# laomao0/BIN

Measured on AMD Instinct MI355X. Metric: interpolated frames/sec at 1280x720, higher is better.
Workload: dtype f16x3 (fp16 hi+lo pairs = 22-bit significands, 3 MFMA products, f32 accumulate; fp32-class: 1e-6 vs the fp32 reference); 1 GPU; Adobe240 test_blur 1280x720 inference, batch=1 per GPU (6-frame window padded to 768x1344 by the test.py rule), window-sharded; precision=f16x3, streams=1, pipelined_steps=False, four_call_schedule=False, parity=max-abs <= 2e-5 (f16x3) vs the fp32 reference (tests/)

## Files before the change

### bin_amd/_lib.py

```python
import ctypes as C
import os

from .build import EMA_LIB_PATH, ENS_LIB_PATH, GRAD_LIB_PATH, LIB_PATH, OPT_LIB_PATH, YUV_LIB_PATH

RDN_LAYERS = 66
RDN_MAX_LAYERS, RDN_MAX_CONVS = 192, 7
PLAN_KEEP_ACTS, PLAN_NO_FUSE, PLAN_RDB3, PLAN_FUSED_UPNET, PLAN_FUSED_UPNET_TRAIN = 1, 2, 4, 8, 16
BWD_ACCUMULATE = 1
BWD_SAVED_X3 = 2
BWD_FUSED_UPNET = 4
EPI_PLANES, EPI_SHUFFLE, EPI_FINAL, EPI_FINAL_SUBPIX = 0, 1, 2, 4
PROF_WGRAD = 16
LOSS_CHARBONNIER, LOSS_L1_SUM, LOSS_L2_SUM = 0, 1, 2
RDN_LAYOUT_WORDS, RDN_BWD_LAYOUT_WORDS = 16, 24


class BinConvDesc(C.Structure):
    _fields_ = [("N", C.c_int32), ("H", C.c_int32), ("W", C.c_int32), ("ksize", C.c_int32),
                ("cin_chunks", C.c_int32), ("cout", C.c_int32), ("cout_pad", C.c_int32),
                ("nterms", C.c_int32), ("epilogue", C.c_int32), ("relu", C.c_int32),
                ("x_cpg", C.c_int32), ("x_group_stride", C.c_int64), ("n_images", C.c_int32),
                ("reserved", C.c_int32), ("status", C.c_void_p)]


LOSS_MAX_TERMS = 24
CONV_HALF_LAST_CHUNK = 1


class BinLossTerms(C.Structure):
    _fields_ = [("x", C.c_void_p * LOSS_MAX_TERMS), ("y", C.c_void_p * LOSS_MAX_TERMS), ("n_terms", C.c_int32)]


class BinLossGrads(C.Structure):
    _fields_ = [("out", C.c_void_p * LOSS_MAX_TERMS), ("term_a", C.c_int32 * LOSS_MAX_TERMS),
                ("term_b", C.c_int32 * LOSS_MAX_TERMS), ("sign_a", C.c_float * LOSS_MAX_TERMS),
                ("sign_b", C.c_float * LOSS_MAX_TERMS), ("n_out", C.c_int32)]


class BinRdnShape(C.Structure):
    _fields_ = [("G0", C.c_int32), ("D", C.c_int32), ("C", C.c_int32), ("G", C.c_int32)]


class BinRdnPlan(C.Structure):
    _fields_ = [("N", C.c_int32), ("H", C.c_int32), ("W", C.c_int32), ("n_inputs", C.c_int32),
                ("nterms", C.c_int32), ("reserved", C.c_int32), ("shape", BinRdnShape),
                ("w_hi", C.c_void_p * RDN_MAX_LAYERS), ("w_lo", C.c_void_p * RDN_MAX_LAYERS),
                ("bias", C.c_void_p * RDN_MAX_LAYERS), ("status", C.c_void_p), ("profiler", C.c_void_p)]


class BinRdnBwdPlan(C.Structure):
    _fields_ = [("N", C.c_int32), ("H", C.c_int32), ("W", C.c_int32), ("n_inputs", C.c_int32),
                ("nterms", C.c_int32), ("reserved", C.c_int32), ("shape", BinRdnShape),
                ("wt_hi", C.c_void_p * RDN_MAX_LAYERS), ("wt_lo", C.c_void_p * RDN_MAX_LAYERS),
                ("zero_bias", C.c_void_p),
                ("dw", C.c_void_p * RDN_MAX_LAYERS), ("db", C.c_void_p * RDN_MAX_LAYERS), ("gin", C.c_void_p * 5),
                ("status", C.c_void_p), ("aux_stream", C.c_void_p), ("profiler", C.c_void_p)]


class BinRelayoutItem(C.Structure):
    _fields_ = [("w", C.c_void_p * (RDN_MAX_CONVS + 1)), ("bias", C.c_void_p), ("w_hi", C.c_void_p), ("w_lo", C.c_void_p),
                ("bias_out", C.c_void_p), ("kind", C.c_int32), ("cout", C.c_int32), ("cin", C.c_int32),
                ("ksize", C.c_int32), ("rows_pad", C.c_int32), ("cin_chunks", C.c_int32), ("cout_block", C.c_int32),
                ("shuffle_or_group", C.c_int32), ("shape", BinRdnShape)]


RELAYOUT_FWD, RELAYOUT_DGRAD, RELAYOUT_RDB_GATHER = 0, 1, 2
SCORE_SSIM_G11, SCORE_SSIM_U7 = 1, 2
SCORE_MAX_PAIRS = 32

ADAM_MAX_TENSORS = 64


class BinAdamTensor(C.Structure):
    _fields_ = [("p", C.c_void_p), ("g", C.c_void_p), ("m", C.c_void_p), ("v", C.c_void_p), ("numel", C.c_int64),
                ("step_size", C.c_float), ("inv_sqrt_bc2", C.c_float)]


GRAD_MAX_TENSORS = 128
GRAD_FLAG_NONFINITE, GRAD_FLAG_STATUS = 1, 2


class BinGradTensor(C.Structure):
    _fields_ = [("g", C.c_void_p), ("numel", C.c_int64)]


class BinGradRecord(C.Structure):
    _fields_ = [("sumsq", C.c_double), ("norm", C.c_float), ("coef", C.c_float), ("flags", C.c_int32), ("status", C.c_uint32),
                ("reserved", C.c_int32 * 2)]


EMA_MAX_TENSORS = 136


class BinEmaTensor(C.Structure):
    _fields_ = [("e", C.c_void_p), ("p", C.c_void_p), ("numel", C.c_int64)]


ENS_FLIP_W, ENS_FLIP_H = 1, 2
ENS_MAX_ORIENT, ENS_MAX_SOURCES, ENS_MAX_SLOTS = 8, 6, 14


class BinEnsOrient(C.Structure):
    _fields_ = [("src", C.c_void_p), ("dst", C.c_void_p * ENS_MAX_ORIENT), ("flip", C.c_uint8 * ENS_MAX_ORIENT), ("n_dst", C.c_int32)]


class BinEnsMerge(C.Structure):
    _fields_ = [("src", C.c_void_p * ENS_MAX_ORIENT), ("dst", C.c_void_p)]


YUV_CHROMA_420, YUV_CHROMA_444 = 420, 444
YUV_MATRIX_BT601, YUV_MATRIX_BT709 = 0, 1
YUV_RANGE_LIMITED, YUV_RANGE_FULL = 0, 1


class BinYuvFormat(C.Structure):
    _fields_ = [("chroma", C.c_int32), ("matrix", C.c_int32), ("range", C.c_int32)]


_SIGNATURES = {
    "binhip_version": (C.c_int, []),
    "binhip_device_cus": (C.c_int, []),
    "binhip_conv_cout_block": (C.c_int, [C.c_int, C.c_int, C.c_int]),
    "binhip_weights_bytes": (C.c_size_t, [C.c_int, C.c_int, C.c_int]),
    "binhip_weights_relayout": (C.c_int, [C.c_void_p, C.c_void_p, C.c_int, C.c_int, C.c_int, C.c_int, C.c_int,
                                          C.c_int, C.c_int, C.c_void_p, C.c_void_p, C.c_void_p, C.c_void_p]),
    "binhip_weights_relayout_batch": (C.c_int, [C.POINTER(BinRelayoutItem), C.c_int, C.c_void_p]),
    "binhip_conv2d_fwd": (C.c_int, [C.POINTER(BinConvDesc)] + [C.c_void_p] * 10 +
                          [C.POINTER(C.c_void_p), C.c_void_p]),
    "binhip_nchw_to_planes": (C.c_int, [C.c_void_p, C.c_int, C.c_int, C.c_int, C.c_int, C.c_void_p, C.c_void_p,
                                        C.c_void_p, C.c_void_p]),
    "binhip_planes_to_nchw": (C.c_int, [C.c_void_p, C.c_void_p, C.c_int, C.c_int, C.c_int, C.c_int, C.c_void_p,
                                        C.c_void_p]),
    "binhip_pixel_unshuffle_f32": (C.c_int, [C.c_void_p, C.c_int, C.c_int, C.c_int, C.c_int, C.c_int, C.c_void_p,
                                             C.c_void_p]),
    "binhip_pack_inputs": (C.c_int, [C.POINTER(C.c_void_p), C.c_int, C.c_int, C.c_int, C.c_int, C.c_void_p,
                                     C.c_void_p, C.c_void_p, C.c_void_p]),
    "binhip_u8_to_frame": (C.c_int, [C.c_void_p, C.c_int, C.c_int, C.c_int, C.c_int, C.c_int, C.c_int, C.c_void_p,
                                     C.c_void_p]),
    "binhip_frame_to_u8": (C.c_int, [C.c_void_p, C.c_int, C.c_int, C.c_int, C.c_int, C.c_int, C.c_int, C.c_void_p,
                                     C.c_void_p]),
    "binhip_convlstm_fwd": (C.c_int, [C.c_void_p] * 5 + [C.c_float, C.c_int, C.c_int, C.c_int, C.c_void_p,
                                                          C.c_void_p, C.c_void_p]),
    "binhip_lstm_gates_fwd": (C.c_int, [C.c_void_p, C.c_void_p, C.c_float, C.c_int, C.c_int, C.c_int, C.c_int, C.c_void_p,
                                        C.c_void_p, C.c_void_p]),
    "binhip_lstm_gates_bwd": (C.c_int, [C.c_void_p] * 4 + [C.c_float, C.c_int, C.c_int, C.c_int, C.c_int, C.c_void_p, C.c_void_p,
                                        C.c_void_p]),
    "binhip_charbonnier_partials": (C.c_int, [C.c_int64]),
    "binhip_charbonnier_fwd": (C.c_int, [C.c_void_p, C.c_void_p, C.c_int64, C.c_float, C.c_void_p, C.c_void_p,
                                         C.c_void_p]),
    "binhip_charbonnier_bwd": (C.c_int, [C.c_void_p, C.c_void_p, C.c_int64, C.c_float, C.c_void_p, C.c_void_p,
                                         C.c_void_p, C.c_void_p]),
    "binhip_pixel_loss_fwd": (C.c_int, [C.c_int, C.c_void_p, C.c_void_p, C.c_int64, C.c_float, C.c_void_p, C.c_void_p,
                                        C.c_void_p]),
    "binhip_pixel_loss_bwd": (C.c_int, [C.c_int, C.c_void_p, C.c_void_p, C.c_int64, C.c_float, C.c_void_p, C.c_void_p,
                                        C.c_void_p, C.c_void_p]),
    "binhip_multi_loss_fwd": (C.c_int, [C.c_int, C.POINTER(BinLossTerms), C.c_int64, C.c_float, C.c_void_p, C.c_void_p,
                                        C.c_void_p, C.c_void_p]),
    "binhip_multi_loss_bwd": (C.c_int, [C.c_int, C.POINTER(BinLossTerms), C.c_int64, C.c_float, C.c_void_p,
                                        C.POINTER(BinLossGrads), C.c_void_p]),
    "binhip_dgrad_rows_pad": (C.c_int, [C.c_int, C.c_int]),
    "binhip_weights_relayout_dgrad": (C.c_int, [C.c_void_p, C.c_int, C.c_int, C.c_int, C.c_int, C.c_int, C.c_int,
                                                C.c_int, C.c_void_p, C.c_void_p, C.c_void_p, C.c_void_p]),
    "binhip_weights_relayout_rdb_gather": (C.c_int, [C.c_void_p, C.c_int, C.c_int, C.c_void_p, C.c_void_p, C.c_void_p,
                                                     C.c_void_p]),
    "binhip_conv2d_bwd_data": (C.c_int, [C.POINTER(BinConvDesc)] + [C.c_void_p] * 7 + [C.c_int, C.c_void_p,
                                         C.c_void_p, C.c_void_p, C.c_int, C.c_int, C.c_int64, C.c_void_p,
                                         C.c_void_p, C.c_void_p]),
    "binhip_wgrad_workspace_bytes": (C.c_size_t, [C.c_int] * 6),
    "binhip_conv2d_bwd_weight": (C.c_int, [C.POINTER(BinConvDesc)] + [C.c_void_p] * 6 + [C.c_size_t, C.c_void_p,
                                           C.c_void_p, C.c_int, C.c_int, C.c_int, C.c_void_p]),
    "binhip_grad_scale": (C.c_int, [C.c_void_p, C.c_int64, C.c_float, C.c_void_p, C.c_void_p, C.c_void_p]),
    "binhip_nchw_to_planes_scaled": (C.c_int, [C.c_void_p, C.c_int, C.c_int, C.c_int, C.c_int, C.c_void_p,
                                               C.c_void_p, C.c_void_p, C.c_void_p, C.c_void_p]),
    "binhip_unshuffle_planes": (C.c_int, [C.c_void_p, C.c_void_p, C.c_int, C.c_int, C.c_int, C.c_int, C.c_void_p,
                                          C.c_void_p, C.c_void_p]),
    "binhip_unpack_input_grads": (C.c_int, [C.c_void_p, C.c_void_p, C.c_void_p, C.c_void_p, C.c_int, C.c_int, C.c_int,
                                            C.c_int, C.POINTER(C.c_void_p), C.c_void_p]),
    "binhip_convlstm_bwd_workspace_bytes": (C.c_size_t, [C.c_int, C.c_int, C.c_int]),
    "binhip_convlstm_bwd": (C.c_int, [C.c_void_p] * 5 + [C.c_float, C.c_int, C.c_int, C.c_int, C.c_void_p, C.c_void_p,
                                      C.c_void_p, C.c_size_t] + [C.c_void_p] * 6),
    "binhip_rdn_backward_workspace_bytes": (C.c_size_t, [C.c_int] * 5 + [C.POINTER(BinRdnShape)]),
    "binhip_rdn_backward": (C.c_int, [C.POINTER(BinRdnBwdPlan), C.c_void_p, C.c_size_t, C.c_void_p, C.c_void_p,
                                      C.c_size_t, C.c_void_p]),
    "binhip_profiler_create": (C.c_int, [C.c_int, C.c_int, C.c_int, C.c_int, C.POINTER(C.c_void_p)]),
    "binhip_profiler_read": (C.c_int, [C.c_void_p, C.POINTER(C.c_double), C.POINTER(C.c_int)]),
    "binhip_profiler_destroy": (None, [C.c_void_p]),
    "binhip_rdb_tail_fwd": (C.c_int, [C.c_int, C.c_int, C.c_int, C.c_int] + [C.c_void_p] * 10 +
                            [C.c_int, C.c_void_p, C.c_void_p]),
    "binhip_rdn_workspace_bytes": (C.c_size_t, [C.c_int, C.c_int, C.c_int, C.c_int, C.c_int, C.POINTER(BinRdnShape)]),
    "binhip_rdn_workspace_layout": (C.c_int, [C.c_int] * 5 + [C.POINTER(BinRdnShape), C.POINTER(C.c_int64), C.c_int]),
    "binhip_rdn_backward_workspace_layout": (C.c_int, [C.c_int] * 5 + [C.POINTER(BinRdnShape), C.POINTER(C.c_int64), C.c_int]),
    "binhip_rdn_forward": (C.c_int, [C.POINTER(BinRdnPlan), C.POINTER(C.c_void_p), C.c_void_p, C.c_void_p,
                                     C.c_size_t, C.c_void_p]),
    "binhip_image_score_workspace_bytes": (C.c_size_t, [C.c_int] * 4),
    "binhip_image_score": (C.c_int, [C.c_void_p, C.c_void_p, C.c_int, C.c_int, C.c_int, C.c_int, C.POINTER(C.c_double),
                                     C.c_void_p, C.c_size_t, C.c_void_p, C.c_void_p]),
    "binhip_frame_score_workspace_bytes": (C.c_size_t, [C.c_int] * 4),
    "binhip_frame_score": (C.c_int, [C.POINTER(C.c_void_p), C.POINTER(C.c_void_p), C.c_int, C.c_int, C.c_int, C.c_int,
                                     C.POINTER(C.c_double), C.c_void_p, C.c_size_t, C.c_void_p, C.c_void_p]),
    "binhip_gather_windows": (C.c_int, [C.c_void_p, C.c_int, C.c_int, C.c_int, C.c_void_p, C.c_int, C.c_int, C.c_int, C.c_int,
                                        C.c_void_p, C.c_void_p]),
    "binhip_gather_windows_blur": (C.c_int, [C.c_void_p, C.c_int, C.c_int, C.c_int, C.c_void_p] + [C.c_int] * 5 +
                                   [C.c_void_p, C.c_void_p]),
}

OPT_VERSION = 100
_OPT_SIGNATURES = {
    "binopt_version": (C.c_int, []),
    "binopt_adam_step": (C.c_int, [C.POINTER(BinAdamTensor), C.c_int, C.c_float, C.c_float, C.c_float, C.c_float, C.c_void_p]),
}

GRAD_VERSION = 100
_GRAD_SIGNATURES = {
    "bingrad_version": (C.c_int, []),
    "bingrad_norm_workspace_bytes": (C.c_int64, [C.POINTER(BinGradTensor), C.c_int]),
    "bingrad_norm": (C.c_int, [C.POINTER(BinGradTensor), C.c_int, C.c_float, C.c_void_p, C.c_uint32, C.c_void_p, C.c_void_p,
                               C.c_void_p]),
    "bingrad_scale": (C.c_int, [C.POINTER(BinGradTensor), C.c_int, C.c_void_p, C.c_void_p]),
}

EMA_VERSION = 100
_EMA_SIGNATURES = {
    "binema_version": (C.c_int, []),
    "binema_step": (C.c_int, [C.POINTER(BinEmaTensor), C.c_int, C.c_float, C.c_void_p]),
}

ENS_VERSION = 100
_ENS_SIGNATURES = {
    "binens_version": (C.c_int, []),
    "binens_orient": (C.c_int, [C.POINTER(BinEnsOrient), C.c_int, C.c_int, C.c_int, C.c_int, C.c_void_p]),
    "binens_merge": (C.c_int, [C.POINTER(BinEnsMerge), C.c_int, C.c_int, C.POINTER(C.c_uint8), C.c_int, C.c_int, C.c_int, C.c_void_p]),
}

YUV_VERSION = 100
_YUV_SIGNATURES = {
    "binyuv_version": (C.c_int, []),
    "binyuv_to_frame": (C.c_int, [C.c_void_p, C.c_void_p, C.c_void_p, C.c_int, C.c_int, C.POINTER(BinYuvFormat), C.c_int, C.c_int, C.c_int,
                                  C.c_int, C.c_void_p, C.c_void_p]),
    "binyuv_from_frame": (C.c_int, [C.c_void_p, C.c_int, C.c_int, C.c_int, C.c_int, C.c_int, C.c_int, C.POINTER(BinYuvFormat), C.c_void_p,
                                    C.c_void_p, C.c_void_p, C.c_void_p]),
}

STATUS_SATURATED = 1
STATUS_SYNC_TIMEOUT = 2

_lib = _optlib = _gradlib = _emalib = _enslib = _yuvlib = None


def _load(path, built_path, signatures, version=None):
    if not os.path.exists(path):
        raise RuntimeError(
            f"bin_amd: HIP library {built_path} not built. Run `python -c 'import __graft_entry__ as g; "
            f"g.build()'` (hipcc --offload-arch=gfx950). There is no CPU fallback by design.")
    h = C.CDLL(path)
    for name, (res, args) in signatures.items():
        fn = getattr(h, name)
        fn.restype = res
        fn.argtypes = args
    if version is not None and getattr(h, version[0])() != version[1]:
        raise RuntimeError(f"bin_amd: {path} is version {getattr(h, version[0])()}, this binding is for {version[1]}")
    return h


def exported_symbols():
    return sorted(_SIGNATURES)


def lib():
    global _lib
    if _lib is None:
        _lib = _load(os.environ.get("BIN_AMD_LIB", LIB_PATH), LIB_PATH, _SIGNATURES)
    return _lib


def opt_exported_symbols():
    return sorted(_OPT_SIGNATURES)


def optlib():
    global _optlib
    if _optlib is None:
        _optlib = _load(OPT_LIB_PATH, OPT_LIB_PATH, _OPT_SIGNATURES, ("binopt_version", OPT_VERSION))
    return _optlib


def grad_exported_symbols():
    return sorted(_GRAD_SIGNATURES)


def gradlib():
    global _gradlib
    if _gradlib is None:
        _gradlib = _load(GRAD_LIB_PATH, GRAD_LIB_PATH, _GRAD_SIGNATURES, ("bingrad_version", GRAD_VERSION))
    return _gradlib


def ema_exported_symbols():
    return sorted(_EMA_SIGNATURES)


def emalib():
    global _emalib
    if _emalib is None:
        _emalib = _load(EMA_LIB_PATH, EMA_LIB_PATH, _EMA_SIGNATURES, ("binema_version", EMA_VERSION))
    return _emalib


def ens_exported_symbols():
    return sorted(_ENS_SIGNATURES)


def enslib():
    global _enslib
    if _enslib is None:
        _enslib = _load(ENS_LIB_PATH, ENS_LIB_PATH, _ENS_SIGNATURES, ("binens_version", ENS_VERSION))
    return _enslib


def yuv_exported_symbols():
    return sorted(_YUV_SIGNATURES)


def yuvlib():
    global _yuvlib
    if _yuvlib is None:
        _yuvlib = _load(YUV_LIB_PATH, YUV_LIB_PATH, _YUV_SIGNATURES, ("binyuv_version", YUV_VERSION))
    return _yuvlib


def check(rc, what):
    if rc != 0:
        kind = {-1: "bad argument", -2: "unsupported shape", -3: "workspace too small"}.get(rc, f"hipError {rc}")
        raise RuntimeError(f"bin_amd: {what} failed: {kind}")
```

### bin_amd/csrc/binhip_conv.hip

```cpp
#include "binhip_conv_common.h"
#include <vector>
#include <cstdio>
#include <cstdlib>

template <int KS, int MT, int WM, int R, int WN, int KC, int NT, int NBUF, int EPI>
struct ConvCfg {
    static constexpr int PAD = KS / 2;
    static constexpr int COUTB = 32 * MT * WM;
    static constexpr int TH = R * WN;
    static constexpr int PH = TH + KS - 1;
    static constexpr int PW = 32 + KS - 1;
    static constexpr int PP = (PH * PW * 2 + 63) / 64;
    static constexpr int WP = KS * KS * MT * WM;
    static constexpr int CHUNK_BYTES = (PP + WP) * 1024;
    static constexpr int NPL = (NT == 3) ? 2 : 1;
    static constexpr int PLANE_BYTES = KC * CHUNK_BYTES;
    static constexpr int BUF_BYTES = NPL * PLANE_BYTES;
    static constexpr int NW = WM * WN;
    static constexpr int LDS_BYTES = NBUF * BUF_BYTES + 1024;
    static constexpr int NPJ = (PP + NW - 1) / NW;
    static constexpr int NWJ = (WP + NW - 1) / NW;
    static constexpr int PS = NPL * KC * (NPJ + NWJ);
    static_assert(NW == 4 || NW == 8 || NW == 16, "4, 8 or 16 waves per workgroup");
    static_assert(LDS_BYTES <= 160 * 1024, "LDS budget");
    static_assert(NBUF >= 2, "ring of at least two stage buffers");
    static_assert(NBUF <= 2 || (NBUF - 2) * PS <= 63, "vmcnt immediate range");
};

template <class C, int KS, int KC>
__device__ __forceinline__ void issue_stage(const ConvKArgs& a, char* smem, int st, int buf, int wave, int lane, const ConvTile& t,
                                            const unsigned* voff) {
    char* bbase = smem + buf * C::BUF_BYTES;
    char* dummy = smem + (C::LDS_BYTES - 1024);
    const int nchunks = a.nchunks;
#pragma unroll
    for (int pl = 0; pl < C::NPL; ++pl) {
#pragma unroll
        for (int kc = 0; kc < KC; ++kc) {
            const int c = st * KC + kc;
            if (c < nchunks) {
                __amdgpu_buffer_rsrc_t rs = patch_plane_grouped(a, c, pl, t);
                char* lds = bbase + pl * C::PLANE_BYTES + kc * C::CHUNK_BYTES;
#pragma unroll
                for (int j = 0; j < C::NPJ; ++j) {
                    const int i = wave + C::NW * j;
                    const bool real = ((C::PP % C::NW == 0) || (i < C::PP));
                    __builtin_amdgcn_raw_ptr_buffer_load_lds(rs, (lds_void_t*)(real ? lds + i * 1024 : dummy), 16,
                                                             real ? voff[j] : 0x80000000u, 0, 0, 0);
                }
                const _Float16* wb = (pl ? a.w_lo : a.w_hi) +
                                     ((long long)t.z * nchunks + c) * (KS * KS * C::COUTB * 16);
                __amdgpu_buffer_rsrc_t ws = __builtin_amdgcn_make_buffer_rsrc(
                    (void*)wb, 0, KS * KS * C::COUTB * 32, 0x00020000);
#pragma unroll
                for (int j = 0; j < C::NWJ; ++j) {
                    const int i = wave + C::NW * j;
                    const bool real = ((C::WP % C::NW == 0) || (i < C::WP));
                    __builtin_amdgcn_raw_ptr_buffer_load_lds(ws, (lds_void_t*)(real ? lds + (C::PP + i) * 1024 : dummy), 16,
                                                             real ? (unsigned)(lane * 16) : 0x80000000u,
                                                             real ? i * 1024 : 0, 0, 0);
                }
            }
        }
    }
}

template <class C, int KS, int MT, int R, int NT>
__device__ __forceinline__ void load_frags(const char* bbase, int kc, int dx, int wm, int a_lane_off, int b_lane_off,
                                           half8 (&Bh)[R + KS - 1], half8 (&Bl)[R + KS - 1],
                                           half8 (&Ah)[KS][MT], half8 (&Al)[KS][MT]) {
    const char* pb = bbase + kc * C::CHUNK_BYTES;
    const char* wb = pb + C::PP * 1024 + wm * (MT * 32 * 32);
#pragma unroll
    for (int rr = 0; rr < R + KS - 1; ++rr) {
        const int off = b_lane_off + (rr * C::PW + dx) * 16;
        Bh[rr] = ld8(pb + off);
        if constexpr (NT == 3) Bl[rr] = ld8(pb + C::PLANE_BYTES + off);
    }
#pragma unroll
    for (int dy = 0; dy < KS; ++dy)
#pragma unroll
        for (int mt = 0; mt < MT; ++mt) {
            const int off = ((dy * KS + dx) * C::COUTB + mt * 32) * 32 + a_lane_off;
            Ah[dy][mt] = ld8(wb + off);
            if constexpr (NT == 3) Al[dy][mt] = ld8(wb + C::PLANE_BYTES + off);
        }
}

template <class C, int KS, int MT, int R, int KC, int NT>
__device__ __forceinline__ void compute_stage(const char* smem, int st, int buf, int nchunks, int wm,
                                              int a_lane_off, int b_lane_off, floatx16 (&acc)[MT][R]) {
    const char* bbase = smem + buf * C::BUF_BYTES;
    constexpr int NSTEP = KC * KS;
    constexpr int FRAG_REGS = ((R + KS - 1) + KS * MT) * 4 * ((NT == 3) ? 2 : 1);
    constexpr bool PIPE = (MT * R * 16 + 2 * FRAG_REGS + 40) <= 232;
    constexpr int NSET = PIPE ? 2 : 1;
    half8 Bh[NSET][R + KS - 1], Bl[NSET][R + KS - 1], Ah[NSET][KS][MT], Al[NSET][KS][MT];
    int nvalid = NSTEP;
    if constexpr (KC > 1) {
        const int left = nchunks - st * KC;
        nvalid = (left < KC ? left : KC) * KS;
    }
    if constexpr (PIPE)
        load_frags<C, KS, MT, R, NT>(bbase, 0, 0, wm, a_lane_off, b_lane_off, Bh[0], Bl[0], Ah[0], Al[0]);
#pragma unroll
    for (int s = 0; s < NSTEP; ++s) {
        if (KC == 1 || s < nvalid) {
            if constexpr (PIPE) {
                if (s + 1 < NSTEP && (KC == 1 || s + 1 < nvalid))
                    load_frags<C, KS, MT, R, NT>(bbase, (s + 1) / KS, (s + 1) % KS, wm, a_lane_off, b_lane_off,
                                                 Bh[(s + 1) & 1], Bl[(s + 1) & 1], Ah[(s + 1) & 1], Al[(s + 1) & 1]);
            } else {
                load_frags<C, KS, MT, R, NT>(bbase, s / KS, s % KS, wm, a_lane_off, b_lane_off, Bh[0], Bl[0], Ah[0], Al[0]);
            }
            if constexpr (PIPE) __builtin_amdgcn_sched_barrier(0);
#pragma unroll
            for (int dy = 0; dy < KS; ++dy)
#pragma unroll
                for (int mt = 0; mt < MT; ++mt)
#pragma unroll
                    for (int r = 0; r < R; ++r) {
                        if constexpr (NT == 3) {
                            acc[mt][r] = mfma_32x32x16(Al[s & (NSET - 1)][dy][mt], Bh[s & (NSET - 1)][r + dy], acc[mt][r]);
                            acc[mt][r] = mfma_32x32x16(Ah[s & (NSET - 1)][dy][mt], Bl[s & (NSET - 1)][r + dy], acc[mt][r]);
                        }
                        acc[mt][r] = mfma_32x32x16(Ah[s & (NSET - 1)][dy][mt], Bh[s & (NSET - 1)][r + dy], acc[mt][r]);
                    }
            if constexpr (PIPE) __builtin_amdgcn_sched_barrier(0);
        }
    }
}

template <int KS, int MT, int WM, int R, int WN, int KC, int NT, int NBUF, int EPI, bool XTRA>
__global__ void __launch_bounds__(64 * WM * WN) __attribute__((amdgpu_waves_per_eu(2)))
conv_mfma_kernel(const ConvKArgs a, const float* __restrict__ bias) {
    using C = ConvCfg<KS, MT, WM, R, WN, KC, NT, NBUF, EPI>;
    extern __shared__ __attribute__((aligned(16))) char smem[];

    const int tid = threadIdx.x;
    const int lane = tid & 63;
    const int wave = __builtin_amdgcn_readfirstlane(tid >> 6);
    const int wm = wave / WN;
    const int wn = wave % WN;
    const int n = lane & 31;
    const int kg = lane >> 5;

    const ConvTile t = tile_decode<C::TH>(a, a.ncol);
    unsigned voff[C::NPJ];
    patch_offsets<C, C::PAD>(voff, t, a.H, a.W, wave, lane);

    floatx16 acc[MT][R];
#pragma unroll
    for (int mt = 0; mt < MT; ++mt)
#pragma unroll
        for (int r = 0; r < R; ++r)
#pragma unroll
            for (int e = 0; e < 16; ++e) acc[mt][r][e] = 0.f;

    const int nchunks = a.nchunks;
    const int nst = (nchunks + KC - 1) / KC;
    const int a_lane_off = weight_lane_off(n, kg);
    const int b_lane_off = patch_lane_off<C>(n, kg, wn * R);

    const int nfull = nchunks / KC;
#pragma unroll
    for (int s0 = 0; s0 < NBUF - 1; ++s0)
        if (s0 < nst) issue_stage<C, KS, KC>(a, smem, s0, s0, wave, lane, t, voff);
    int cur = 0, nxt = NBUF - 1;
    for (int st = 0; st < nst; ++st) {
        int yf = nfull - 1 - st;
        yf = yf < 0 ? 0 : (yf > NBUF - 2 ? NBUF - 2 : yf);
        if (NBUF >= 4 && yf >= 2) wait_vmcnt<(NBUF >= 4 ? 2 : 0) * C::PS>();
        else if (NBUF >= 3 && yf >= 1) wait_vmcnt<(NBUF >= 3 ? 1 : 0) * C::PS>();
        else wait_vmcnt<0>();
        __builtin_amdgcn_s_barrier();
        __builtin_amdgcn_sched_barrier(0);
        if (st + NBUF - 1 < nst)
            issue_stage<C, KS, KC>(a, smem, st + NBUF - 1, nxt, wave, lane, t, voff);
        compute_stage<C, KS, MT, R, KC, NT>(smem, st, cur, nchunks, wm, a_lane_off, b_lane_off, acc);
        cur = (cur + 1 == NBUF) ? 0 : cur + 1;
        nxt = (nxt + 1 == NBUF) ? 0 : nxt + 1;
    }

    conv_epilogue<MT, R, NT, EPI, XTRA>(a, bias, acc, t.img, t.ty0 + wn * R, t.tx0, t.z * C::COUTB + wm * MT * 32, t.z == 0 && wm == 0,
                                        n, kg, t.plane_elems);
}

template <int KS, int MT, int WM, int R, int WN, int KC, int NT, int NBUF, int EPI, bool XTRA>
static int launch_cfg_x(const ConvKArgs& ka, int cout_pad, hipStream_t s) {
    using C = ConvCfg<KS, MT, WM, R, WN, KC, NT, NBUF, EPI>;
    static std::atomic<unsigned long long> lds_set{0};
    if (int rc = bh_set_max_lds(&conv_mfma_kernel<KS, MT, WM, R, WN, KC, NT, NBUF, EPI, XTRA>, C::LDS_BYTES, lds_set)) return rc;
    ConvKArgs a = ka;
    const dim3 grid(set_tiles<C>(a, cout_pad / C::COUTB));
    conv_mfma_kernel<KS, MT, WM, R, WN, KC, NT, NBUF, EPI, XTRA><<<grid, dim3(64 * C::NW), C::LDS_BYTES, s>>>(a, a.bias);
    BH_CHECK_LAUNCH();
    return 0;
}
template <int KS, int MT, int WM, int R, int WN, int KC, int NT, int NBUF, int EPI>
static int launch_cfg(const ConvKArgs& ka, int cout_pad, hipStream_t s) {
    if constexpr (EPI == BINHIP_EPI_PLANES) {
        if (ka.has_res || ka.r2_hi || ka.m_hi || ka.y_unshuf)
            return launch_cfg_x<KS, MT, WM, R, WN, KC, NT, NBUF, EPI, true>(ka, cout_pad, s);
    }
    return launch_cfg_x<KS, MT, WM, R, WN, KC, NT, NBUF, EPI, false>(ka, cout_pad, s);
}

struct BinhipProfiler {
    int ks = 0, cout_pad = 0, epi = 0;
    std::vector<hipEvent_t> ev;
    size_t used = 0;
};
namespace { constexpr size_t PROF_MAX_PAIRS = 16384; }

int bh_conv_cout_block(int ksize, int cout_pad, int nterms) {
    if (cout_pad <= 0 || cout_pad % 32) return -1;
    if (ksize == 3 && nterms == 3) return 32;
    if (ksize == 3 && cout_pad == 256) return 128;
    if (ksize == 5) return 32;
    if (ksize == 1 && cout_pad == 224) return 224;
    if (ksize == 1 && cout_pad == 1152) return 192;
    if (cout_pad % 96 == 0) return 96;
    if (ksize == 3 && cout_pad % 64 == 0) return 64;
    return 32;
}

static int bh_dispatch_conv(const ConvKArgs& a, int k, int cp, int nt, int e, hipStream_t s);
int bh_launch_conv_x3(const ConvKArgs& a, int cout_pad, int epilogue, hipStream_t s);
int bh_launch_final_dot2(const ConvKArgs& a, hipStream_t s);
int bh_launch_conv_x3_k5(const ConvKArgs& a, int cout_pad, hipStream_t s);
int bh_launch_conv_x3_k5_subpix(const ConvKArgs& a, hipStream_t s);
int bh_launch_final_m16(const ConvKArgs& a, hipStream_t s);

int bh_prepare_conv(const BhConvCall& c, ConvKArgs* out) {
    const BinConvDesc& d = c.d;
    if (!c.x_hi || !c.w_hi || !c.bias) return BINHIP_E_ARG;
    if (d.nterms != 1 && d.nterms != 3) return BINHIP_E_ARG;
    if (d.nterms == 3 && (!c.x_lo || !c.w_lo)) return BINHIP_E_ARG;
    if (d.N <= 0 || d.H <= 0 || d.W <= 0 || d.cin_chunks <= 0) return BINHIP_E_SHAPE;
    if ((long long)d.N * d.H * d.W >= (1ll << 26)) return BINHIP_E_SHAPE;
    ConvKArgs a;
    a.x_hi = (const _Float16*)c.x_hi; a.x_lo = (const _Float16*)c.x_lo;
    a.w_hi = (const _Float16*)c.w_hi; a.w_lo = (const _Float16*)c.w_lo;
    a.bias = c.bias;
    a.y_hi = (_Float16*)c.y_hi; a.y_lo = (_Float16*)c.y_lo;
    a.r_hi = (const _Float16*)c.r_hi; a.r_lo = (const _Float16*)c.r_lo;
    a.r2_hi = (const _Float16*)c.r2_hi; a.r2_lo = (const _Float16*)c.r2_lo;
    a.m_hi = (const _Float16*)c.m_hi;
    a.flags = (unsigned*)c.status;
    a.res_chunks = c.res_chunks > 0 ? c.res_chunks : (1 << 30);
    a.mask_from = c.mask_from;
    a.y_cpg = c.y_cpg; a.y_group_stride = c.y_group_stride;
    a.y_cpg_inv = c.y_cpg > 0 ? (unsigned)(((1u << 20) + c.y_cpg - 1) / c.y_cpg) : 0u;
    if (c.y_cpg > 128 || (c.y_cpg > 0 && d.cout_pad / 16 >= 4096)) return BINHIP_E_SHAPE;
    a.half_last = (d.reserved & BINHIP_CONV_HALF_LAST_CHUNK) ? 1 : 0;
    a.y_unshuf = c.y_unshuf;
    if (c.y_unshuf && (d.epilogue != BINHIP_EPI_PLANES || c.y_cpg > 0 || (d.H & 1) || (d.W & 1) || c.y_unshuf * 16 < d.cout))
        return BINHIP_E_SHAPE;
    if (c.r2_hi && d.nterms == 3 && !c.r2_lo) return BINHIP_E_ARG;
    a.out_f32 = c.y_f32;
    for (int i = 0; i < 5; ++i) a.img[i] = c.images[i];
    a.group_stride = d.x_group_stride;
    a.N = d.N; a.H = d.H; a.W = d.W;
    a.nchunks = d.cin_chunks;
    a.cpg = d.x_cpg;
    a.relu = d.relu; a.has_res = (c.r_hi != nullptr); a.nimg = d.n_images; a.cout = d.cout;
    a.och_limit = (d.epilogue == BINHIP_EPI_PLANES) ? (d.cout + 15) / 16 : (1 << 30);
    a.tiles_x = a.tiles_y = 0;
    a.ncol = 1;
    a.wt = 0;
    a.prog_prio = 0;
#if BINHIP_TIMELINE
    a.tl = nullptr; a.tl_launch = 0; a.tl_base = 0;
#endif
    const int P = BINHIP_EPI_PLANES, S = BINHIP_EPI_SHUFFLE, F = BINHIP_EPI_FINAL;
    if (d.epilogue == P) {
        if (!c.y_hi || (d.nterms == 3 && !c.y_lo)) return BINHIP_E_ARG;
        if (a.has_res && d.nterms == 3 && !c.r_lo) return BINHIP_E_ARG;
    } else if (d.epilogue == S) {
        if (!c.y_hi || (d.nterms == 3 && !c.y_lo)) return BINHIP_E_ARG;
        if (d.cout % 4) return BINHIP_E_SHAPE;
    } else if (d.epilogue == F) {
        if (!c.y_f32 || d.cout > 4 || d.n_images < 0 || d.n_images > 5) return BINHIP_E_ARG;
    } else if (d.epilogue == BINHIP_EPI_FINAL_SUBPIX) {
        if (!c.y_f32 || d.cout <= 0 || (d.cout & 3) || d.cout > 12 || d.n_images < 0 || d.n_images > 5) return BINHIP_E_ARG;
        if (d.ksize != 5 || d.cout_pad != 32) return BINHIP_E_SHAPE;
    } else {
        return BINHIP_E_ARG;
    }
    {
        const int e = d.epilogue, cp = d.cout_pad;
        const long long out_chunks = (e == BINHIP_EPI_SHUFFLE) ? (a.cout / 4 + 15) / 16 : (cp + 15) / 16;
        const long long px = (long long)a.N * a.H * a.W * ((e == BINHIP_EPI_SHUFFLE) ? 4 : 1);
        const long long span = (a.y_cpg > 0 ? ((out_chunks + a.y_cpg - 1) / a.y_cpg) * a.y_group_stride * 2 : out_chunks * px * 32);
        a.wt = (e == BINHIP_EPI_PLANES && span < (1ll << 32) - 64) ? 1 : 0;
    }
    *out = a;
    return 0;
}

bool bh_prof_begin(BinhipProfiler* pr, int ks, int cout_pad, int epi, hipStream_t s) {
    if (!pr || ks != pr->ks || cout_pad != pr->cout_pad || epi != pr->epi || pr->used + 2 > pr->ev.size()) return false;
    (void)hipEventRecord(pr->ev[pr->used], s);
    return true;
}
void bh_prof_end(BinhipProfiler* pr, hipStream_t s) {
    (void)hipEventRecord(pr->ev[pr->used + 1], s);
    pr->used += 2;
}

int bh_launch_conv(const BhConvCall& c, hipStream_t s) {
    ConvKArgs a;
    if (int rc = bh_prepare_conv(c, &a)) return rc;
    const BinConvDesc& d = c.d;
    const int k = d.ksize, cp = d.cout_pad, nt = d.nterms, e = d.epilogue;
    if (bh_prof_begin(c.prof, k, cp, e, s)) {
        const int rc = bh_dispatch_conv(a, k, cp, nt, e, s);
        bh_prof_end(c.prof, s);
        return rc;
    }
    return bh_dispatch_conv(a, k, cp, nt, e, s);
}

static int bh_dispatch_conv(const ConvKArgs& a, int k, int cp, int nt, int e, hipStream_t s) {
    const int P = BINHIP_EPI_PLANES, S = BINHIP_EPI_SHUFFLE, F = BINHIP_EPI_FINAL;
    const int cb = bh_conv_cout_block(k, cp, nt);
    if (cb <= 0 || cp % cb) return BINHIP_E_SHAPE;
    if (e == BINHIP_EPI_FINAL_SUBPIX)
        return nt == 3 ? bh_launch_conv_x3_k5_subpix(a, s) : launch_cfg<5, 1, 1, 2, 8, 1, 1, 2, BINHIP_EPI_FINAL_SUBPIX>(a, cp, s);
    if (e == F && k == 3 && cp == 32 && a.cout <= 3 && nt == 1)
        return bh_launch_final_dot2(a, s);
    if (e == F && k == 3 && cp == 32 && a.cout <= 3 && nt == 3 && a.nchunks <= 4)
        return bh_launch_final_m16(a, s);
    if (nt == 1) {
        if (e == F && k == 3 && cp == 32) return launch_cfg<3, 1, 1, 2, 8, 1, 1, 2, F>(a, cp, s);
        if (e == S && k == 3 && cp == 256) return launch_cfg<3, 2, 2, 4, 4, 1, 1, 2, S>(a, cp, s);
        if (e == P && k == 3 && cb == 32)  return launch_cfg<3, 1, 1, 2, 8, 1, 1, 2, P>(a, cp, s);
        if (e == P && k == 3 && cb == 64)  return launch_cfg<3, 2, 1, 2, 4, 1, 1, 2, P>(a, cp, s);
        if (e == P && k == 3 && cb == 96)  return launch_cfg<3, 3, 1, 2, 4, 1, 1, 2, P>(a, cp, s);
        if (e == P && k == 3 && cb == 128) return launch_cfg<3, 2, 2, 4, 4, 1, 1, 2, P>(a, cp, s);
        if (e == P && k == 1 && cb == 224) return launch_cfg<1, 7, 1, 1, 8, 2, 1, 2, P>(a, cp, s);
        if (e == P && k == 1 && cb == 192) return launch_cfg<1, 6, 1, 1, 8, 2, 1, 2, P>(a, cp, s);
        if (e == P && k == 1 && cb == 32)  return launch_cfg<1, 1, 1, 4, 4, 4, 1, 2, P>(a, cp, s);
        if (e == P && k == 1 && cb == 96) {
            if (a.nchunks >= 32) return launch_cfg<1, 3, 1, 2, 4, 2, 1, 2, P>(a, cp, s);
            return launch_cfg<1, 3, 1, 1, 8, 2, 1, 2, P>(a, cp, s);
        }
        if (e == P && k == 5 && cb == 32)  return launch_cfg<5, 1, 1, 2, 8, 1, 1, 2, P>(a, cp, s);
    } else {
        if (k == 3 && cb == 32) return bh_launch_conv_x3(a, cp, e, s);
        if (e == S && k == 3 && cp == 256) return launch_cfg<3, 1, 2, 4, 2, 1, 3, 2, S>(a, cp, s);
        if (e == P && k == 3 && cb == 64)  return launch_cfg<3, 2, 1, 2, 4, 1, 3, 2, P>(a, cp, s);
        if (e == P && k == 3 && cb == 96)  return launch_cfg<3, 3, 1, 1, 8, 1, 3, 2, P>(a, cp, s);
        if (e == P && k == 1 && cb == 224) {
            if (a.has_res && a.m_hi && !a.r2_hi && a.res_chunks == 6 && a.mask_from == 12 && a.y_cpg <= 0 && !a.y_unshuf &&
                a.och_limit >= 14 && cp == 224)
                return launch_cfg_x<1, 7, 1, 1, 8, 1, 3, 2, BINHIP_EPI_PLANES_LFFD, true>(a, cp, s);
            return launch_cfg<1, 7, 1, 1, 8, 1, 3, 2, P>(a, cp, s);
        }
        if (e == P && k == 1 && cb == 192) return launch_cfg<1, 6, 1, 1, 8, 1, 3, 2, P>(a, cp, s);
        if (e == P && k == 1 && cb == 32)  return launch_cfg<1, 1, 1, 4, 4, 2, 3, 2, P>(a, cp, s);
        if (e == P && k == 1 && cb == 96) {
            if (a.nchunks >= 32) return launch_cfg<1, 3, 1, 2, 4, 1, 3, 2, P>(a, cp, s);
            return launch_cfg<1, 3, 1, 1, 8, 1, 3, 2, P>(a, cp, s);
        }
        if (e == P && k == 5 && cb == 32)  return bh_launch_conv_x3_k5(a, cp, s);
    }
    return BINHIP_E_SHAPE;
}

__device__ __forceinline__ void relayout_body(long long t, const float* __restrict__ w, const float* __restrict__ bias,
                                              int cout, int cin, int ks, int cout_pad, int nchunks, int cb, int shuffle,
                                              _Float16* __restrict__ w_hi, _Float16* __restrict__ w_lo,
                                              float* __restrict__ bias_out) {
    const long long total = (long long)cout_pad * nchunks * ks * ks * 2;
    if (t < cout_pad) {
        int src = (int)t;
        if (shuffle) { const int cq = cout / 4; const int sub = (int)t / cq, cc = (int)t % cq; src = cc * 4 + sub; }
        bias_out[t] = (src < cout && bias) ? bias[src] : 0.f;
    }
    if (t >= total) return;
    const int s = (int)(t & 1);
    long long u = t >> 1;
    const int row = (int)(u % cb); u /= cb;
    const int tap = (int)(u % (ks * ks)); u /= (ks * ks);
    const int c = (int)(u % nchunks); u /= nchunks;
    const int zb = (int)u;
    const int rg = zb * cb + row;
    int src = rg;
    if (shuffle) { const int cq = cout / 4; const int sub = rg / cq, cc = rg % cq; src = cc * 4 + sub; }
    const int cg = s ^ ((row >> 3) & 1);
    const int dy = tap / ks, dx = tap % ks;
    half8 hv, lv;
#pragma unroll
    for (int e = 0; e < 8; ++e) {
        const int ci = c * 16 + cg * 8 + e;
        float v = 0.f;
        if (src < cout && ci < cin) v = w[(((long long)src * cin + ci) * ks + dy) * ks + dx];
        hv[e] = (_Float16)v;
        lv[e] = (_Float16)(v - (float)hv[e]);
    }
    *reinterpret_cast<half8*>(w_hi + t * 8) = hv;
    if (w_lo) *reinterpret_cast<half8*>(w_lo + t * 8) = lv;
}
__global__ void relayout_kernel(const float* __restrict__ w, const float* __restrict__ bias, int cout, int cin,
                                int ks, int cout_pad, int nchunks, int cb, int shuffle,
                                _Float16* __restrict__ w_hi, _Float16* __restrict__ w_lo,
                                float* __restrict__ bias_out) {
    relayout_body((long long)blockIdx.x * blockDim.x + threadIdx.x, w, bias, cout, cin, ks, cout_pad, nchunks, cb, shuffle,
                  w_hi, w_lo, bias_out);
}

__device__ __forceinline__ void relayout_dgrad_body(long long t, const float* __restrict__ w, int cout, int cin, int ks,
                                                    int rows_pad, int nchunks, int cb, int shuffle,
                                                    _Float16* __restrict__ w_hi, _Float16* __restrict__ w_lo,
                                                    float* __restrict__ bias_out) {
    const long long total = (long long)rows_pad * nchunks * ks * ks * 2;
    if (t < rows_pad) bias_out[t] = 0.f;
    if (t >= total) return;
    const int s = (int)(t & 1);
    long long u = t >> 1;
    const int row = (int)(u % cb); u /= cb;
    const int tap = (int)(u % (ks * ks)); u /= (ks * ks);
    const int c = (int)(u % nchunks); u /= nchunks;
    const int zb = (int)u;
    const int r = zb * cb + row;
    const int cg = s ^ ((row >> 3) & 1);
    const int dy = ks - 1 - tap / ks, dx = ks - 1 - tap % ks;
    half8 hv, lv;
#pragma unroll
    for (int e = 0; e < 8; ++e) {
        const int j = c * 16 + cg * 8 + e;
        int co = j;
        if (shuffle) { const int cq = cout / 4; const int sub = j / cq, cc = j % cq; co = cc * 4 + sub; }
        float v = 0.f;
        if (r < cin && j < cout) v = w[(((long long)co * cin + r) * ks + dy) * ks + dx];
        hv[e] = (_Float16)v;
        lv[e] = (_Float16)(v - (float)hv[e]);
    }
    *reinterpret_cast<half8*>(w_hi + t * 8) = hv;
    if (w_lo) *reinterpret_cast<half8*>(w_lo + t * 8) = lv;
}
__global__ void relayout_dgrad_kernel(const float* __restrict__ w, int cout, int cin, int ks, int rows_pad,
                                      int nchunks, int cb, int shuffle, _Float16* __restrict__ w_hi,
                                      _Float16* __restrict__ w_lo, float* __restrict__ bias_out) {
    relayout_dgrad_body((long long)blockIdx.x * blockDim.x + threadIdx.x, w, cout, cin, ks, rows_pad, nchunks, cb, shuffle,
                        w_hi, w_lo, bias_out);
}

struct GatherSrc { const float* w[BINHIP_RDN_MAX_CONVS + 1]; int G0, G; };
__device__ __forceinline__ void relayout_rdb_gather_body(long long t, const GatherSrc& src, int group, int rows, int nchunks,
                                                         int cb, _Float16* __restrict__ w_hi, _Float16* __restrict__ w_lo,
                                                         float* __restrict__ bias_out) {
    const long long total = (long long)rows * nchunks * 9 * 2;
    if (t < rows) bias_out[t] = 0.f;
    if (t >= total) return;
    const int s = (int)(t & 1);
    long long u = t >> 1;
    const int row = (int)(u % cb); u /= cb;
    const int tap = (int)(u % 9); u /= 9;
    const int c = (int)(u % nchunks); u /= nchunks;
    const int r = (int)u * cb + row;
    const int cg = s ^ ((row >> 3) & 1);
    const int dy = 2 - tap / 3, dx = 2 - tap % 3;
    const int G0 = src.G0, G = src.G;
    const int cmin = group;
    const int ci = (group == 0) ? r : G0 + G * (group - 1) + r;
    const int j0 = c * 16 + cg * 8;
    const int conv = cmin + j0 / G;
    const int cin_c = G0 + G * conv;
    const float* w = src.w[conv];
    half8 hv, lv;
#pragma unroll
    for (int e = 0; e < 8; ++e) {
        const int co = (j0 % G) + e;
        const float v = w[(((long long)co * cin_c + ci) * 3 + dy) * 3 + dx];
        hv[e] = (_Float16)v;
        lv[e] = (_Float16)(v - (float)hv[e]);
    }
    *reinterpret_cast<half8*>(w_hi + t * 8) = hv;
    if (w_lo) *reinterpret_cast<half8*>(w_lo + t * 8) = lv;
}
__global__ void relayout_rdb_gather_kernel(GatherSrc src, int group, int rows, int nchunks, int cb,
                                           _Float16* __restrict__ w_hi, _Float16* __restrict__ w_lo,
                                           float* __restrict__ bias_out) {
    relayout_rdb_gather_body((long long)blockIdx.x * blockDim.x + threadIdx.x, src, group, rows, nchunks, cb, w_hi, w_lo, bias_out);
}

#define RELAYOUT_BATCH 22
struct RelayoutBatch {
    BinRelayoutItem it[RELAYOUT_BATCH];
    unsigned start[RELAYOUT_BATCH + 1];
    int n;
};
__global__ void __launch_bounds__(256)
relayout_batch_kernel(const RelayoutBatch rb) {
    const unsigned b = blockIdx.x;
    int li = 0;
#pragma unroll
    for (int i = 1; i < RELAYOUT_BATCH; ++i)
        if (i < rb.n && b >= rb.start[i]) li = i;
    const BinRelayoutItem& L = rb.it[li];
    const long long t = (long long)(b - rb.start[li]) * 256 + threadIdx.x;
    if (L.kind == BINHIP_RELAYOUT_FWD) {
        relayout_body(t, L.w[0], L.bias, L.cout, L.cin, L.ksize, L.rows_pad, L.cin_chunks, L.cout_block, L.shuffle_or_group,
                      (_Float16*)L.w_hi, (_Float16*)L.w_lo, L.bias_out);
    } else if (L.kind == BINHIP_RELAYOUT_DGRAD) {
        relayout_dgrad_body(t, L.w[0], L.cout, L.cin, L.ksize, L.rows_pad, L.cin_chunks, L.cout_block, L.shuffle_or_group,
                            (_Float16*)L.w_hi, (_Float16*)L.w_lo, L.bias_out);
    } else {
        GatherSrc src;
#pragma unroll
        for (int i = 0; i <= BINHIP_RDN_MAX_CONVS; ++i) src.w[i] = L.w[i];
        src.G0 = L.shape.G0 > 0 ? L.shape.G0 : 96;
        src.G = L.shape.G > 0 ? L.shape.G : 32;
        relayout_rdb_gather_body(t, src, L.shuffle_or_group, L.rows_pad, L.cin_chunks, L.cout_block, (_Float16*)L.w_hi,
                                 (_Float16*)L.w_lo, L.bias_out);
    }
}

extern "C" {

int binhip_weights_relayout_batch(const BinRelayoutItem* items, int n, void* stream) {
    if (!items || n <= 0) return BINHIP_E_ARG;
    for (int i = 0; i < n; ++i) {
        const BinRelayoutItem& L = items[i];
        if (!L.w[0] || !L.w_hi || !L.bias_out) return BINHIP_E_ARG;
        if (L.kind == BINHIP_RELAYOUT_FWD) {
            if (L.rows_pad % 32 || L.cout_block <= 0 || L.rows_pad % L.cout_block || L.cout_block % 32) return BINHIP_E_SHAPE;
            if (L.cin > L.cin_chunks * 16 || L.cout > L.rows_pad) return BINHIP_E_SHAPE;
            if (L.shuffle_or_group && (L.cout % 4 || L.cout != L.rows_pad)) return BINHIP_E_SHAPE;
        } else if (L.kind == BINHIP_RELAYOUT_DGRAD) {
            if (L.rows_pad % 32 || L.cout_block <= 0 || L.rows_pad % L.cout_block || L.cout_block % 32) return BINHIP_E_SHAPE;
            if (L.cin > L.rows_pad || L.cout > L.cin_chunks * 16) return BINHIP_E_SHAPE;
            if (L.shuffle_or_group && L.cout % 4) return BINHIP_E_SHAPE;
        } else if (L.kind == BINHIP_RELAYOUT_RDB_GATHER) {
            const int g = L.shuffle_or_group;
            const int G0 = L.shape.G0 > 0 ? L.shape.G0 : 96, G = L.shape.G > 0 ? L.shape.G : 32, C = L.shape.C > 0 ? L.shape.C : 4;
            if (C > BINHIP_RDN_MAX_CONVS || G0 % 32 || G % 32) return BINHIP_E_SHAPE;
            if (g < 0 || g >= C) return BINHIP_E_ARG;
            if (L.rows_pad != (g == 0 ? G0 : G) || L.cin_chunks != (C - g) * G / 16 || L.ksize != 3) return BINHIP_E_SHAPE;
            if (L.cout_block <= 0 || L.rows_pad % L.cout_block || L.cout_block % 32) return BINHIP_E_SHAPE;
            for (int k = g; k < C; ++k) if (!L.w[k]) return BINHIP_E_ARG;
        } else {
            return BINHIP_E_ARG;
        }
    }
    for (int i0 = 0; i0 < n; i0 += RELAYOUT_BATCH) {
        RelayoutBatch rb;
        const int m = (n - i0 < RELAYOUT_BATCH) ? n - i0 : RELAYOUT_BATCH;
        unsigned blocks = 0;
        for (int i = 0; i < m; ++i) {
            rb.it[i] = items[i0 + i];
            rb.start[i] = blocks;
            const BinRelayoutItem& L = rb.it[i];
            const long long total = (long long)L.rows_pad * L.cin_chunks * L.ksize * L.ksize * 2;
            blocks += (unsigned)((total + 255) / 256);
        }
        for (int i = m; i < RELAYOUT_BATCH; ++i) rb.it[i] = rb.it[0];
        for (int i = m; i <= RELAYOUT_BATCH; ++i) rb.start[i] = blocks;
        rb.n = m;
        hipLaunchKernelGGL(relayout_batch_kernel, dim3(blocks), dim3(256), 0, (hipStream_t)stream, rb);
        BH_CHECK_LAUNCH();
    }
    return 0;
}

int binhip_dgrad_rows_pad(int ksize, int cin) {
    return ((cin + 31) / 32) * 32;
}

int binhip_weights_relayout_dgrad(const float* w_oihw, int cout, int cin, int ksize, int rows_pad, int cin_chunks,
                                  int cout_block, int shuffle_perm, void* w_hi, void* w_lo, float* bias_out,
                                  void* stream) {
    if (!w_oihw || !w_hi || !bias_out) return BINHIP_E_ARG;
    if (rows_pad % 32 || cout_block <= 0 || rows_pad % cout_block || cout_block % 32) return BINHIP_E_SHAPE;
    if (cin > rows_pad || cout > cin_chunks * 16) return BINHIP_E_SHAPE;
    if (shuffle_perm && cout % 4) return BINHIP_E_SHAPE;
    const long long total = (long long)rows_pad * cin_chunks * ksize * ksize * 2;
    const long long nb = (total + 255) / 256;
    hipLaunchKernelGGL(relayout_dgrad_kernel, dim3((unsigned)nb), dim3(256), 0, (hipStream_t)stream, w_oihw, cout, cin,
                       ksize, rows_pad, cin_chunks, cout_block, shuffle_perm, (_Float16*)w_hi, (_Float16*)w_lo, bias_out);
    BH_CHECK_LAUNCH();
    return 0;
}

int binhip_weights_relayout_rdb_gather(const float* const* w_oihw4, int group, int cout_block, void* w_hi, void* w_lo,
                                       float* bias_out, void* stream) {
    if (!w_oihw4 || !w_hi || !bias_out || group < 0 || group > 3) return BINHIP_E_ARG;
    const int rows = group == 0 ? 96 : 32;
    const int nchunks = 2 * (4 - group);
    if (cout_block <= 0 || rows % cout_block || cout_block % 32) return BINHIP_E_SHAPE;
    GatherSrc src;
    for (int i = 0; i <= BINHIP_RDN_MAX_CONVS; ++i) src.w[i] = nullptr;
    src.G0 = 96; src.G = 32;
    for (int i = 0; i < 4; ++i) {
        src.w[i] = w_oihw4[i];
        if (i >= group && !src.w[i]) return BINHIP_E_ARG;
    }
    const long long total = (long long)rows * nchunks * 9 * 2;
    hipLaunchKernelGGL(relayout_rdb_gather_kernel, dim3((unsigned)((total + 255) / 256)), dim3(256), 0,
                       (hipStream_t)stream, src, group, rows, nchunks, cout_block, (_Float16*)w_hi, (_Float16*)w_lo,
                       bias_out);
    BH_CHECK_LAUNCH();
    return 0;
}

int binhip_conv2d_bwd_data(const BinConvDesc* d, const void* gy_hi, const void* gy_lo, const void* wt_hi,
                           const void* wt_lo, const float* zero_bias, const void* res_hi, const void* res_lo,
                           int res_chunks, const void* acc_hi, const void* acc_lo, const void* mask_hi, int mask_from,
                           int y_cpg, int64_t y_group_stride, void* gx_hi, void* gx_lo, void* stream) {
    if (!d) return BINHIP_E_ARG;
    if (d->epilogue != BINHIP_EPI_PLANES) return BINHIP_E_ARG;
    if (d->reserved < 0) return BINHIP_E_ARG;
    BhConvCall c;
    c.d = *d;
    c.x_hi = gy_hi; c.x_lo = gy_lo; c.w_hi = wt_hi; c.w_lo = wt_lo; c.bias = zero_bias;
    c.r_hi = res_hi; c.r_lo = res_lo; c.res_chunks = res_chunks;
    c.r2_hi = acc_hi; c.r2_lo = acc_lo;
    c.m_hi = mask_hi; c.mask_from = mask_from;
    c.y_cpg = y_cpg; c.y_group_stride = y_group_stride;
    c.y_unshuf = d->reserved > 0 ? d->reserved : 0;
    c.d.reserved = 0;
    c.y_hi = gx_hi; c.y_lo = gx_lo;
    c.status = d->status;
    return bh_launch_conv(c, (hipStream_t)stream);
}

#if BINHIP_TIMELINE
BINHIP_API int binhip_set_timeline(void* buf, unsigned cap) {
    const unsigned used = g_bh_tl_next.exchange(0);
    g_bh_tl_buf = buf;
    g_bh_tl_cap = cap;
    g_bh_tl_serial.store(0);
    return (int)(used < g_bh_tl_cap || !buf ? used : used);
}
#endif

int binhip_profiler_create(int ksize, int cout_pad, int epilogue, int max_launches, BinhipProfiler** out) {
    if (!out || max_launches <= 0 || (size_t)max_launches > PROF_MAX_PAIRS) return BINHIP_E_ARG;
    BinhipProfiler* p = new BinhipProfiler();
    p->ks = ksize; p->cout_pad = cout_pad; p->epi = epilogue;
    for (int i = 0; i < 2 * max_launches; ++i) {
        hipEvent_t ev;
        hipError_t e = hipEventCreate(&ev);
        if (e != hipSuccess) { binhip_profiler_destroy(p); return (int)e; }
        p->ev.push_back(ev);
    }
    *out = p;
    return 0;
}

int binhip_profiler_read(BinhipProfiler* p, double* total_ms, int* launches) {
    if (!p) return BINHIP_E_ARG;
    double tot = 0.0;
    int n = 0;
    for (size_t i = 0; i + 1 < p->used; i += 2) {
        hipError_t e = hipEventSynchronize(p->ev[i + 1]);
        if (e != hipSuccess) return (int)e;
        float ms = 0.f;
        e = hipEventElapsedTime(&ms, p->ev[i], p->ev[i + 1]);
        if (e != hipSuccess) return (int)e;
        tot += ms;
        ++n;
    }
    if (total_ms) *total_ms = tot;
    if (launches) *launches = n;
    p->used = 0;
    return 0;
}

void binhip_profiler_destroy(BinhipProfiler* p) {
    if (!p) return;
    for (hipEvent_t ev : p->ev) (void)hipEventDestroy(ev);
    delete p;
}

int binhip_conv_cout_block(int ksize, int cout_pad, int nterms) { return bh_conv_cout_block(ksize, cout_pad, nterms); }

size_t binhip_weights_bytes(int cout_pad, int cin_chunks, int ksize) {
    return (size_t)cout_pad * cin_chunks * ksize * ksize * 32;
}

int binhip_weights_relayout(const float* w_oihw, const float* bias, int cout, int cin, int ksize,
                            int cout_pad, int cin_chunks, int cout_block, int shuffle_perm,
                            void* w_hi, void* w_lo, float* bias_out, void* stream) {
    if (!w_oihw || !w_hi || !bias_out) return BINHIP_E_ARG;
    if (cout_pad % 32 || cout_block <= 0 || cout_pad % cout_block || cout_block % 32) return BINHIP_E_SHAPE;
    if (cin > cin_chunks * 16 || cout > cout_pad) return BINHIP_E_SHAPE;
    if (shuffle_perm && (cout % 4 || cout != cout_pad)) return BINHIP_E_SHAPE;
    const long long total = (long long)cout_pad * cin_chunks * ksize * ksize * 2;
    const int th = 256;
    const long long nb = (total + th - 1) / th;
    hipLaunchKernelGGL(relayout_kernel, dim3((unsigned)nb), dim3(th), 0, (hipStream_t)stream, w_oihw, bias, cout, cin,
                       ksize, cout_pad, cin_chunks, cout_block, shuffle_perm, (_Float16*)w_hi, (_Float16*)w_lo,
                       bias_out);
    BH_CHECK_LAUNCH();
    return 0;
}

int binhip_conv2d_fwd(const BinConvDesc* d, const void* x_hi, const void* x_lo, const void* w_hi,
                      const void* w_lo, const float* bias, const void* res_hi, const void* res_lo,
                      void* y_hi, void* y_lo, float* y_f32, const float* const* images, void* stream) {
    if (!d) return BINHIP_E_ARG;
    if (d->reserved & ~BINHIP_CONV_HALF_LAST_CHUNK) return BINHIP_E_ARG;
    if ((d->reserved & BINHIP_CONV_HALF_LAST_CHUNK) && d->ksize != 5) return BINHIP_E_ARG;
    BhConvCall c;
    c.d = *d;
    c.x_hi = x_hi; c.x_lo = x_lo; c.w_hi = w_hi; c.w_lo = w_lo; c.bias = bias;
    c.r_hi = res_hi; c.r_lo = res_lo; c.y_hi = y_hi; c.y_lo = y_lo; c.y_f32 = y_f32;
    c.status = d->status;
    for (int i = 0; images && i < d->n_images && i < 5; ++i) c.images[i] = images[i];
    if (d->epilogue == BINHIP_EPI_FINAL && d->n_images > 0 && !images) return BINHIP_E_ARG;
    return bh_launch_conv(c, (hipStream_t)stream);
}

}
```

### bin_amd/csrc/binhip_conv_common.h

```cpp
#pragma once
#include "binhip_internal.h"
#include <type_traits>
#ifndef BINHIP_TIMELINE
#define BINHIP_TIMELINE 0
#endif

typedef _Float16 half8 __attribute__((ext_vector_type(8)));
typedef _Float16 half4 __attribute__((ext_vector_type(4)));
typedef float floatx16 __attribute__((ext_vector_type(16)));
typedef float floatx4 __attribute__((ext_vector_type(4)));
typedef __attribute__((address_space(3))) void lds_void_t;
typedef unsigned u32x4 __attribute__((ext_vector_type(4)));

int bh_launch_upnet_ring(const void* x_hi, const void* x_lo, const float* wvar, const float* bvar, float* out, const float* const* images,
                         int nimg, int N, int H, int W, int cin, hipStream_t s);
int bh_upnet_gsub(const float* g, int N, int H, int W, const float* scale, void* y_hi, void* y_lo, void* status, hipStream_t s);
int bh_upnet_ring_dgrad(const float* g, const float* wvar, const float* scale, void* gx_hi, void* gx_lo, void* status, int N, int H, int W,
                        int cin, hipStream_t s);
int bh_upnet_ring_wgrad(const float* g, const void* x_hi, const void* x_lo, float* dwvar, float* dbvar, int N, int H, int W, int cin,
                        int accumulate, hipStream_t s);
struct ConvKArgs {
    const _Float16* x_hi;
    const _Float16* x_lo;
    const _Float16* w_hi;
    const _Float16* w_lo;
    const float* bias;
    _Float16* y_hi;
    _Float16* y_lo;
    const _Float16* r_hi;
    const _Float16* r_lo;
    const _Float16* r2_hi;
    const _Float16* r2_lo;
    const _Float16* m_hi;
    float* out_f32;
    const float* img[5];
    unsigned* flags;
    long long group_stride;
    int N, H, W;
    int nchunks;
    int cpg;
    int tiles_x, tiles_y;
    int ncol;
    int relu, has_res, nimg, cout;
    int wt;
    int och_limit;
    int res_chunks;
    int mask_from;
    int y_cpg;
    unsigned y_cpg_inv;
    long long y_group_stride;
    int prog_prio;
    int half_last;
#if BINHIP_TIMELINE
    void* tl;
    unsigned tl_launch;
    unsigned tl_base;
#endif
    int y_unshuf;
};

#if BINHIP_TIMELINE
#include <atomic>
struct BhTlRec {
    unsigned kind_launch, bid, hwid, xcc;
    unsigned long long rt[5];
    unsigned long long clk[2];
    unsigned long long pad;
};
static_assert(sizeof(BhTlRec) == 80, "record size (tools/wg_timeline.py)");
struct BhTlBuf { unsigned cursor, cap, pad[2]; BhTlRec rec[1]; };
inline void* g_bh_tl_buf = nullptr;
inline unsigned g_bh_tl_cap = 0;
inline std::atomic<unsigned> g_bh_tl_serial{0}, g_bh_tl_next{0};
inline void* bh_tl_reserve(unsigned n, unsigned* base) {
    if (!g_bh_tl_buf) return nullptr;
    const unsigned b = g_bh_tl_next.fetch_add(n);
    *base = b;
    return (b + n <= g_bh_tl_cap) ? g_bh_tl_buf : nullptr;
}
struct BhTl {
    unsigned long long rt[5], clk[2];
    __device__ __forceinline__ void stamp(int i) {
        __builtin_amdgcn_sched_barrier(0);
        rt[i] = __builtin_amdgcn_s_memrealtime();
        __builtin_amdgcn_sched_barrier(0);
    }
    __device__ __forceinline__ void begin() { clk[0] = __builtin_amdgcn_s_memtime(); stamp(0); }
    __device__ __forceinline__ void finish(void* tl, unsigned kind_launch, unsigned i) {
        stamp(3);
        if (threadIdx.x < 64) asm volatile("s_waitcnt vmcnt(0)" ::: "memory");
        stamp(4);
        clk[1] = __builtin_amdgcn_s_memtime();
        if (tl && threadIdx.x == 0) {
            BhTlBuf* b = (BhTlBuf*)tl;
            {
                BhTlRec& r = b->rec[i];
                r.kind_launch = kind_launch; r.bid = blockIdx.x;
                r.hwid = __builtin_amdgcn_s_getreg((31 << 11) | 4);
                r.xcc = __builtin_amdgcn_s_getreg((31 << 11) | 20);
                for (int k = 0; k < 5; ++k) r.rt[k] = rt[k];
                r.clk[0] = clk[0]; r.clk[1] = clk[1];
            }
        }
    }
};
#define BH_TL_DECL BhTl tl__
#define BH_TL_BEGIN() tl__.begin()
#define BH_TL_STAMP(i) tl__.stamp(i)
#define BH_TL_FINISH(a, i) tl__.finish((a).tl, (a).tl_launch, (a).tl_base + (unsigned)(i))
#else
#define BH_TL_DECL
#define BH_TL_BEGIN()
#define BH_TL_STAMP(i)
#define BH_TL_FINISH(a, i)
#endif

#define BINHIP_EPI_PLANES_LFFD 3

template <int N>
__device__ __forceinline__ void wait_vmcnt() {
    asm volatile("s_waitcnt vmcnt(%0)" ::"n"(N) : "memory");
}

__device__ __forceinline__ void store16(_Float16* base, long long off_elems, uint4 v, int wt) {
    if (wt) {
        __amdgpu_buffer_rsrc_t rs = __builtin_amdgcn_make_buffer_rsrc((void*)base, 0, 0xFFFFFFFFu, 0x00020000);
        u32x4 d = {v.x, v.y, v.z, v.w};
        __builtin_amdgcn_raw_buffer_store_b128(d, rs, (int)(off_elems * 2), 0, 16);
    } else {
        *reinterpret_cast<uint4*>(base + off_elems) = v;
    }
}

__device__ __forceinline__ int xcd_band(int bid, int nwg) {
    const int q = nwg >> 3, r = nwg & 7, xcd = bid & 7, k = bid >> 3;
    return (xcd < r ? xcd * (q + 1) : r * (q + 1) + (xcd - r) * q) + k;
}

struct ConvTile {
    int z, tx, ty, img;
    int tx0, ty0;
    long long plane_elems;
    unsigned plane_bytes;
};
template <int TH, class A>
__device__ __forceinline__ ConvTile tile_at(const A& a, int t, int z) {
    ConvTile o;
    o.z = z;
    o.tx = t % a.tiles_x;
    t /= a.tiles_x;
    o.ty = t % a.tiles_y;
    o.img = t / a.tiles_y;
    o.tx0 = o.tx * 32;
    o.ty0 = o.ty * TH;
    o.plane_elems = (long long)a.N * a.H * a.W * 16;
    o.plane_bytes = (unsigned)(o.plane_elems * 2);
    return o;
}
template <int TH, class A>
__device__ __forceinline__ ConvTile tile_decode(const A& a, int ncol) {
    const int bid = xcd_band(blockIdx.x, gridDim.x);
    return tile_at<TH>(a, bid / ncol, bid % ncol);
}
template <class C, class A>
inline unsigned set_tiles(A& a, int ncol = 1) {
    a.tiles_x = (a.W + 31) / 32;
    a.tiles_y = (a.H + C::TH - 1) / C::TH;
    if constexpr (std::is_same<A, ConvKArgs>::value) a.ncol = ncol;
    return (unsigned)(a.tiles_x * a.tiles_y * a.N * ncol);
}

template <class C, int PAD>
__device__ __forceinline__ void patch_offsets(unsigned (&voff)[C::NPJ], const ConvTile& t, int H, int W, int wave, int lane) {
#pragma unroll
    for (int j = 0; j < C::NPJ; ++j) {
        const int i = wave + C::NW * j;
        const int q = i * 64 + lane;
        const int cg = q >= C::PH * C::PW ? 1 : 0;
        const int p = q - cg * (C::PH * C::PW);
        const int py = p / C::PW;
        const int px = p - py * C::PW;
        const int gy = t.ty0 + py - PAD;
        const int gx = t.tx0 + px - PAD;
        const bool ok = (p < C::PH * C::PW) && (gy >= 0) && (gy < H) && (gx >= 0) && (gx < W);
        voff[j] = ok ? (unsigned)((((long long)t.img * H + gy) * W + gx) * 32 + cg * 16) : 0x80000000u;
    }
}

template <class A>
__device__ __forceinline__ __amdgpu_buffer_rsrc_t patch_plane(const A& a, int c, int pl, const ConvTile& t) {
    return __builtin_amdgcn_make_buffer_rsrc((void*)((pl ? a.x_lo : a.x_hi) + (long long)c * t.plane_elems), 0, t.plane_bytes, 0x00020000);
}
__device__ __forceinline__ __amdgpu_buffer_rsrc_t patch_plane_grouped(const ConvKArgs& a, int c, int pl, const ConvTile& t) {
    const long long coff = (a.cpg > 0) ? (long long)(c / a.cpg) * a.group_stride + (long long)(c % a.cpg) * t.plane_elems
                                       : (long long)c * t.plane_elems;
    return __builtin_amdgcn_make_buffer_rsrc((void*)((pl ? a.x_lo : a.x_hi) + coff), 0, t.plane_bytes, 0x00020000);
}

__device__ __forceinline__ half8 ld8(const char* p) { return *reinterpret_cast<const half8*>(p); }
__device__ __forceinline__ floatx16 mfma_32x32x16(half8 a, half8 b, floatx16 c) {
    return __builtin_amdgcn_mfma_f32_32x32x16_f16(a, b, c, 0, 0, 0);
}
__device__ __forceinline__ int weight_lane_off(int n, int kg) { return n * 32 + ((kg ^ ((n >> 3) & 1)) << 4); }
template <class C>
__device__ __forceinline__ int patch_lane_off(int n, int kg, int row) { return (kg * (C::PH * C::PW) + row * C::PW + n) * 16; }

template <int MT, int R, int NT, int EPI, bool XTRA>
__device__ __forceinline__ void conv_epilogue(const ConvKArgs& a, const float* __restrict__ bias, floatx16 (&acc)[MT][R],
                                              int img, int row0, int tx0, int co0, bool first_col, int n, int kg,
                                              long long plane_elems) {
    const int H = a.H, W = a.W;
    const int gx = tx0 + n;
    auto bias4 = [&](int co_u, float (&bv)[4]) {
        float b8[8];
#pragma unroll
        for (int j = 0; j < 8; ++j) b8[j] = bias[co_u + j];
#pragma unroll
        for (int j = 0; j < 4; ++j) bv[j] = kg ? b8[4 + j] : b8[j];
    };
    if constexpr (EPI == BINHIP_EPI_FINAL_SUBPIX) {
        const int ncolour = a.cout >> 2;
        const int H2 = 2 * H, W2 = 2 * W;
        float bv[2][4];
        bias4(co0, bv[0]);
        bias4(co0 + 8, bv[1]);
        const bool col_ok = first_col && (gx < W);
        float sum[R][2][4];
#pragma unroll
        for (int r = 0; r < R; ++r) {
            const int gy = row0 + r;
#pragma unroll
            for (int g = 0; g < 2; ++g) {
                const int c = 2 * g + kg;
                const bool ok = col_ok && gy < H && c < ncolour;
#pragma unroll
                for (int q = 0; q < 4; ++q) {
                    float sj = 0.f;
                    if (ok && a.nimg > 0) {
                        const long long idx = (((long long)img * ncolour + c) * H2 + 2 * gy + (q >> 1)) * W2 + 2 * gx + (q & 1);
                        sj = a.img[0][idx];
                        for (int t = 1; t < a.nimg; ++t) sj += a.img[t][idx];
                        sj = sj / (float)a.nimg;
                    }
                    sum[r][g][q] = sj;
                }
            }
        }
#pragma unroll
        for (int r = 0; r < R; ++r) {
            const int gy = row0 + r;
#pragma unroll
            for (int g = 0; g < 2; ++g) {
                const int c = 2 * g + kg;
                if (!(col_ok && gy < H && c < ncolour)) continue;
#pragma unroll
                for (int q = 0; q < 4; ++q) {
                    const long long idx = (((long long)img * ncolour + c) * H2 + 2 * gy + (q >> 1)) * W2 + 2 * gx + (q & 1);
                    a.out_f32[idx] = (acc[0][r][4 * g + q] + bv[g][q]) + sum[r][g][q];
                }
            }
        }
    } else if constexpr (EPI == BINHIP_EPI_FINAL) {
        float bv[4];
        bias4(co0, bv);
        const bool mine = (kg == 0) && first_col && (gx < W);
        float sum[R][4];
#pragma unroll
        for (int r = 0; r < R; ++r) {
            const int gy = row0 + r;
#pragma unroll
            for (int j = 0; j < 4; ++j) {
                float sj = 0.f;
                if (mine && gy < H && j < a.cout && a.nimg > 0) {
                    const long long idx = (((long long)img * a.cout + j) * H + gy) * W + gx;
                    sj = a.img[0][idx];
                    for (int t = 1; t < a.nimg; ++t) sj += a.img[t][idx];
                    sj = sj / (float)a.nimg;
                }
                sum[r][j] = sj;
            }
        }
#pragma unroll
        for (int r = 0; r < R; ++r) {
            const int gy = row0 + r;
            if (!(mine && gy < H)) continue;
#pragma unroll
            for (int j = 0; j < 4; ++j) {
                if (j >= a.cout) break;
                const long long idx = (((long long)img * a.cout + j) * H + gy) * W + gx;
                a.out_f32[idx] = (acc[0][r][j] + bv[j]) + sum[r][j];
            }
        }
    } else {
        union H4 { half4 h; unsigned u[2]; };
        unsigned sat = 0;
        const int gxc = gx < W ? gx : W - 1;
        constexpr bool X = XTRA && (EPI == BINHIP_EPI_PLANES || EPI == BINHIP_EPI_PLANES_LFFD);
        constexpr int MTG = (X && MT >= 6) ? 2 : 1;
        const bool use_res = X && a.has_res;
        const bool use_r2 = X && (a.r2_hi != nullptr);
        const bool use_m = X && (a.m_hi != nullptr);
        constexpr bool LFFD = EPI == BINHIP_EPI_PLANES_LFFD;
        static_assert(!LFFD || (XTRA && MT == 7 && NT == 3), "the LFF backward-data epilogue");
        if constexpr (LFFD) {
            {
#pragma unroll
                for (int r = 0; r < R; ++r) {
                    const int gy = row0 + r;
                    const bool ok = (gy < H) && (gx < W);
                    const int gyc = gy < H ? gy : H - 1;
                    const long long pix = (((long long)img * H + gyc) * W + gxc) << 4;
                    auto emit = [&](const int mt, const half4 (&xr)[4], const half4 (&xrl)[4], const half4 (&xm)[4], const int kind)
                        __attribute__((always_inline)) {
#pragma unroll
                        for (int gp = 0; gp < 2; ++gp) {
                            H4 hv[2], lv[2];
                            long long o_slot = 0;
#pragma unroll
                            for (int ge = 0; ge < 2; ++ge) {
                                const int g = 2 * gp + ge;
                                float bv[4];
                                bias4(mt * 32 + 8 * g, bv);
                                float v[4] = {acc[mt][r][4 * g + 0] + bv[0], acc[mt][r][4 * g + 1] + bv[1],
                                              acc[mt][r][4 * g + 2] + bv[2], acc[mt][r][4 * g + 3] + bv[3]};
                                const int co = mt * 32 + 8 * g + 4 * kg;
                                const long long o = (long long)(co >> 4) * plane_elems + pix + (co & 15);
                                if (kind == 1) {
#pragma unroll
                                    for (int j = 0; j < 4; ++j) v[j] += (float)xr[g][j];
#pragma unroll
                                    for (int j = 0; j < 4; ++j) v[j] += (float)xrl[g][j];
                                }
                                if (kind == 2) {
#pragma unroll
                                    for (int j = 0; j < 4; ++j) v[j] = ((float)xm[g][j] > 0.f) ? v[j] : 0.f;
                                }
                                if (ge == kg) o_slot = o - 4 * kg;
                                split_pair(v[0], v[1], sat, hv[ge].u[0], lv[ge].u[0], a.relu);
                                split_pair(v[2], v[3], sat, hv[ge].u[1], lv[ge].u[1], a.relu);
                            }
#pragma unroll
                            for (int k = 0; k < 2; ++k) {
                                auto sw = __builtin_amdgcn_permlane32_swap(hv[0].u[k], hv[1].u[k], false, false);
                                hv[0].u[k] = sw[0]; hv[1].u[k] = sw[1];
                                auto sl = __builtin_amdgcn_permlane32_swap(lv[0].u[k], lv[1].u[k], false, false);
                                lv[0].u[k] = sl[0]; lv[1].u[k] = sl[1];
                            }
                            if (ok) {
                                store16(a.y_hi, o_slot, make_uint4(hv[0].u[0], hv[0].u[1], hv[1].u[0], hv[1].u[1]), a.wt);
                                store16(a.y_lo, o_slot, make_uint4(lv[0].u[0], lv[0].u[1], lv[1].u[0], lv[1].u[1]), a.wt);
                            }
                        }
                    };
                    auto fetch = [&](const int mt, const _Float16* hi, const _Float16* lo, half4 (&xh)[4], half4 (&xl)[4])
                        __attribute__((always_inline)) {
#pragma unroll
                        for (int g = 0; g < 4; ++g) {
                            const int co = mt * 32 + 8 * g + 4 * kg;
                            const long long o = (long long)(co >> 4) * plane_elems + pix + (co & 15);
                            xh[g] = *reinterpret_cast<const half4*>(hi + o);
                            if (lo) xl[g] = *reinterpret_cast<const half4*>(lo + o);
                        }
                    };
                    half4 ra[4], ral[4], rb[4], rbl[4], rc[4], rcl[4], rm[4], none[4] = {};
                    fetch(0, a.r_hi, a.r_lo, ra, ral);
                    fetch(1, a.r_hi, a.r_lo, rb, rbl);
                    fetch(2, a.r_hi, a.r_lo, rc, rcl);
                    fetch(6, a.m_hi, nullptr, rm, none);
                    auto pin = [](half4 (&x)[4]) __attribute__((always_inline)) {
#pragma unroll
                        for (int g = 0; g < 4; ++g) {
                            H4 t;
                            t.h = x[g];
                            asm volatile("" : "+v"(t.u[0]), "+v"(t.u[1]));
                            x[g] = t.h;
                        }
                    };
                    asm volatile("s_waitcnt vmcnt(0)" ::: "memory");
                    pin(ra); pin(ral); pin(rb); pin(rbl); pin(rc); pin(rcl); pin(rm);
                    __builtin_amdgcn_sched_barrier(0);
                    emit(0, ra, ral, none, 1);
                    emit(1, rb, rbl, none, 1);
                    emit(2, rc, rcl, none, 1);
                    emit(6, none, none, rm, 2);
                    emit(3, none, none, none, 0);
                    emit(4, none, none, none, 0);
                    emit(5, none, none, none, 0);
                }
            }
        }
        if constexpr (!LFFD) {
#pragma unroll
        for (int r = 0; r < R; ++r) {
            const int gy = row0 + r;
            const bool ok = (gy < H) && (gx < W);
            const int gyc = gy < H ? gy : H - 1;
#pragma unroll
            for (int mt0 = 0; mt0 < MT; mt0 += MTG) {
                long long off[MTG][4];
                half4 xr[MTG][4] = {}, xrl[MTG][4] = {}, x2[MTG][4] = {}, x2l[MTG][4] = {}, xm[MTG][4] = {};
#pragma unroll
                for (int mi = 0; mi < MTG; ++mi) {
                    const int mt = mt0 + mi;
                    if (mt >= MT) continue;
#pragma unroll
                    for (int g = 0; g < 4; ++g) {
                        const int co = co0 + mt * 32 + 8 * g + 4 * kg;
                        long long o;
                        if constexpr (EPI == BINHIP_EPI_SHUFFLE) {
                            const int cq = (a.cout + 3) / 4;
                            const int sub = co / cq, cc = co - sub * cq;
                            const int oy = 2 * gyc + (sub >> 1), ox = 2 * gxc + (sub & 1);
                            o = (long long)(cc >> 4) * (plane_elems * 4) +
                                ((((long long)img * 2 * H + oy) * (2 * W) + ox) << 4) + (cc & 15);
                        } else {
                            const int och = co >> 4;
                            const long long pix16 = ((((long long)img * H + gyc) * W + gxc) << 4) + (co & 15);
                            if (a.y_cpg > 0) {
                                const int q = (int)(((unsigned)och * a.y_cpg_inv) >> 20);
                                o = (long long)q * a.y_group_stride + (long long)(och - q * a.y_cpg) * plane_elems + pix16;
                            } else {
                                o = (long long)och * plane_elems + pix16;
                            }
                            if constexpr (X) {
                                if (a.y_unshuf > 0) {
                                    const int sub = ((gyc & 1) << 1) | (gxc & 1);
                                    o = (long long)(sub * a.y_unshuf + och) * (plane_elems >> 2) +
                                        ((((long long)img * (H >> 1) + (gyc >> 1)) * (W >> 1) + (gxc >> 1)) << 4) + (co & 15);
                                }
                            }
                            if constexpr (X) {
                                const bool live = och < a.och_limit;
                                if (use_res && och < a.res_chunks && live) {
                                    xr[mi][g] = *reinterpret_cast<const half4*>(a.r_hi + o);
                                    if constexpr (NT == 3) xrl[mi][g] = *reinterpret_cast<const half4*>(a.r_lo + o);
                                }
                                if (use_r2 && live) {
                                    x2[mi][g] = *reinterpret_cast<const half4*>(a.r2_hi + o);
                                    if constexpr (NT == 3) x2l[mi][g] = *reinterpret_cast<const half4*>(a.r2_lo + o);
                                }
                                if (use_m && och >= a.mask_from && live) xm[mi][g] = *reinterpret_cast<const half4*>(a.m_hi + o);
                            }
                        }
                        off[mi][g] = o;
                    }
                }
                if constexpr (X) {
                    asm volatile("s_waitcnt vmcnt(0)" ::: "memory");
#pragma unroll
                    for (int mi = 0; mi < MTG; ++mi)
#pragma unroll
                        for (int g = 0; g < 4; ++g) {
                            auto pin = [](half4& x) __attribute__((always_inline)) {
                                H4 t;
                                t.h = x;
                                asm volatile("" : "+v"(t.u[0]), "+v"(t.u[1]));
                                x = t.h;
                            };
                            pin(xr[mi][g]); pin(x2[mi][g]); pin(xm[mi][g]);
                            if constexpr (NT == 3) { pin(xrl[mi][g]); pin(x2l[mi][g]); }
                        }
                    __builtin_amdgcn_sched_barrier(0);
                }
#pragma unroll
                for (int mi = 0; mi < MTG; ++mi) {
                    const int mt = mt0 + mi;
                    if (mt >= MT) continue;
#pragma unroll
                    for (int gp = 0; gp < 2; ++gp) {
                        H4 hv[2], lv[2];
                        long long o_slot = 0;
#pragma unroll
                        for (int ge = 0; ge < 2; ++ge) {
                            const int g = 2 * gp + ge;
                            float bv[4];
                            bias4(co0 + mt * 32 + 8 * g, bv);
                            float v[4] = {acc[mt][r][4 * g + 0] + bv[0], acc[mt][r][4 * g + 1] + bv[1],
                                          acc[mt][r][4 * g + 2] + bv[2], acc[mt][r][4 * g + 3] + bv[3]};
                            const long long o = off[mi][g];
                            if constexpr (EPI != BINHIP_EPI_SHUFFLE) {
                                const int och = (co0 + mt * 32 + 8 * g + 4 * kg) >> 4;
                                const bool live = och < a.och_limit;
                                if constexpr (X) {
                                    if (use_res && och < a.res_chunks && live) {
#pragma unroll
                                        for (int j = 0; j < 4; ++j) v[j] += (float)xr[mi][g][j];
                                        if constexpr (NT == 3) {
#pragma unroll
                                            for (int j = 0; j < 4; ++j) v[j] += (float)xrl[mi][g][j];
                                        }
                                    }
                                    if (use_r2 && live) {
#pragma unroll
                                        for (int j = 0; j < 4; ++j) v[j] += (float)x2[mi][g][j];
                                        if constexpr (NT == 3) {
#pragma unroll
                                            for (int j = 0; j < 4; ++j) v[j] += (float)x2l[mi][g][j];
                                        }
                                    }
                                }
                                if constexpr (X) {
                                    if (use_m && och >= a.mask_from && live) {
#pragma unroll
                                        for (int j = 0; j < 4; ++j) v[j] = ((float)xm[mi][g][j] > 0.f) ? v[j] : 0.f;
                                    }
                                }
                            }
                            if (ge == kg) o_slot = o - 4 * kg;
                            const bool fold_relu = a.relu && (EPI != BINHIP_EPI_SHUFFLE);
                            split_pair(v[0], v[1], sat, hv[ge].u[0], lv[ge].u[0], fold_relu);
                            split_pair(v[2], v[3], sat, hv[ge].u[1], lv[ge].u[1], fold_relu);
                        }
#pragma unroll
                        for (int k = 0; k < 2; ++k) {
                            auto sw = __builtin_amdgcn_permlane32_swap(hv[0].u[k], hv[1].u[k], false, false);
                            hv[0].u[k] = sw[0]; hv[1].u[k] = sw[1];
                            if constexpr (NT == 3) {
                                auto sl = __builtin_amdgcn_permlane32_swap(lv[0].u[k], lv[1].u[k], false, false);
                                lv[0].u[k] = sl[0]; lv[1].u[k] = sl[1];
                            }
                        }
                        if (ok && ((co0 + mt * 32 + 16 * gp) >> 4) < a.och_limit) {
                            store16(a.y_hi, o_slot, make_uint4(hv[0].u[0], hv[0].u[1], hv[1].u[0], hv[1].u[1]), a.wt);
                            if constexpr (NT == 3)
                                store16(a.y_lo, o_slot, make_uint4(lv[0].u[0], lv[0].u[1], lv[1].u[0], lv[1].u[1]), a.wt);
                        }
                    }
                }
            }
        }
        }
        if (a.flags && __builtin_amdgcn_ballot_w64(sat != 0) != 0 && (threadIdx.x & 63) == 0)
            atomicOr(a.flags, BINHIP_FLAG_SATURATED);
    }
}
```

### bin_amd/csrc/binhip_conv_x3.hip

```cpp
#include "binhip_conv_common.h"
constexpr int X3_R = 2, X3_WN = 8;

template <int KS, int R, int WN>
struct X3Cfg {
    static constexpr int PAD = KS / 2;
    static constexpr int TH = R * WN;
    static constexpr int PH = TH + KS - 1;
    static constexpr int PW = 32 + KS - 1;
    static constexpr int PP = (PH * PW * 2 + 63) / 64;
    static constexpr int WP = KS * KS;
    static constexpr int NW = WN;
    static constexpr int PATCH_BYTES = PP * 1024;
    static constexpr int WBUF_BYTES = 2 * WP * 1024;
    static constexpr int LDS_BYTES = 2 * PATCH_BYTES + 2 * WBUF_BYTES;
    static constexpr int NPJ = (PP + NW - 1) / NW;
    static constexpr int NWJ = (2 * WP + NW - 1) / NW;
    static_assert((KS == 3 ? 2 : 1) * LDS_BYTES <= 160 * 1024, "LDS budget");
};

template <class C>
__device__ __forceinline__ void x3_issue_patch(const ConvKArgs& a, char* smem, int c, int pl, int buf, int wave,
                                               const unsigned* voff, const ConvTile& t) {
    __amdgpu_buffer_rsrc_t rs = patch_plane_grouped(a, c, pl, t);
    char* lds = smem + buf * C::PATCH_BYTES;
#pragma unroll
    for (int j = 0; j < C::NPJ; ++j) {
        const int i = wave + C::NW * j;
        if ((C::PP % C::NW == 0) || (i < C::PP))
            __builtin_amdgcn_raw_ptr_buffer_load_lds(rs, (lds_void_t*)(lds + i * 1024), 16, voff[j], 0, 0, 0);
    }
}

template <class C, int KS>
__device__ __forceinline__ void x3_issue_weights(const ConvKArgs& a, char* smem, int c, int buf, int wave, int lane, int z) {
    const long long woff = ((long long)z * a.nchunks + c) * (KS * KS * 32 * 16);
    __amdgpu_buffer_rsrc_t wh = __builtin_amdgcn_make_buffer_rsrc((void*)(a.w_hi + woff), 0, KS * KS * 1024, 0x00020000);
    __amdgpu_buffer_rsrc_t wl = __builtin_amdgcn_make_buffer_rsrc((void*)(a.w_lo + woff), 0, KS * KS * 1024, 0x00020000);
    char* lds = smem + 2 * C::PATCH_BYTES + buf * C::WBUF_BYTES;
#pragma unroll
    for (int j = 0; j < C::NWJ; ++j) {
        const int i = wave + C::NW * j;
        if (((2 * C::WP) % C::NW == 0) || (i < 2 * C::WP)) {
            const bool lo = i >= C::WP;
            const int t = lo ? i - C::WP : i;
            __builtin_amdgcn_raw_ptr_buffer_load_lds(lo ? wl : wh, (lds_void_t*)(lds + i * 1024), 16,
                                                     (unsigned)(lane * 16), t * 1024, 0, 0);
        }
    }
}

template <class C, int KS, int R, bool HI>
__device__ __forceinline__ void x3_compute(const char* pb, const char* wb, int a_lane_off, int b_lane_off, floatx16 (&acc)[R]) {
    constexpr int NTAP = KS * KS;
    half8 B[2][R + KS - 1];
    half8 Ah[2], Al[2];
    auto load_b = [&](int dx, half8 (&dst)[R + KS - 1]) {
#pragma unroll
        for (int rr = 0; rr < R + KS - 1; ++rr) dst[rr] = ld8(pb + b_lane_off + (rr * C::PW + dx) * 16);
    };
    auto load_a = [&](int s, half8& h, half8& l) {
        const int dx = s / KS, dy = s % KS;
        const int off = ((dy * KS + dx) * 32) * 32 + a_lane_off;
        h = ld8(wb + off);
        if constexpr (HI) l = ld8(wb + C::WP * 1024 + off);
    };
    load_b(0, B[0]);
    load_a(0, Ah[0], Al[0]);
#pragma unroll
    for (int s = 0; s < NTAP; ++s) {
        const int dx = s / KS, dy = s % KS;
        if (s + 1 < NTAP) load_a(s + 1, Ah[(s + 1) & 1], Al[(s + 1) & 1]);
        if (dy == 0 && dx + 1 < KS) load_b(dx + 1, B[(dx + 1) & 1]);
        __builtin_amdgcn_sched_barrier(0);
        if constexpr (HI) {
#pragma unroll
            for (int r = 0; r < R; ++r)
                acc[r] = mfma_32x32x16(Al[s & 1], B[dx & 1][r + dy], acc[r]);
        }
#pragma unroll
        for (int r = 0; r < R; ++r)
            acc[r] = mfma_32x32x16(Ah[s & 1], B[dx & 1][r + dy], acc[r]);
        __builtin_amdgcn_sched_barrier(0);
    }
}

template <class C, int KS, int R, bool HI>
__device__ __forceinline__ void x3_compute_pair(const char* pb, const char* wb, int n, int kg, int wave, floatx16 (&acc)[R]) {
    static_assert(KS & 1, "odd kernels");
    constexpr int NP = KS / 2;
    const int s16 = ((n >> 3) & 1) << 4;
    const int a_pair = n * 32 + s16 + kg * (KS * 1024);
    const int a_plain = n * 32 + ((kg << 4) ^ s16);
    const int b_pair = ((wave * R + kg) * C::PW + n) * 16;
    const int b_plain = patch_lane_off<C>(n, kg, wave * R);
    half8 Bp[2][R + KS - 3], Bl[2][R];
    half8 Ah[2], Al[2];
    auto load_b = [&](int dx, half8 (&bp)[R + KS - 3], half8 (&bl)[R]) {
#pragma unroll
        for (int rr = 0; rr < R + KS - 3; ++rr) bp[rr] = ld8(pb + b_pair + (rr * C::PW + dx) * 16);
#pragma unroll
        for (int r = 0; r < R; ++r) bl[r] = ld8(pb + b_plain + ((r + KS - 1) * C::PW + dx) * 16);
    };
    auto load_a = [&](int s, half8& h, half8& l) {
        const int dx = s / (NP + 1), j = s % (NP + 1);
        const int off = (j < NP) ? ((2 * j) * KS + dx) * 1024 + a_pair : ((KS - 1) * KS + dx) * 1024 + a_plain;
        h = ld8(wb + off);
        if constexpr (HI) l = ld8(wb + C::WP * 1024 + off);
    };
    constexpr int NS = KS * (NP + 1);
    load_b(0, Bp[0], Bl[0]);
    load_a(0, Ah[0], Al[0]);
#pragma unroll
    for (int s = 0; s < NS; ++s) {
        const int dx = s / (NP + 1), j = s % (NP + 1);
        if (s + 1 < NS) load_a(s + 1, Ah[(s + 1) & 1], Al[(s + 1) & 1]);
        if (j == 0 && dx + 1 < KS) load_b(dx + 1, Bp[(dx + 1) & 1], Bl[(dx + 1) & 1]);
        __builtin_amdgcn_sched_barrier(0);
#pragma unroll
        for (int r = 0; r < R; ++r) {
            const half8 b = (j < NP) ? Bp[dx & 1][r + 2 * j] : Bl[dx & 1][r];
            if constexpr (HI) acc[r] = mfma_32x32x16(Al[s & 1], b, acc[r]);
            acc[r] = mfma_32x32x16(Ah[s & 1], b, acc[r]);
        }
        __builtin_amdgcn_sched_barrier(0);
    }
}

struct X3Gate {
    const unsigned* flags;
    unsigned epoch;
    int chunk;
    unsigned* status;
};
constexpr unsigned RDB3_SPIN_LIMIT = 1u << 22;

template <int KS, int R, int WN, int EPI, bool XTRA, bool GATED = false>
__device__ __forceinline__ void x3_tile(const ConvKArgs& a, const float* __restrict__ bias, char* smem, const ConvTile& t,
                                        const X3Gate gate = X3Gate{nullptr, 0u, 1 << 30, nullptr}) {
    using C = X3Cfg<KS, R, WN>;
    BH_TL_DECL;
    BH_TL_BEGIN();
    const int tid = threadIdx.x;
    const int lane = tid & 63;
    const int wave = __builtin_amdgcn_readfirstlane(tid >> 6);
    const int n = lane & 31;
    const int kg = lane >> 5;
    const int img = t.img, ty = t.ty, tx = t.tx, z = t.z;
    unsigned voff[C::NPJ];
    patch_offsets<C, C::PAD>(voff, t, a.H, a.W, wave, lane);

    floatx16 acc[1][R];
#pragma unroll
    for (int r = 0; r < R; ++r)
#pragma unroll
        for (int e = 0; e < 16; ++e) acc[0][r][e] = 0.f;

    const int nchunks = a.nchunks;
    const int a_lane_off = weight_lane_off(n, kg);
    const int b_lane_off = patch_lane_off<C>(n, kg, wave * R);

    __builtin_amdgcn_s_setprio(2);
    x3_issue_weights<C, KS>(a, smem, 0, 0, wave, lane, z);
    if constexpr (GATED) {
        if (gate.chunk <= 0 && gate.flags) {
            if (tid < 9) {
                const int ny = ty + tid / 3 - 1, nx = tx + tid % 3 - 1;
                if (ny >= 0 && ny < a.tiles_y && nx >= 0 && nx < a.tiles_x) {
                    const unsigned* f = gate.flags + ((size_t)img * a.tiles_y + ny) * a.tiles_x + nx;
                    unsigned spins = 0;
                    while (__hip_atomic_load(f, __ATOMIC_RELAXED, __HIP_MEMORY_SCOPE_AGENT) != gate.epoch) {
                        __builtin_amdgcn_s_sleep(2);
                        if (++spins > RDB3_SPIN_LIMIT) {
                            if (gate.status) atomicOr(gate.status, BINHIP_STATUS_SYNC_TIMEOUT);
                            break;
                        }
                    }
                }
            }
            __builtin_amdgcn_s_barrier();
            __builtin_amdgcn_sched_barrier(0);
        }
    }
    x3_issue_patch<C>(a, smem, 0, 0, 0, wave, voff, t);
    for (int c = 0; c < nchunks; ++c) {
        const char* wb = smem + 2 * C::PATCH_BYTES + (c & 1) * C::WBUF_BYTES;
        if (a.prog_prio) {
            const int q = (4 * c) / nchunks;
            if (q == 0) __builtin_amdgcn_s_setprio(3);
            else if (q == 1) __builtin_amdgcn_s_setprio(2);
            else if (q == 2) __builtin_amdgcn_s_setprio(1);
            else __builtin_amdgcn_s_setprio(0);
        }
        wait_vmcnt<0>();
        __builtin_amdgcn_s_barrier();
        __builtin_amdgcn_sched_barrier(0);
#if BINHIP_TIMELINE
        if (c == 0) BH_TL_STAMP(1);
#endif
        x3_issue_patch<C>(a, smem, c, 1, 1, wave, voff, t);
        if (c + 1 < nchunks) x3_issue_weights<C, KS>(a, smem, c + 1, (c + 1) & 1, wave, lane, z);
        unsigned gate_seen = gate.epoch;
        const unsigned* gate_word = nullptr;
        if constexpr (GATED) {
            if (c + 1 == gate.chunk && gate.flags && tid < 9) {
                const int ny = ty + tid / 3 - 1, nx = tx + tid % 3 - 1;
                if (ny >= 0 && ny < a.tiles_y && nx >= 0 && nx < a.tiles_x) {
                    gate_word = gate.flags + ((size_t)img * a.tiles_y + ny) * a.tiles_x + nx;
                    gate_seen = __hip_atomic_load(gate_word, __ATOMIC_RELAXED, __HIP_MEMORY_SCOPE_AGENT);
                }
            }
        }
        const bool pair = (KS == 5) && !XTRA && a.half_last && (c + 1 == nchunks);
        if constexpr (KS == 5 && !XTRA) {
            if (pair) x3_compute_pair<C, KS, R, true>(smem, wb, n, kg, wave, acc[0]);
            else x3_compute<C, KS, R, true>(smem, wb, a_lane_off, b_lane_off, acc[0]);
        } else {
            x3_compute<C, KS, R, true>(smem, wb, a_lane_off, b_lane_off, acc[0]);
        }
        wait_vmcnt<0>();
        __builtin_amdgcn_s_barrier();
        __builtin_amdgcn_sched_barrier(0);
        if constexpr (GATED) {
            if (c + 1 == gate.chunk && gate.flags) {
                if (gate_word) {
                    unsigned spins = 0;
                    while (gate_seen != gate.epoch) {
                        __builtin_amdgcn_s_sleep(2);
                        gate_seen = __hip_atomic_load(gate_word, __ATOMIC_RELAXED, __HIP_MEMORY_SCOPE_AGENT);
                        if (++spins > RDB3_SPIN_LIMIT) {
                            if (gate.status) atomicOr(gate.status, BINHIP_STATUS_SYNC_TIMEOUT);
                            break;
                        }
                    }
                }
                __builtin_amdgcn_s_barrier();
                __builtin_amdgcn_sched_barrier(0);
            }
        }
        if (c + 1 < nchunks) x3_issue_patch<C>(a, smem, c + 1, 0, 0, wave, voff, t);
        if constexpr (KS == 5 && !XTRA) {
            if (pair) x3_compute_pair<C, KS, R, false>(smem + C::PATCH_BYTES, wb, n, kg, wave, acc[0]);
            else x3_compute<C, KS, R, false>(smem + C::PATCH_BYTES, wb, a_lane_off, b_lane_off, acc[0]);
        } else {
            x3_compute<C, KS, R, false>(smem + C::PATCH_BYTES, wb, a_lane_off, b_lane_off, acc[0]);
        }
    }
    BH_TL_STAMP(2);
    __builtin_amdgcn_s_setprio(0);
    conv_epilogue<1, R, 3, EPI, XTRA>(a, bias, acc, img, t.ty0 + wave * R, t.tx0, z * 32, z == 0, n, kg, t.plane_elems);
    BH_TL_FINISH(a, (((img * a.tiles_y + ty) * a.tiles_x + tx) * a.ncol + z));
}

template <int KS, int R, int WN, int EPI, int WIDE, bool XTRA>
__global__ void __launch_bounds__(64 * WN)
    __attribute__((amdgpu_waves_per_eu((KS == 5 && !XTRA) ? WN / 4 : WN / 2, (KS == 5 && !XTRA) ? WN / 4 : WN / 2)))
conv_x3_kernel(const ConvKArgs a, const float* __restrict__ bias) {
    extern __shared__ __attribute__((aligned(16))) char smem[];
    x3_tile<KS, R, WN, EPI, XTRA>(a, bias, smem, tile_decode<X3Cfg<KS, R, WN>::TH>(a, a.ncol));
}

struct Rdb3Args {
    ConvKArgs conv[3];
    unsigned* flags;
    unsigned epoch;
    int T;
};

template <int R, int WN>
__global__ void __launch_bounds__(64 * WN) __attribute__((amdgpu_waves_per_eu(WN / 2, WN / 2)))
conv_x3_rdbs_kernel(const Rdb3Args a, const float* __restrict__ bias0, const float* __restrict__ bias1,
                    const float* __restrict__ bias2) {
    extern __shared__ __attribute__((aligned(16))) char smem[];
    const int G = (int)gridDim.x;
    const int b = xcd_band((int)blockIdx.x, G);
#pragma unroll 1
    for (int p = 0; p < 3; ++p) {
        const ConvKArgs& ka = a.conv[p];
        const float* bias = p == 0 ? bias0 : (p == 1 ? bias1 : bias2);
        X3Gate gate;
        gate.flags = p > 0 ? a.flags + (size_t)(p - 1) * a.T : nullptr;
        gate.epoch = a.epoch;
        gate.chunk = ka.nchunks - 2;
        gate.status = ka.flags;
#pragma unroll 1
        for (int t0 = b; t0 < a.T; t0 += G) {
            x3_tile<3, R, WN, BINHIP_EPI_PLANES, false, true>(ka, bias, smem, tile_at<R * WN>(ka, t0, 0), gate);
            asm volatile("s_waitcnt vmcnt(0)" ::: "memory");
            __syncthreads();
            if (threadIdx.x == 0 && p < 2)
                __hip_atomic_store(a.flags + (size_t)p * a.T + t0, a.epoch, __ATOMIC_RELAXED, __HIP_MEMORY_SCOPE_AGENT);
        }
    }
}

template <int KS, int R, int WN, int EPI, int WIDE, bool XTRA>
static int launch_x3_x(const ConvKArgs& ka, int cout_pad, hipStream_t s) {
    using C = X3Cfg<KS, R, WN>;
    static std::atomic<unsigned long long> lds_set{0};
    if (int rc = bh_set_max_lds(&conv_x3_kernel<KS, R, WN, EPI, WIDE, XTRA>, C::LDS_BYTES, lds_set)) return rc;
    ConvKArgs a = ka;
    const dim3 grid(set_tiles<C>(a, cout_pad / 32));
    a.prog_prio = (KS == 3 && !XTRA && (long long)grid.x <= 2ll * binhip_device_cus()) ? 1 : 0;
#if BINHIP_TIMELINE
    a.tl = bh_tl_reserve(grid.x, &a.tl_base);
    a.tl_launch = ((KS == 3 && EPI == BINHIP_EPI_PLANES && WIDE == 0 && !XTRA ? 1u : 3u) << 24) | (g_bh_tl_serial.fetch_add(1) & 0xFFFFFFu);
#endif
    conv_x3_kernel<KS, R, WN, EPI, WIDE, XTRA><<<grid, dim3(64 * C::NW), C::LDS_BYTES, s>>>(a, a.bias);
    BH_CHECK_LAUNCH();
    return 0;
}
template <int KS, int R, int WN, int EPI, int WIDE>
static int launch_x3(const ConvKArgs& ka, int cout_pad, hipStream_t s) {
    if constexpr (EPI == BINHIP_EPI_PLANES) {
        if (ka.has_res || ka.r2_hi || ka.m_hi || ka.y_unshuf) return launch_x3_x<KS, R, WN, EPI, WIDE, true>(ka, cout_pad, s);
    }
    return launch_x3_x<KS, R, WN, EPI, WIDE, false>(ka, cout_pad, s);
}

int bh_launch_rdb3_x3(const ConvKArgs* convs, unsigned* flags, unsigned epoch, int cus, hipStream_t s) {
    using C = X3Cfg<3, X3_R, X3_WN>;
    static std::atomic<unsigned long long> lds_set{0};
    static std::atomic<int> per_cu{-1};
    if (int rc = bh_set_max_lds(&conv_x3_rdbs_kernel<X3_R, X3_WN>, C::LDS_BYTES, lds_set)) return rc;
    int occ = per_cu.load(std::memory_order_acquire);
    if (occ < 0) {
        int n = 0;
        hipError_t e = hipOccupancyMaxActiveBlocksPerMultiprocessor(&n, conv_x3_rdbs_kernel<X3_R, X3_WN>, 64 * C::NW,
                                                                    C::LDS_BYTES);
        if (e != hipSuccess) return (int)e;
        occ = n > 2 ? 2 : n;
        per_cu.store(occ, std::memory_order_release);
    }
    if (occ < 1) return BINHIP_E_SHAPE;
    Rdb3Args a;
    for (int p = 0; p < 3; ++p) {
        a.conv[p] = convs[p];
        set_tiles<C>(a.conv[p]);
        if (!a.conv[p].wt || a.conv[p].nchunks < 3) return BINHIP_E_SHAPE;
#if BINHIP_TIMELINE
        a.conv[p].tl = bh_tl_reserve((unsigned)(a.conv[p].tiles_x * a.conv[p].tiles_y * a.conv[p].N), &a.conv[p].tl_base);
        a.conv[p].tl_launch = ((4u + p) << 24) | (g_bh_tl_serial.load() & 0xFFFFFFu);
#endif
    }
#if BINHIP_TIMELINE
    g_bh_tl_serial.fetch_add(1);
#endif
    a.T = a.conv[0].tiles_x * a.conv[0].tiles_y * a.conv[0].N;
    a.flags = flags; a.epoch = epoch;
    const long long slots = (long long)occ * (cus > 0 ? cus : 256);
    const unsigned grid = (unsigned)(a.T < slots ? a.T : slots);
    for (int p = 0; p < 3; ++p) a.conv[p].prog_prio = (a.T <= slots) ? 1 : 0;
    conv_x3_rdbs_kernel<X3_R, X3_WN><<<dim3(grid), dim3(64 * C::NW), C::LDS_BYTES, s>>>(a, a.conv[0].bias, a.conv[1].bias,
                                                                                                   a.conv[2].bias);
    BH_CHECK_LAUNCH();
    return 0;
}

__global__ void __launch_bounds__(256)
final_dot2_kernel(const ConvKArgs a, const unsigned* __restrict__ w_hi32) {
    using C = X3Cfg<3, 2, 4>;
    extern __shared__ __attribute__((aligned(16))) char smem[];
    const int tid = threadIdx.x;
    const int lane = tid & 63;
    const int wave = __builtin_amdgcn_readfirstlane(tid >> 6);
    const ConvTile t = tile_decode<C::TH>(a, 1);
    const int img = t.img, tx0 = t.tx0, ty0 = t.ty0;
    const int H = a.H, W = a.W;
    unsigned voff[C::NPJ];
    patch_offsets<C, C::PAD>(voff, t, H, W, wave, lane);
    const int px = lane & 31, py = 2 * wave + (lane >> 5);
    const int base_off = (py * C::PW + px) * 16;
    float acc[3] = {0.f, 0.f, 0.f};
    typedef _Float16 half2v __attribute__((ext_vector_type(2)));
    union X8 { half8 h; half2v p[4]; };
    union W2 { unsigned u; half2v p; };

    const int nchunks = a.nchunks;
    auto compute = [&](const char* pb, int c) {
        const unsigned* wh = w_hi32 + (long long)c * (9 * 32 * 8);
#pragma unroll
        for (int t = 0; t < 9; ++t) {
            const int dy = t / 3, dx = t % 3;
#pragma unroll
            for (int cg = 0; cg < 2; ++cg) {
                X8 x;
                x.h = *reinterpret_cast<const half8*>(pb + cg * (C::PH * C::PW * 16) + base_off + (dy * C::PW + dx) * 16);
#pragma unroll
                for (int r = 0; r < 3; ++r) {
#pragma unroll
                    for (int k = 0; k < 4; ++k) {
                        W2 w;
                        w.u = wh[(t * 32 + r) * 8 + cg * 4 + k];
                        acc[r] = __builtin_amdgcn_fdot2(x.p[k], w.p, acc[r], false);
                    }
                }
            }
        }
    };

    x3_issue_patch<C>(a, smem, 0, 0, 0, wave, voff, t);
    for (int c = 0; c < nchunks; ++c) {
        wait_vmcnt<0>();
        __builtin_amdgcn_s_barrier();
        __builtin_amdgcn_sched_barrier(0);
        if (c + 1 < nchunks) x3_issue_patch<C>(a, smem, c + 1, 0, (c + 1) & 1, wave, voff, t);
        compute(smem + (c & 1) * C::PATCH_BYTES, c);
    }
    const int gy = ty0 + py, gx = tx0 + px;
    if (gy < H && gx < W) {
        float sum[3], bj[3];
        const int nimg = a.nimg;
#pragma unroll
        for (int j = 0; j < 3; ++j) {
            const long long idx = (((long long)img * a.cout + (j < a.cout ? j : 0)) * H + gy) * W + gx;
            float v[5];
#pragma unroll
            for (int t = 0; t < 5; ++t) v[t] = (t < nimg) ? a.img[t][idx] : 0.f;
            bj[j] = a.bias[j < a.cout ? j : 0];
            float sj = v[0];
#pragma unroll
            for (int t = 1; t < 5; ++t)
                if (t < nimg) sj += v[t];
            sum[j] = nimg > 0 ? sj / (float)nimg : 0.f;
        }
#pragma unroll
        for (int j = 0; j < 3; ++j) asm volatile("" : "+v"(sum[j]), "+v"(bj[j]));
        __builtin_amdgcn_sched_barrier(0);
#pragma unroll
        for (int j = 0; j < 3; ++j) {
            if (j >= a.cout) break;
            const long long idx = (((long long)img * a.cout + j) * H + gy) * W + gx;
            a.out_f32[idx] = (acc[j] + bj[j]) + sum[j];
        }
    }
}

struct M16 {
    using C = X3Cfg<3, 2, 8>;
    static constexpr int NSTAGE = 3;
    static constexpr int WPIECES = 5;
    static constexpr int W_OFF = NSTAGE * C::PATCH_BYTES;
    static constexpr int LDS_BYTES = W_OFF + 2 * WPIECES * 1024;
    static_assert(2 * LDS_BYTES <= 160 * 1024, "two workgroups per CU");
};

template <bool HI>
__device__ __forceinline__ void m16_compute(const char* pb, const char* wb, int a_lane_off, int b_lane_off, int slot, int a_zero,
                                            floatx4 (&acc)[2][2]) {
    using C = X3Cfg<3, 2, 8>;
    half8 Ah[2], Al[2], B[2][2][2];
    auto tap_off = [](int t) { return ((t / 3) * C::PW + (t % 3)) * 16; };
    auto load = [&](int p, half8& ah, half8& al, half8 (&b)[2][2]) {
        const int aoff = (p < 4) ? (2 * p + slot) * 128 + a_lane_off : (slot ? 8 * 128 + a_zero : 8 * 128 + a_lane_off);
        ah = ld8(wb + aoff);
        if constexpr (HI) al = ld8(wb + M16::WPIECES * 1024 + aoff);
        const int boff = b_lane_off + tap_off(2 * p) + slot * (p < 4 ? tap_off(2 * p + 1) - tap_off(2 * p) : 0);
#pragma unroll
        for (int r = 0; r < 2; ++r)
#pragma unroll
            for (int g = 0; g < 2; ++g) b[r][g] = ld8(pb + boff + (r * C::PW + g * 16) * 16);
    };
    load(0, Ah[0], Al[0], B[0]);
#pragma unroll
    for (int p = 0; p < 5; ++p) {
        if (p + 1 < 5) load(p + 1, Ah[(p + 1) & 1], Al[(p + 1) & 1], B[(p + 1) & 1]);
        __builtin_amdgcn_sched_barrier(0);
#pragma unroll
        for (int r = 0; r < 2; ++r)
#pragma unroll
            for (int g = 0; g < 2; ++g) {
                if constexpr (HI) acc[r][g] = __builtin_amdgcn_mfma_f32_16x16x32_f16(Al[p & 1], B[p & 1][r][g], acc[r][g], 0, 0, 0);
                acc[r][g] = __builtin_amdgcn_mfma_f32_16x16x32_f16(Ah[p & 1], B[p & 1][r][g], acc[r][g], 0, 0, 0);
            }
        __builtin_amdgcn_sched_barrier(0);
    }
}

__global__ void __launch_bounds__(512) __attribute__((amdgpu_waves_per_eu(4, 4)))
final_m16_kernel(const ConvKArgs a, const float* __restrict__ bias) {
    using C = X3Cfg<3, 2, 8>;
    extern __shared__ __attribute__((aligned(16))) char smem[];
    const int tid = threadIdx.x;
    const int lane = tid & 63;
    const int wave = __builtin_amdgcn_readfirstlane(tid >> 6);
    const ConvTile t = tile_decode<C::TH>(a, 1);
    const int img = t.img, tx0 = t.tx0, ty0 = t.ty0;
    const int H = a.H, W = a.W;
    unsigned voff[C::NPJ];
    patch_offsets<C, C::PAD>(voff, t, H, W, wave, lane);
    const int n16 = lane & 15, kb = lane >> 4;
    const int slot = kb >> 1;
    const int a_lane_off = ((n16 < 3 ? n16 : 3) * 2 + (kb & 1)) * 16;
    const int a_zero = (3 * 2 + (kb & 1)) * 16;
    const int b_lane_off = ((kb & 1) * (C::PH * C::PW) + wave * 2 * C::PW + n16) * 16;
    floatx4 acc[2][2];
#pragma unroll
    for (int r = 0; r < 2; ++r)
#pragma unroll
        for (int g = 0; g < 2; ++g) acc[r][g] = floatx4{0.f, 0.f, 0.f, 0.f};

    const int nchunks = a.nchunks;
    const int nstage = 2 * nchunks;
    {
        const int ntaps = nchunks * 9;
        for (int i = wave; i < 2 * M16::WPIECES; i += C::NW) {
            const int pl = i >= M16::WPIECES ? 1 : 0;
            const int t = (i - pl * M16::WPIECES) * 8 + (lane >> 3);
            __amdgpu_buffer_rsrc_t rs = __builtin_amdgcn_make_buffer_rsrc((void*)(pl ? a.w_lo : a.w_hi), 0, (unsigned)(ntaps * 1024), 0x00020000);
            const unsigned off = t < ntaps ? (unsigned)(t * 1024 + (lane & 7) * 16) : 0x80000000u;
            __builtin_amdgcn_raw_ptr_buffer_load_lds(rs, (lds_void_t*)(smem + M16::W_OFF + i * 1024), 16, off, 0, 0, 0);
        }
    }
    x3_issue_patch<C>(a, smem, 0, 0, 0, wave, voff, t);
    if (nstage > 1) x3_issue_patch<C>(a, smem, 0, 1, 1, wave, voff, t);
    const bool three = wave < (C::PP - 2 * C::NW);
    for (int s = 0; s < nstage; ++s) {
        if (s + 1 < nstage) {
            if (three) wait_vmcnt<3>(); else wait_vmcnt<2>();
        } else {
            wait_vmcnt<0>();
        }
        __builtin_amdgcn_s_barrier();
        __builtin_amdgcn_sched_barrier(0);
        if (s + 2 < nstage) x3_issue_patch<C>(a, smem, (s + 2) >> 1, (s + 2) & 1, (s + 2) % 3, wave, voff, t);
        const char* pb = smem + (s % 3) * C::PATCH_BYTES;
        const char* wb = smem + M16::W_OFF + (s >> 1) * (9 * 128);
        if (s & 1) m16_compute<false>(pb, wb, a_lane_off, b_lane_off, slot, a_zero, acc);
        else m16_compute<true>(pb, wb, a_lane_off, b_lane_off, slot, a_zero, acc);
    }
    if (kb == 0) {
        float sum[2][2][3];
        const int nimg = a.nimg;
#pragma unroll
        for (int r = 0; r < 2; ++r)
#pragma unroll
            for (int g = 0; g < 2; ++g) {
                const int gy = ty0 + wave * 2 + r, gx = tx0 + g * 16 + n16;
                const bool ok = gy < H && gx < W;
                const int gyc = gy < H ? gy : H - 1, gxc = gx < W ? gx : W - 1;
#pragma unroll
                for (int j = 0; j < 3; ++j) {
                    const long long idx = (((long long)img * a.cout + (j < a.cout ? j : 0)) * H + gyc) * W + gxc;
                    float v[5];
#pragma unroll
                    for (int t = 0; t < 5; ++t) v[t] = (t < nimg) ? a.img[t][idx] : 0.f;
                    float sj = v[0];
#pragma unroll
                    for (int t = 1; t < 5; ++t)
                        if (t < nimg) sj += v[t];
                    sum[r][g][j] = (ok && nimg > 0) ? sj / (float)nimg : 0.f;
                }
            }
        float bj[3];
#pragma unroll
        for (int j = 0; j < 3; ++j) bj[j] = bias[j < a.cout ? j : 0];
#pragma unroll
        for (int r = 0; r < 2; ++r)
#pragma unroll
            for (int g = 0; g < 2; ++g)
#pragma unroll
                for (int j = 0; j < 3; ++j) asm volatile("" : "+v"(sum[r][g][j]));
#pragma unroll
        for (int j = 0; j < 3; ++j) asm volatile("" : "+v"(bj[j]));
        __builtin_amdgcn_sched_barrier(0);
#pragma unroll
        for (int r = 0; r < 2; ++r)
#pragma unroll
            for (int g = 0; g < 2; ++g) {
                const int gy = ty0 + wave * 2 + r, gx = tx0 + g * 16 + n16;
                if (gy >= H || gx >= W) continue;
#pragma unroll
                for (int j = 0; j < 3; ++j) {
                    if (j >= a.cout) break;
                    const long long idx = (((long long)img * a.cout + j) * H + gy) * W + gx;
                    a.out_f32[idx] = (acc[r][g][j] + bj[j]) + sum[r][g][j];
                }
            }
    }
}

int bh_launch_final_m16(const ConvKArgs& ka, hipStream_t s) {
    using C = X3Cfg<3, 2, 8>;
    static std::atomic<unsigned long long> lds_set{0};
    if (ka.nchunks * 9 > M16::WPIECES * 8) return BINHIP_E_SHAPE;
    if (int rc = bh_set_max_lds(&final_m16_kernel, M16::LDS_BYTES, lds_set)) return rc;
    ConvKArgs a = ka;
    final_m16_kernel<<<dim3(set_tiles<C>(a)), dim3(512), M16::LDS_BYTES, s>>>(a, a.bias);
    BH_CHECK_LAUNCH();
    return 0;
}

int bh_launch_final_dot2(const ConvKArgs& ka, hipStream_t s) {
    using C = X3Cfg<3, 2, 4>;
    ConvKArgs a = ka;
    const dim3 grid(set_tiles<C>(a));
    final_dot2_kernel<<<grid, dim3(256), 2 * C::PATCH_BYTES, s>>>(a, reinterpret_cast<const unsigned*>(a.w_hi));
    BH_CHECK_LAUNCH();
    return 0;
}

int bh_launch_conv_x3_k5(const ConvKArgs& a, int cout_pad, hipStream_t s) {
    return launch_x3<5, X3_R, X3_WN, BINHIP_EPI_PLANES, 1>(a, cout_pad, s);
}

int bh_launch_conv_x3_k5_subpix(const ConvKArgs& a, hipStream_t s) {
    return launch_x3<5, X3_R, X3_WN, BINHIP_EPI_FINAL_SUBPIX, 0>(a, 32, s);
}

struct RingArgs {
    const _Float16* x_hi;
    const _Float16* x_lo;
    const float* wvar;
    const float* bvar;
    float* out;
    const float* img[5];
    int N, H, W, cin, nimg;
};
constexpr int RING_THREADS = 128;
__global__ void __launch_bounds__(RING_THREADS) upnet_ring_kernel(const RingArgs a) {
    __shared__ float red[3][RING_THREADS / 64];
    const int tid = threadIdx.x, lane = tid & 63, wave = tid >> 6;
    const int H = a.H, W = a.W, H2 = 2 * H, W2 = 2 * W;
    const int ring = 2 * W2 + 2 * (H2 - 2);
    int id = blockIdx.x;
    const int img = id / ring;
    id -= img * ring;
    int Y, X;
    if (id < W2) { Y = 0; X = id; }
    else if (id < 2 * W2) { Y = H2 - 1; X = id - W2; }
    else { const int k = id - 2 * W2; Y = 1 + (k >> 1); X = (k & 1) ? W2 - 1 : 0; }
    const int y = Y >> 1, i = Y & 1, x = X >> 1, j = X & 1;
    const int vy = (Y == 0) ? 0 : (Y == H2 - 1 ? 2 : 1), vx = (X == 0) ? 0 : (X == W2 - 1 ? 2 : 1);
    const int var = 3 * vy + vx, sub = 2 * i + j;
    const int cin = a.cin, ng = cin >> 3, items = 25 * ng;
    const long long wstride = (long long)25 * cin;
    const float* w = a.wvar + ((long long)var * 12 + sub) * wstride;
    float s0 = 0.f, s1 = 0.f, s2 = 0.f;
    for (int it = tid; it < items; it += RING_THREADS) {
        const int tap = it / ng, ci = (it - tap * ng) << 3;
        const int yy = y + tap / 5 - 2, xx = x + tap % 5 - 2;
        if (yy < 0 || yy >= H || xx < 0 || xx >= W) continue;
        const long long o = (((((long long)(ci >> 4) * a.N + img) * H + yy) * W + xx) << 4) + (ci & 15);
        const half8 xh = *reinterpret_cast<const half8*>(a.x_hi + o);
        half8 xl;
        if (a.x_lo) xl = *reinterpret_cast<const half8*>(a.x_lo + o);
        const float* wq = w + (long long)tap * cin + ci;
        floatx4 wa[3][2];
#pragma unroll
        for (int c = 0; c < 3; ++c) {
            wa[c][0] = *reinterpret_cast<const floatx4*>(wq + 4 * c * wstride);
            wa[c][1] = *reinterpret_cast<const floatx4*>(wq + 4 * c * wstride + 4);
        }
#pragma unroll
        for (int e = 0; e < 8; ++e) {
            float v = (float)xh[e];
            if (a.x_lo) v += (float)xl[e];
            s0 = fmaf(wa[0][e >> 2][e & 3], v, s0);
            s1 = fmaf(wa[1][e >> 2][e & 3], v, s1);
            s2 = fmaf(wa[2][e >> 2][e & 3], v, s2);
        }
    }
#pragma unroll
    for (int off = 32; off > 0; off >>= 1) {
        s0 += __shfl_xor(s0, off);
        s1 += __shfl_xor(s1, off);
        s2 += __shfl_xor(s2, off);
    }
    if (lane == 0) { red[0][wave] = s0; red[1][wave] = s1; red[2][wave] = s2; }
    __syncthreads();
    if (tid < 3) {
        const int c = tid;
        const float v = red[c][0] + red[c][1];
        const long long idx = (((long long)img * 3 + c) * H2 + Y) * W2 + X;
        float m = 0.f;
        if (a.nimg > 0) {
            m = a.img[0][idx];
            for (int t = 1; t < a.nimg; ++t) m += a.img[t][idx];
            m = m / (float)a.nimg;
        }
        a.out[idx] = (v + a.bvar[var * 12 + 4 * c + sub]) + m;
    }
}
int bh_launch_upnet_ring(const void* x_hi, const void* x_lo, const float* wvar, const float* bvar, float* out, const float* const* images,
                         int nimg, int N, int H, int W, int cin, hipStream_t s) {
    if (!x_hi || !wvar || !bvar || !out || N <= 0 || H <= 0 || W <= 0 || cin <= 0 || (cin & 15) || nimg < 0 || nimg > 5) return BINHIP_E_ARG;
    RingArgs a;
    a.x_hi = (const _Float16*)x_hi; a.x_lo = (const _Float16*)x_lo; a.wvar = wvar; a.bvar = bvar; a.out = out;
    for (int t = 0; t < 5; ++t) a.img[t] = (t < nimg) ? images[t] : nullptr;
    a.N = N; a.H = H; a.W = W; a.cin = cin; a.nimg = nimg;
    const long long ring = 4ll * W + 4ll * H - 4;
    upnet_ring_kernel<<<dim3((unsigned)(ring * N)), dim3(RING_THREADS), 0, s>>>(a);
    BH_CHECK_LAUNCH();
    return 0;
}

int bh_launch_conv_x3(const ConvKArgs& a, int cout_pad, int epilogue, hipStream_t s) {
    if (epilogue == BINHIP_EPI_PLANES)
        return cout_pad == 32 ? launch_x3<3, X3_R, X3_WN, BINHIP_EPI_PLANES, 0>(a, cout_pad, s)
                              : launch_x3<3, X3_R, X3_WN, BINHIP_EPI_PLANES, 1>(a, cout_pad, s);
    if (epilogue == BINHIP_EPI_SHUFFLE) return launch_x3<3, X3_R, X3_WN, BINHIP_EPI_SHUFFLE, 1>(a, cout_pad, s);
    if (epilogue == BINHIP_EPI_FINAL) return launch_x3<3, X3_R, X3_WN, BINHIP_EPI_FINAL, 0>(a, cout_pad, s);
    return BINHIP_E_SHAPE;
}
```

### bin_amd/csrc/binhip_plan.hip

```cpp
#include "binhip_conv_common.h"

namespace {

struct Shp {
    int G0, D, C, G;
    int c0, cg, cb;
    int L;
    bool stage4;
};
bool resolve_shape(const BinRdnShape* s, Shp* o) {
    Shp h;
    const bool dflt = !s || (s->G0 == 0 && s->D == 0 && s->C == 0 && s->G == 0);
    h.G0 = dflt ? 96 : s->G0; h.D = dflt ? 12 : s->D; h.C = dflt ? 4 : s->C; h.G = dflt ? 32 : s->G;
    if (h.G0 < 32 || h.G0 > 256 || h.G0 % 32 || h.G < 32 || h.G > 128 || h.G % 32) return false;
    if (h.C < 1 || h.C > BINHIP_RDN_MAX_CONVS || h.D < 1 || h.D > 20) return false;
    h.c0 = h.G0 / 16; h.cg = h.G / 16; h.cb = h.c0 + h.C * h.cg;
    h.L = 2 + h.D * (h.C + 1) + 4;
    if (h.L > BINHIP_RDN_MAX_LAYERS) return false;
    h.stage4 = (h.G0 == 96 && h.C == 4 && h.G == 32);
    *o = h;
    return true;
}
inline int layer_conv(const Shp& sh, int d, int c) { return 2 + d * (sh.C + 1) + c; }

bool frames_ok(int N, int H, int W, int n_inputs) {
    return N > 0 && H > 0 && W > 0 && !(H & 1) && !(W & 1) && (n_inputs == 2 || n_inputs == 3 || n_inputs == 5);
}

struct Planes {
    int64_t off = -1, size = 0;
    bool present() const { return off >= 0; }
    Planes sub(int64_t elems) const { return {off + elems, size}; }
};
struct Bind {
    _Float16* base;
    bool has_lo;
    Bind(const void* p, bool lo) : base((_Float16*)(((uintptr_t)p + 255) & ~(uintptr_t)255)), has_lo(lo) {}
    void* hi(Planes t) const { return t.present() ? base + t.off : nullptr; }
    void* lo(Planes t) const { return t.present() && has_lo ? base + t.off + t.size : nullptr; }
};
struct Carve {
    int64_t next; int mul;
    Planes take(int64_t size) { const Planes t{next, size}; next += mul * size; return t; }
};

struct Ws {
    int64_t P, PF;
    int kc0;
    Planes x0, f1, blk, g0, g1, u;
    int64_t sync, total;
    int tiles;
};

Ws make_ws(int N, int H, int W, int nin, int nt, const Shp& sh) {
    Ws w;
    const int h = H / 2, ww = W / 2;
    w.P = (int64_t)N * h * ww * 16; w.PF = (int64_t)N * H * W * 16;
    w.kc0 = (12 * nin + 15) / 16;
    Carve o{0, nt == 3 ? 2 : 1};
    w.x0 = o.take(w.kc0 * w.P); w.f1 = o.take(sh.c0 * w.P);
    w.blk = o.take((int64_t)(sh.D + 1) * sh.cb * w.P);
    w.g0 = o.take(sh.c0 * w.P); w.g1 = o.take(sh.c0 * w.P);
    w.u = o.take(4 * w.PF);
    w.tiles = N * ((h + 15) / 16) * ((ww + 31) / 32);
    w.sync = (o.next + 127) & ~(int64_t)127;
    w.total = w.sync + 2 * (32 + 2 * (int64_t)w.tiles);
    return w;
}

struct Conv {
    int layer, ks = 3, cin_chunks, cout, cout_pad = 0;
    int epi = BINHIP_EPI_PLANES, relu = 0, H = 0, W = 0;
    Planes x;
    int x_cpg = 0;
    int64_t x_group_stride = 0;
    Planes y, res;
};

}

extern "C" {

size_t binhip_rdn_workspace_bytes(int N, int H, int W, int n_inputs, int nterms, const BinRdnShape* shape) {
    Shp sh;
    if (!frames_ok(N, H, W, n_inputs) || !resolve_shape(shape, &sh)) return 0;
    return (size_t)make_ws(N, H, W, n_inputs, nterms, sh).total * 2 + 256;
}

int binhip_rdn_workspace_layout(int N, int H, int W, int n_inputs, int nterms, const BinRdnShape* shape, int64_t* out, int n_out) {
    if (!out || n_out < BINHIP_RDN_LAYOUT_WORDS) return BINHIP_E_ARG;
    Shp sh;
    if (!frames_ok(N, H, W, n_inputs) || !resolve_shape(shape, &sh)) return BINHIP_E_SHAPE;
    const Ws w = make_ws(N, H, W, n_inputs, nterms, sh);
    const Planes t[6] = {w.x0, w.f1, w.blk, w.g0, w.g1, w.u};
    out[0] = w.P; out[1] = w.PF; out[2] = w.kc0; out[15] = nterms == 3 ? 1 : 0;
    for (int i = 0; i < 6; ++i) { out[3 + 2 * i] = t[i].off; out[4 + 2 * i] = t[i].size; }
    return 0;
}

int binhip_rdn_forward(const BinRdnPlan* p, const float* const* inputs, float* out, void* workspace, size_t workspace_bytes, void* stream) {
    if (!p || !inputs || !out || !workspace) return BINHIP_E_ARG;
    const int N = p->N, H = p->H, W = p->W, nin = p->n_inputs, nt = p->nterms;
    if (!frames_ok(N, H, W, nin)) return BINHIP_E_SHAPE;
    if (nt != 1 && nt != 3) return BINHIP_E_ARG;
    Shp sh;
    if (!resolve_shape(&p->shape, &sh)) return BINHIP_E_SHAPE;
    const size_t need = binhip_rdn_workspace_bytes(N, H, W, nin, nt, &p->shape);
    if (workspace_bytes < need) return BINHIP_E_WORKSPACE;
    for (int i = 0; i < nin; ++i) if (!inputs[i]) return BINHIP_E_ARG;
    for (int i = 0; i < sh.L; ++i) if (!p->w_hi[i] || !p->bias[i] || (nt == 3 && !p->w_lo[i])) return BINHIP_E_ARG;

    hipStream_t s = (hipStream_t)stream;
    const Ws w = make_ws(N, H, W, nin, nt, sh);
    const int h = H / 2, ww = W / 2;
    const Bind A(workspace, nt == 3);

    int rc = binhip_pack_inputs(inputs, nin, N, H, W, A.hi(w.x0), A.lo(w.x0), p->status, stream);
    if (rc) return rc;

    auto mk = [&](const Conv& l) -> BhConvCall {
        BhConvCall c;
        c.d.N = N; c.d.H = l.H ? l.H : h; c.d.W = l.W ? l.W : ww; c.d.ksize = l.ks; c.d.cin_chunks = l.cin_chunks; c.d.cout = l.cout;
        c.d.cout_pad = l.cout_pad ? l.cout_pad : l.cout; c.d.nterms = nt; c.d.epilogue = l.epi; c.d.relu = l.relu;
        c.d.x_cpg = l.x_cpg; c.d.x_group_stride = l.x_group_stride; c.d.status = p->status;
        if (l.ks == 1 && l.epi == BINHIP_EPI_PLANES && c.d.W > 32 && c.d.W % 32 == 0) { c.d.H *= c.d.W / 32; c.d.W = 32; }
        if (l.layer == 0 && l.ks == 5 && (12 * nin) % 16 >= 1 && (12 * nin) % 16 <= 8) c.d.reserved = BINHIP_CONV_HALF_LAST_CHUNK;
        c.x_hi = A.hi(l.x); c.x_lo = A.lo(l.x);
        c.w_hi = p->w_hi[l.layer]; c.w_lo = p->w_lo[l.layer]; c.bias = p->bias[l.layer];
        c.r_hi = A.hi(l.res); c.r_lo = A.lo(l.res);
        c.y_hi = A.hi(l.y); c.y_lo = A.lo(l.y);
        c.status = p->status; c.prof = p->profiler;
        if (l.epi == BINHIP_EPI_FINAL || l.epi == BINHIP_EPI_FINAL_SUBPIX) {
            c.y_f32 = out; c.d.n_images = nin;
            for (int i = 0; i < nin; ++i) c.images[i] = inputs[i];
        }
        return c;
    };
    auto conv = [&](const Conv& l) -> int { return bh_launch_conv(mk(l), s); };
    const bool rdb3 = (p->reserved & BINHIP_PLAN_RDB3) && nt == 3 && sh.stage4;
    unsigned* sync_words = (unsigned*)(A.base + w.sync);
    const int cus = binhip_device_cus();
    if (rdb3) {
        hipError_t me = hipMemsetAsync(sync_words, 0, (size_t)(32 + 2 * (size_t)w.tiles) * 4, s);
        if (me != hipSuccess) return (int)me;
    }
    const int64_t P = w.P;
    const int G0 = sh.G0, G = sh.G, C = sh.C, D = sh.D, c0 = sh.c0, cg = sh.cg, cb = sh.cb;
    if ((rc = conv({.layer = 0, .ks = 5, .cin_chunks = w.kc0, .cout = G0, .x = w.x0, .y = w.f1}))) return rc;
    if ((rc = conv({.layer = 1, .cin_chunks = c0, .cout = G0, .x = w.f1, .y = w.blk}))) return rc;
    for (int d = 0; d < D; ++d) {
        const Planes b = w.blk.sub((int64_t)d * cb * P), b_next = b.sub(cb * P);
        auto dense = [&](int c) -> Conv {
            return {.layer = layer_conv(sh, d, c), .cin_chunks = c0 + cg * c, .cout = G, .relu = 1, .x = b, .y = b.sub((c0 + cg * c) * P)};
        };
        const bool fuse = sh.stage4 && !(p->reserved & BINHIP_PLAN_NO_FUSE);
        bool done3 = false;
        if (rdb3 && fuse) {
            ConvKArgs ka[3];
            bool ok3 = true;
            for (int c = 0; c < 3 && ok3; ++c) {
                if ((rc = bh_prepare_conv(mk(dense(c)), &ka[c]))) return rc;
                ok3 = ok3 && ka[c].wt;
            }
            if (ok3) {
                rc = bh_launch_rdb3_x3(ka, sync_words + 32, (unsigned)(d + 1), cus, s);
                if (rc == 0) done3 = true;
                else if (rc != BINHIP_E_SHAPE) return rc;
            }
        }
        for (int c = 0; c < (fuse ? C - 1 : C) && !done3; ++c) if ((rc = conv(dense(c)))) return rc;
        if (fuse) {
            const int L3 = layer_conv(sh, d, 3), LF = layer_conv(sh, d, 4);
            if ((rc = binhip_rdb_tail_fwd(N, h, ww, nt, A.hi(b), A.lo(b), p->w_hi[L3], p->w_lo[L3], p->bias[L3], p->w_hi[LF], p->w_lo[LF], p->bias[LF],
                                          A.hi(b_next), A.lo(b_next), (p->reserved & BINHIP_PLAN_KEEP_ACTS) ? 1 : 0, p->status, stream)))
                return rc;
        } else if ((rc = conv({.layer = layer_conv(sh, d, C), .ks = 1, .cin_chunks = cb, .cout = G0, .x = b, .y = b_next, .res = b})))
            return rc;
    }
    const int LG = sh.L - 4;
    if ((rc = conv({.layer = LG, .ks = 1, .cin_chunks = D * c0, .cout = G0, .x = w.blk.sub(cb * P), .x_cpg = c0, .x_group_stride = cb * P, .y = w.g0})))
        return rc;
    if ((rc = conv({.layer = LG + 1, .cin_chunks = c0, .cout = G0, .x = w.g0, .y = w.g1, .res = w.f1}))) return rc;
    const bool fused_up = (p->reserved & BINHIP_PLAN_FUSED_UPNET) &&
                          (!(p->reserved & BINHIP_PLAN_KEEP_ACTS) || (p->reserved & BINHIP_PLAN_FUSED_UPNET_TRAIN)) &&
                          sh.L + 1 < BINHIP_RDN_MAX_LAYERS && p->w_hi[sh.L] && (nt == 1 || p->w_lo[sh.L]) && p->bias[sh.L] &&
                          p->w_hi[sh.L + 1] && p->bias[sh.L + 1];
    if (fused_up) {
        if ((rc = conv({.layer = sh.L, .ks = 5, .cin_chunks = c0, .cout = 12, .cout_pad = 32, .epi = BINHIP_EPI_FINAL_SUBPIX, .x = w.g1})))
            return rc;
        return bh_launch_upnet_ring(A.hi(w.g1), A.lo(w.g1), (const float*)p->w_hi[sh.L + 1], p->bias[sh.L + 1], out, inputs, nin, N, h, ww,
                                    G0, s);
    }
    if ((rc = conv({.layer = LG + 2, .cin_chunks = c0, .cout = 256, .epi = BINHIP_EPI_SHUFFLE, .x = w.g1, .y = w.u}))) return rc;
    return conv({.layer = LG + 3, .cin_chunks = 4, .cout = 3, .cout_pad = 32, .epi = BINHIP_EPI_FINAL, .H = H, .W = W, .x = w.u});
}

}

namespace {

struct Bws {
    int64_t P, PF;
    int kc0, gx0_chunks;
    Planes gout, gu, guu, gg1, gg0, gf1, gy, gcat, gcat2, gx0;
    size_t wg_bytes, sc_off_bytes, wg_off_bytes, total_bytes;
};

Bws make_bws(int N, int H, int W, int nin, int nt, const Shp& sh) {
    Bws b;
    const int h = H / 2, w = W / 2;
    b.P = (int64_t)N * h * w * 16; b.PF = (int64_t)N * H * W * 16;
    b.kc0 = (12 * nin + 15) / 16; b.gx0_chunks = ((12 * nin + 31) / 32) * 2;
    Carve o{0, nt == 3 ? 2 : 1};
    b.gout = o.take(b.PF);
    b.gu = o.take(4 * b.PF);
    b.guu = o.take(16 * b.P);
    b.gg1 = o.take(sh.c0 * b.P); b.gg0 = o.take(sh.c0 * b.P); b.gf1 = o.take(sh.c0 * b.P);
    b.gy = o.take((int64_t)(sh.D + 1) * sh.c0 * b.P); b.gcat = o.take((int64_t)sh.cb * b.P);
    b.gcat2 = o.take((int64_t)sh.cb * b.P); b.gx0 = o.take((int64_t)b.gx0_chunks * b.P);
    size_t wg = 0;
    auto mx = [&](size_t v) { if (v > wg) wg = v; };
    mx(binhip_wgrad_workspace_bytes(3, N, H, W, 4, 3));
    mx(binhip_wgrad_workspace_bytes(3, N, h, w, sh.c0, 256));
    mx(binhip_wgrad_workspace_bytes(3, N, h, w, sh.c0, sh.G0));
    mx(binhip_wgrad_workspace_bytes(1, N, h, w, sh.D * sh.c0, sh.G0));
    mx(binhip_wgrad_workspace_bytes(1, N, h, w, sh.cb, sh.G0));
    for (int c = 0; c < sh.C; ++c) mx(binhip_wgrad_workspace_bytes(3, N, h, w, sh.c0 + sh.cg * c, sh.G));
    mx(binhip_wgrad_workspace_bytes(5, N, h, w, b.kc0, sh.G0));
    b.wg_bytes = wg;
    size_t bytes = ((size_t)o.next * 2 + 255) & ~(size_t)255;
    b.sc_off_bytes = bytes; bytes += 8192;
    b.wg_off_bytes = bytes; bytes += (size_t)(sh.C + 1) * wg;
    b.total_bytes = bytes + 256;
    return b;
}

struct Wgrad {
    int layer, ks = 3, H = 0, W = 0;
    int cin_chunks, cin, cout;
    Planes x;
    int x_cpg = 0;
    int64_t x_group_stride = 0;
    Planes gy;
    int shuffle = 0;
    int slot = -1;
};
struct Dgrad {
    int layer, ks = 3, H = 0, W = 0;
    int gy_chunks, cout;
    Planes gy, y, res;
    int res_chunks = 0;
    bool acc_inplace = false;
    Planes mask;
    int mask_from = 0, y_cpg = 0;
    int64_t y_group_stride = 0;
    int y_unshuf = 0;
};

}

extern "C" {

size_t binhip_rdn_backward_workspace_bytes(int N, int H, int W, int n_inputs, int nterms, const BinRdnShape* shape) {
    Shp sh;
    if (!frames_ok(N, H, W, n_inputs) || !resolve_shape(shape, &sh)) return 0;
    return make_bws(N, H, W, n_inputs, nterms, sh).total_bytes;
}

int binhip_rdn_backward_workspace_layout(int N, int H, int W, int n_inputs, int nterms, const BinRdnShape* shape, int64_t* out, int n_out) {
    if (!out || n_out < BINHIP_RDN_BWD_LAYOUT_WORDS) return BINHIP_E_ARG;
    Shp sh;
    if (!frames_ok(N, H, W, n_inputs) || !resolve_shape(shape, &sh)) return BINHIP_E_SHAPE;
    const Bws b = make_bws(N, H, W, n_inputs, nterms, sh);
    const Planes t[10] = {b.gout, b.gu, b.guu, b.gg1, b.gg0, b.gf1, b.gy, b.gcat, b.gcat2, b.gx0};
    out[0] = b.P; out[1] = b.PF; out[2] = b.gx0_chunks; out[23] = (int64_t)b.sc_off_bytes;
    for (int i = 0; i < 10; ++i) { out[3 + 2 * i] = t[i].off; out[4 + 2 * i] = t[i].size; }
    return 0;
}

int binhip_rdn_backward(const BinRdnBwdPlan* p, const void* saved, size_t saved_bytes, const float* gout, void* workspace,
                        size_t workspace_bytes, void* stream) {
    if (!p || !saved || !gout || !workspace || !p->zero_bias) return BINHIP_E_ARG;
    const int N = p->N, H = p->H, W = p->W, nin = p->n_inputs, nt = p->nterms;
    if (!frames_ok(N, H, W, nin)) return BINHIP_E_SHAPE;
    if (nt != 1 && nt != 3) return BINHIP_E_ARG;
    const int nt_saved = (p->reserved & BINHIP_BWD_SAVED_X3) ? 3 : nt;
    if (nt == 3 && (p->reserved & BINHIP_BWD_SAVED_X3)) return BINHIP_E_ARG;
    Shp sh;
    if (!resolve_shape(&p->shape, &sh)) return BINHIP_E_SHAPE;
    if (saved_bytes < binhip_rdn_workspace_bytes(N, H, W, nin, nt_saved, &p->shape)) return BINHIP_E_WORKSPACE;
    const Bws b = make_bws(N, H, W, nin, nt, sh);
    if (workspace_bytes < b.total_bytes) return BINHIP_E_WORKSPACE;
    for (int i = 0; i < sh.L; ++i) if (!p->wt_hi[i] || (nt == 3 && !p->wt_lo[i]) || !p->dw[i] || !p->db[i]) return BINHIP_E_ARG;
    const int G0 = sh.G0, G = sh.G, C = sh.C, D = sh.D, c0 = sh.c0, cg = sh.cg, cb = sh.cb, LG = sh.L - 4;

    hipStream_t s = (hipStream_t)stream;
    hipStream_t sb = p->aux_stream ? (hipStream_t)p->aux_stream : s;
    const bool two = (sb != s);
    auto order = [&](hipStream_t from, hipStream_t to) -> int {
        if (!two) return 0;
        hipEvent_t e;
        hipError_t r = hipEventCreateWithFlags(&e, hipEventDisableTiming);
        if (r != hipSuccess) return (int)r;
        r = hipEventRecord(e, from);
        if (r == hipSuccess) r = hipStreamWaitEvent(to, e, 0);
        (void)hipEventDestroy(e);
        return r == hipSuccess ? 0 : (int)r;
    };
    const Ws w = make_ws(N, H, W, nin, nt_saved, sh);
    const int h = H / 2, ww = W / 2;
    const int64_t P = w.P;
    const Bind S(saved, nt == 3);
    const Bind Gw(workspace, nt == 3);
    char* wbytes = (char*)Gw.base;
    float* sc = (float*)(wbytes + b.sc_off_bytes);
    float* amax_part = sc + 16;
    void* wgws = wbytes + b.wg_off_bytes;
    const float* inv = sc + 1;

    const int accumulate = (p->reserved & BINHIP_BWD_ACCUMULATE) ? 1 : 0;
    int rc;
    if ((rc = binhip_grad_scale(gout, (int64_t)N * 3 * H * W, 16.f, amax_part, sc, stream))) return rc;
    const bool fused_up = (p->reserved & BINHIP_BWD_FUSED_UPNET) != 0;
    const Planes gsub = {b.gout.off, P};
    if (fused_up) {
        if (sh.L + 1 >= BINHIP_RDN_MAX_LAYERS || !p->wt_hi[sh.L] || (nt == 3 && !p->wt_lo[sh.L]) || !p->wt_hi[sh.L + 1] || !p->dw[sh.L] ||
            !p->db[sh.L] || !p->dw[sh.L + 1] || !p->db[sh.L + 1]) return BINHIP_E_ARG;
        if ((rc = bh_upnet_gsub(gout, N, h, ww, sc, Gw.hi(gsub), Gw.lo(gsub), p->status, s))) return rc;
    } else if ((rc = binhip_nchw_to_planes_scaled(gout, N, 3, H, W, sc, Gw.hi(b.gout), Gw.lo(b.gout), p->status, stream))) return rc;

    BhWgradReduce pending[BH_WGRAD_BATCH];
    int npending = 0;
    auto wgrad = [&](const Wgrad& g) -> int {
        BinConvDesc d = {};
        d.N = N; d.H = g.H ? g.H : h; d.W = g.W ? g.W : ww; d.ksize = g.ks; d.cin_chunks = g.cin_chunks; d.cout = g.cout;
        d.nterms = nt; d.x_cpg = g.x_cpg; d.x_group_stride = g.x_group_stride; d.status = p->status;
        if (int rf = order(s, sb)) return rf;
        BhWgradReduce r;
        char* region = (char*)wgws + (size_t)(g.slot < 0 ? 0 : g.slot) * b.wg_bytes;
        const bool timed = bh_prof_begin(p->profiler, g.ks, g.cout, BINHIP_PROF_WGRAD, sb);
        const int rw = bh_wgrad_partials(&d, S.hi(g.x), S.lo(g.x), Gw.hi(g.gy), Gw.lo(g.gy), region, b.wg_bytes, p->dw[g.layer],
                                         p->db[g.layer], g.cin, g.shuffle, &r, (void*)sb);
        if (timed) bh_prof_end(p->profiler, sb);
        if (rw) return rw;
        if (g.slot < 0) return bh_wgrad_reduce_batch(&r, 1, inv, g.layer >= sh.L ? 0 : accumulate, (void*)sb);
        pending[npending++] = r;
        return 0;
    };
    auto flush_reduces = [&]() -> int {
        const int rr = bh_wgrad_reduce_batch(pending, npending, inv, accumulate, (void*)sb);
        npending = 0;
        return rr;
    };
    auto dgrad = [&](const Dgrad& g) -> int {
        BhConvCall c;
        c.d.N = N; c.d.H = g.H ? g.H : h; c.d.W = g.W ? g.W : ww; c.d.ksize = g.ks; c.d.cin_chunks = g.gy_chunks; c.d.cout = g.cout;
        c.d.cout_pad = binhip_dgrad_rows_pad(g.ks, g.cout); c.d.nterms = nt; c.d.epilogue = BINHIP_EPI_PLANES; c.d.status = p->status;
        c.x_hi = Gw.hi(g.gy); c.x_lo = Gw.lo(g.gy);
        c.w_hi = p->wt_hi[g.layer]; c.w_lo = p->wt_lo[g.layer]; c.bias = p->zero_bias;
        c.r_hi = Gw.hi(g.res); c.r_lo = Gw.lo(g.res); c.res_chunks = g.res_chunks;
        c.y_hi = Gw.hi(g.y); c.y_lo = Gw.lo(g.y);
        if (g.acc_inplace) { c.r2_hi = c.y_hi; c.r2_lo = c.y_lo; }
        c.m_hi = S.hi(g.mask); c.mask_from = g.mask_from;
        c.y_cpg = g.y_cpg; c.y_group_stride = g.y_group_stride; c.y_unshuf = g.y_unshuf;
        c.status = p->status;
        return bh_launch_conv(c, s);
    };

    hipEvent_t b_done[20] = {};
    auto chain = [&]() -> int {
        if (fused_up) {
            if ((rc = wgrad({.layer = sh.L, .ks = 5, .cin_chunks = c0, .cin = G0, .cout = 12, .x = w.g1, .gy = gsub}))) return rc;
            if ((rc = order(s, sb))) return rc;
            if ((rc = bh_upnet_ring_wgrad(gout, S.hi(w.g1), S.lo(w.g1), p->dw[sh.L + 1], p->db[sh.L + 1], N, h, ww, G0, 0, sb))) return rc;
            if ((rc = dgrad({.layer = sh.L, .ks = 5, .gy_chunks = 1, .cout = G0, .gy = gsub, .y = b.gg1}))) return rc;
            if ((rc = bh_upnet_ring_dgrad(gout, (const float*)p->wt_hi[sh.L + 1], sc, Gw.hi(b.gg1), Gw.lo(b.gg1), p->status, N, h, ww, G0, s))) return rc;
        } else {
            if ((rc = wgrad({.layer = LG + 3, .H = H, .W = W, .cin_chunks = 4, .cin = 64, .cout = 3, .x = w.u, .gy = b.gout}))) return rc;
            if ((rc = dgrad({.layer = LG + 3, .H = H, .W = W, .gy_chunks = 1, .cout = 64, .gy = b.gout, .y = b.guu, .y_unshuf = 4}))) return rc;
            if ((rc = wgrad({.layer = LG + 2, .cin_chunks = c0, .cin = G0, .cout = 256, .x = w.g1, .gy = b.guu, .shuffle = 1}))) return rc;
            if ((rc = dgrad({.layer = LG + 2, .gy_chunks = 16, .cout = G0, .gy = b.guu, .y = b.gg1}))) return rc;
        }
        if ((rc = wgrad({.layer = LG + 1, .cin_chunks = c0, .cin = G0, .cout = G0, .x = w.g0, .gy = b.gg1}))) return rc;
        if ((rc = dgrad({.layer = LG + 1, .gy_chunks = c0, .cout = G0, .gy = b.gg1, .y = b.gg0}))) return rc;
        if ((rc = wgrad({.layer = LG, .ks = 1, .cin_chunks = D * c0, .cin = D * G0, .cout = G0, .x = w.blk.sub(cb * P), .x_cpg = c0,
                         .x_group_stride = cb * P, .gy = b.gg0}))) return rc;
        if ((rc = dgrad({.layer = LG, .ks = 1, .gy_chunks = c0, .cout = D * G0, .gy = b.gg0, .y = b.gy.sub(c0 * P), .y_cpg = c0,
                         .y_group_stride = c0 * P}))) return rc;
        for (int d = D - 1; d >= 0; --d) {
            const Planes blk = w.blk.sub((int64_t)d * cb * P);
            const Planes gy = b.gy.sub((int64_t)(d + 1) * c0 * P);
            const Planes gcat = (d & 1) ? b.gcat2 : b.gcat;
            const int L = layer_conv(sh, d, 0);
            if ((rc = wgrad({.layer = L + C, .ks = 1, .cin_chunks = cb, .cin = G0 + C * G, .cout = G0, .x = blk, .gy = gy, .slot = C}))) return rc;
            if (two && d + 2 <= D - 1 && b_done[d + 2]) {
                hipError_t r = hipStreamWaitEvent(s, b_done[d + 2], 0);
                (void)hipEventDestroy(b_done[d + 2]);
                b_done[d + 2] = nullptr;
                if (r != hipSuccess) return (int)r;
            }
            if ((rc = dgrad({.layer = L + C, .ks = 1, .gy_chunks = c0, .cout = G0 + C * G, .gy = gy, .y = gcat, .res = gy, .res_chunks = c0,
                             .mask = blk, .mask_from = c0 + cg * (C - 1)}))) return rc;
            for (int c = C - 1; c >= 0; --c) {
                const Planes gyc = gcat.sub((c0 + cg * c) * P);
                if ((rc = wgrad({.layer = L + c, .cin_chunks = c0 + cg * c, .cin = G0 + G * c, .cout = G, .x = blk, .gy = gyc, .slot = c})))
                    return rc;
                if (c > 0) {
                    const Planes slot = gcat.sub((c0 + cg * (c - 1)) * P);
                    if ((rc = dgrad({.layer = L + c, .gy_chunks = cg * (C - c), .cout = G, .gy = gyc, .y = slot, .res = slot,
                                     .mask = blk.sub((c0 + cg * (c - 1)) * P)}))) return rc;
                } else {
                    if ((rc = dgrad({.layer = L, .gy_chunks = cg * C, .cout = G0, .gy = gyc, .y = b.gy.sub((int64_t)d * c0 * P), .res = gcat,
                                     .acc_inplace = d >= 1}))) return rc;
                }
            }
            if ((rc = flush_reduces())) return rc;
            if (two) {
                hipError_t r = hipEventCreateWithFlags(&b_done[d], hipEventDisableTiming);
                if (r == hipSuccess) r = hipEventRecord(b_done[d], sb);
                if (r != hipSuccess) return (int)r;
            }
        }
        if ((rc = wgrad({.layer = 1, .cin_chunks = c0, .cin = G0, .cout = G0, .x = w.f1, .gy = b.gy}))) return rc;
        if ((rc = dgrad({.layer = 1, .gy_chunks = c0, .cout = G0, .gy = b.gy, .y = b.gf1, .res = b.gg1}))) return rc;
        if ((rc = wgrad({.layer = 0, .ks = 5, .cin_chunks = w.kc0, .cin = 12 * nin, .cout = G0, .x = w.x0, .gy = b.gf1}))) return rc;
        bool need_in = false;
        for (int i = 0; i < nin; ++i) need_in = need_in || (p->gin[i] != nullptr);
        if (need_in) {
            if ((rc = dgrad({.layer = 0, .ks = 5, .gy_chunks = c0, .cout = 12 * nin, .gy = b.gf1, .y = b.gx0}))) return rc;
            if ((rc = binhip_unpack_input_grads(Gw.hi(b.gx0), Gw.lo(b.gx0), gout, sc, nin, N, H, W, p->gin, stream))) return rc;
        }
        return 0;
    };
    rc = chain();
    for (int d = 0; d < 20; ++d) if (b_done[d]) (void)hipEventDestroy(b_done[d]);
    const int rj = order(sb, s);
    return rc ? rc : rj;
}

}
```

### bin_amd/rdn_plan.py

```python
import ctypes as C

import torch

from . import _lib as L
from .ops import ConvWeights, _ptr, _stream, _need_cuda, on_device, relayout_batch, relayout_item, status_word

STAGE4_SHAPE = (96, 12, 4, 32)


def check_shape(shape):
    G0, D, C, G = (int(v) for v in shape)
    if G0 % 32 or not 32 <= G0 <= 256 or G % 32 or not 32 <= G <= 128 or not 1 <= C <= L.RDN_MAX_CONVS or not 1 <= D <= 20 \
            or 2 + D * (C + 1) + 4 > L.RDN_MAX_LAYERS:
        raise NotImplementedError(
            f"bin_amd RDN: unsupported configuration G0={G0}, D={D}, C={C}, G={G} (built: G0 and G multiples of 32 with "
            f"32 <= G0 <= 256, G <= 128; 1 <= C <= {L.RDN_MAX_CONVS}; 1 <= D <= 20)")
    return G0, D, C, G


def c_shape(shape):
    s = L.BinRdnShape()
    s.G0, s.D, s.C, s.G = shape
    return s


def layer_names(shape=STAGE4_SHAPE):
    _, D, C, _ = shape
    names = ["SFENet1", "SFENet2"]
    for d in range(D):
        names += [f"RDBs.{d}.convs.{c}.conv.0" for c in range(C)]
        names.append(f"RDBs.{d}.LFF")
    names += ["GFF.0", "GFF.1", "UPNet.0", "UPNet.2"]
    return names


def fused_upnet_weights(w0, b0, w2, b2):
    w0, b0, w2, b2 = (t.double() for t in (w0, b0, w2, b2))
    dev, g0 = w0.device, w0.shape[1]
    assert w0.shape == (256, g0, 3, 3) and w2.shape == (3, 64, 3, 3) and b0.shape == (256,) and b2.shape == (3,)
    sub = torch.tensor([[1, 0, 1], [0, 1, 0]], device=dev)
    off = torch.tensor([[-1, 0, 0], [0, 0, 1]], device=dev)
    w0r = w0.view(64, 2, 2, g0, 3, 3)
    w0g = w0r[:, sub.reshape(-1)].view(64, 2, 3, 2, g0, 3, 3)
    w0g = w0g[:, :, :, sub.reshape(-1)].view(64, 2, 3, 2, 3, g0, 3, 3)
    b0g = b0.view(64, 2, 2)[:, sub.reshape(-1)].view(64, 2, 3, 2)[:, :, :, sub.reshape(-1)].view(64, 2, 3, 2, 3)
    T = torch.einsum("ckyx,kiyjxgab->ciyjxgab", w2, w0g)
    Tb = torch.einsum("ckyx,kiyjx->ciyjx", w2, b0g)
    place = torch.zeros(2, 3, 3, 5, dtype=torch.float64, device=dev)
    for i in range(2):
        for dy in range(3):
            for a in range(3):
                place[i, dy, a, int(off[i, dy]) + 1 + a] = 1.0
    keep = torch.ones(3, 2, 3, dtype=torch.float64, device=dev)
    keep[0, 0, 0] = 0.0
    keep[2, 1, 2] = 0.0
    W = torch.einsum("ciyjxgab,viy,wjx,iyat,jxbu->vwcijgtu", T, keep, keep, place, place).reshape(9, 12, g0, 5, 5)
    B = (b2.view(1, 1, 3, 1, 1) + torch.einsum("ciyjx,viy,wjx->vwcij", Tb, keep, keep)).reshape(9, 12)
    return W, B


_FUSED_MAPS = {}


def _fused_upnet_maps(device):
    key = str(device)
    if key in _FUSED_MAPS:
        return _FUSED_MAPS[key]
    import numpy as np
    tap = -np.ones((2, 2, 5, 3), dtype=np.int64)
    sub = np.zeros((2, 3), dtype=np.int64)
    for i in range(2):
        for dy in range(3):
            oy, ip = divmod(i + dy - 1, 2)
            sub[i, dy] = ip
            for a in range(3):
                tap[i, ip, oy + 1 + a, a] = dy
    keep = np.ones((3, 2, 3), dtype=bool)
    keep[0, 0, 0] = False
    keep[2, 1, 2] = False
    sh = (3, 3, 3, 2, 2, 5, 5, 64, 2, 2, 3, 3)
    ax = {n: k for k, n in enumerate(("vy", "vx", "c", "i", "j", "t", "u", "k", "ip", "jp", "a", "b"))}

    def bc(arr, names):
        shape = [1] * len(sh)
        for d, nme in zip(arr.shape, names):
            shape[ax[nme]] = d
        order = sorted(range(len(names)), key=lambda q: ax[names[q]])
        return np.transpose(arr, order).reshape(shape)
    dy = bc(tap, ("i", "ip", "t", "a"))
    dx = bc(tap, ("j", "jp", "u", "b"))
    ok = (dy >= 0) & (dx >= 0)
    vy = np.arange(3).reshape(bc(np.arange(3), ("vy",)).shape)
    vx = np.arange(3).reshape(bc(np.arange(3), ("vx",)).shape)
    ii = np.arange(2).reshape(bc(np.arange(2), ("i",)).shape)
    jj = np.arange(2).reshape(bc(np.arange(2), ("j",)).shape)
    valid = ok & keep[vy, ii, np.where(dy >= 0, dy, 0)] & keep[vx, jj, np.where(dx >= 0, dx, 0)]
    cc = np.arange(3).reshape(bc(np.arange(3), ("c",)).shape)
    kk = np.arange(64).reshape(bc(np.arange(64), ("k",)).shape)
    flat = ((cc * 64 + kk) * 3 + np.where(dy >= 0, dy, 0)) * 3 + np.where(dx >= 0, dx, 0)
    idx = np.where(np.broadcast_to(valid, sh), np.broadcast_to(flat, sh), 3 * 64 * 9).reshape(-1)
    nA, nW = idx.size, 3 * 64 * 9
    order = np.argsort(idx, kind="stable")
    srt = idx[order]
    counts = np.bincount(srt, minlength=nW + 1)
    starts = np.concatenate(([0], np.cumsum(counts)[:-1]))
    rank = np.arange(nA) - starts[srt]
    lmax = int(counts[:nW].max())
    inv = np.full((nW, lmax), nA, dtype=np.int64)
    real = srt < nW
    inv[srt[real], rank[real]] = order[real]
    maps = {"idx": torch.from_numpy(idx.astype(np.int32)).to(device), "inv": torch.from_numpy(inv.astype(np.int32)).to(device),
            "sub": torch.from_numpy(sub).to(device), "keep": torch.from_numpy(keep.astype(np.float32)).to(device)}
    _FUSED_MAPS[key] = maps
    return maps


class _GatherW2(torch.autograd.Function):

    @staticmethod
    def forward(ctx, w2, idx, inv):
        ctx.save_for_backward(inv)
        ctx.shape = w2.shape
        return torch.cat((w2.reshape(-1), w2.new_zeros(1))).index_select(0, idx)

    @staticmethod
    def backward(ctx, gA):
        inv, = ctx.saved_tensors
        ge = torch.cat((gA.reshape(-1), gA.new_zeros(1)))
        return ge.index_select(0, inv.reshape(-1)).view(inv.shape).sum(1).view(ctx.shape), None, None


def fused_upnet_operator(w0, b0, w2, b2):
    m = _fused_upnet_maps(w0.device)
    g0 = w0.shape[1]
    A = _GatherW2.apply(w2, m["idx"], m["inv"]).view(9 * 12 * 25, 64 * 2 * 2 * 9)
    w0p = w0.view(64, 2, 2, g0, 3, 3).permute(0, 1, 2, 4, 5, 3).reshape(64 * 2 * 2 * 9, g0)
    W = (A @ w0p).view(9, 12, 25, g0)
    sub, keep = m["sub"], m["keep"].to(w0.dtype)
    tb = torch.einsum("ckyx,kpq->cyxpq", w2, b0.view(64, 2, 2))
    tg = tb[:, :, :, sub.reshape(-1)].view(3, 3, 3, 2, 3, 2)
    tg = torch.diagonal(tg, dim1=1, dim2=4)
    tg = tg[:, :, :, sub.reshape(-1)].reshape(3, 3, 2, 2, 3, 3)
    tg = torch.diagonal(tg, dim1=1, dim2=4)
    B = b2.view(1, 1, 3, 1, 1) + torch.einsum("cijyx,viy,wjx->vwcij", tg, keep, keep)
    return W, B.reshape(9, 12)


def fused_upnet_reference(x, W, B):
    import torch.nn.functional as F
    x = x.double()
    out = F.pixel_shuffle(F.conv2d(x, W[4], B[4], padding=2), 2)
    h2, w2 = out.shape[-2:]
    for vy in range(3):
        for vx in range(3):
            if vy == 1 and vx == 1:
                continue
            full = F.pixel_shuffle(F.conv2d(x, W[3 * vy + vx], B[3 * vy + vx], padding=2), 2)
            ys = {0: slice(0, 1), 1: slice(1, h2 - 1), 2: slice(h2 - 1, h2)}[vy]
            xs = {0: slice(0, 1), 1: slice(1, w2 - 1), 2: slice(w2 - 1, w2)}[vx]
            out[..., ys, xs] = full[..., ys, xs]
    return out


class RdnWeights:

    def __init__(self, params, n_inputs, nterms, prefix="", shape=STAGE4_SHAPE):
        self.n_inputs, self.nterms, self.shape = n_inputs, nterms, check_shape(shape)
        self.layers = []
        items = []
        for i, nm in enumerate(layer_names(self.shape)):
            w, b = params[f"{prefix}{nm}.weight"], params[f"{prefix}{nm}.bias"]
            shuffle = nm == "UPNet.0"
            cin_chunks = None
            if nm == "SFENet1":
                cin_chunks = (12 * n_inputs + 15) // 16
            self.layers.append(ConvWeights(w, b, nterms=nterms, shuffle=shuffle, cin_chunks=cin_chunks, defer=items))
        assert len(self.layers) == 2 + self.shape[1] * (self.shape[2] + 1) + 4
        relayout_batch(items)

        self._dgrad = None
        w0, _, w2, _ = src = tuple(params[f"{prefix}UPNet.{k}.{t}"] for k in (0, 2) for t in ("weight", "bias"))
        fusable = tuple(w0.shape[2:]) == (3, 3) and w0.shape[0] == 256 and tuple(w2.shape) == (3, 64, 3, 3)
        self._up_src = src if fusable else None
        self.fused_up = None
        self.fused_w4 = None
        self.fused_train = None
        self.fused_train_w4 = None
        self.fused_graph = None

    def ensure_fused_upnet(self, train=False):
        if self._up_src is None:
            return None
        if train:
            if self.fused_train is None:
                with torch.enable_grad():
                    leaves = [t.detach().float().requires_grad_() for t in self._up_src]
                    Wr, Br = fused_upnet_operator(*leaves)
                self.fused_graph = (leaves, Wr, Br)
                with torch.no_grad():
                    g0 = Wr.shape[3]
                    self.fused_train_w4 = Wr[4].permute(0, 2, 1).reshape(12, g0, 5, 5).contiguous()
                    main = ConvWeights(self.fused_train_w4, Br[4].detach().contiguous(), nterms=self.nterms)
                    self.fused_train = (main, Wr.detach().contiguous(), Br.detach().contiguous())
            return self.fused_train
        if self.fused_up is None:
            with torch.no_grad():
                W, B = fused_upnet_weights(*self._up_src)
                self.fused_w4 = W[4].float().contiguous()
                main = ConvWeights(self.fused_w4, B[4].float().contiguous(), nterms=self.nterms)
                ring_w = W.permute(0, 1, 3, 4, 2).reshape(9, 12, 25, W.shape[2]).float().contiguous()
                self.fused_up = (main, ring_w, B.float().contiguous())
        return self.fused_up

    def fill_plan(self, plan, fused=None):
        plan.shape = c_shape(self.shape)
        for i, cw in enumerate(self.layers):
            plan.w_hi[i] = cw.w_hi.data_ptr()
            plan.w_lo[i] = cw.w_lo.data_ptr() if cw.w_lo is not None else None
            plan.bias[i] = cw.bias.data_ptr()
        n = len(self.layers)
        if fused is not None:
            main, ring_w, ring_b = fused
            plan.w_hi[n], plan.bias[n] = main.w_hi.data_ptr(), main.bias.data_ptr()
            plan.w_lo[n] = main.w_lo.data_ptr() if main.w_lo is not None else None
            plan.w_hi[n + 1], plan.w_lo[n + 1], plan.bias[n + 1] = ring_w.data_ptr(), None, ring_b.data_ptr()

    def dgrad(self, module, nterms=None, fused=False):
        nterms = self.nterms if nterms is None else nterms
        if self._dgrad is None:
            self._dgrad = {}
        key = (nterms, bool(fused))
        if key not in self._dgrad:
            if fused and self.fused_train is None:
                raise RuntimeError("bin_amd: backward of a fused-UPNet forward on weights that never built the training operands")
            with torch.no_grad():
                self._dgrad[key] = RdnDgradWeights(dict(module.named_parameters()), self.n_inputs, nterms, shape=self.shape,
                                                   fused=(self.fused_train_w4, self.fused_train[1]) if fused else None)
        return self._dgrad[key]


class RdnDgradWeights:

    def __init__(self, params, n_inputs, nterms, prefix="", shape=STAGE4_SHAPE, fused=None):
        lib = L.lib()
        self.shape = G0, D, C, G = check_shape(shape)
        self.w_hi, self.w_lo = [], []
        self.fused_ring_w = None
        dev = None
        names = layer_names(self.shape)
        fp32 = {nm: params[f"{prefix}{nm}.weight"].detach().contiguous().float() for nm in names}

        def alloc(rows, chunks, ks):
            nbytes = lib.binhip_weights_bytes(rows, chunks, ks)
            hi = torch.empty(nbytes // 2, dtype=torch.float16, device=dev)
            lo = torch.empty(nbytes // 2, dtype=torch.float16, device=dev) if nterms == 3 else None
            return hi, lo, torch.empty(rows, dtype=torch.float32, device=dev)

        items, scratch = [], []
        self._src = fp32
        for nm in names:
            w = fp32[nm]
            dev = w.device
            cout, cin, ks, _ = w.shape
            if ".convs." in nm:
                d, g = int(nm.split(".")[1]), int(nm.split(".")[3])
                rows, chunks = (G0 if g == 0 else G), (C - g) * G // 16
                hi, lo, zb = alloc(rows, chunks, 3)
                srcs = [fp32[f"RDBs.{d}.convs.{c}.conv.0"] for c in range(C)]
                cb = lib.binhip_conv_cout_block(3, rows, nterms)
                items.append(relayout_item(L.RELAYOUT_RDB_GATHER, srcs, None, hi, lo, zb, G, G0 + G * g, 3, rows, chunks, cb, g,
                                           shape=self.shape))
            else:
                rows_pad = lib.binhip_dgrad_rows_pad(ks, cin)
                cin_chunks = (cout + 15) // 16
                cb = lib.binhip_conv_cout_block(ks, rows_pad, nterms)
                hi, lo, zb = alloc(rows_pad, cin_chunks, ks)
                items.append(relayout_item(L.RELAYOUT_DGRAD, [w], None, hi, lo, zb, cout, cin, ks, rows_pad, cin_chunks, cb,
                                           1 if nm == "UPNet.0" else 0))
            self.w_hi.append(hi)
            self.w_lo.append(lo)
            scratch.append(zb)
        if fused is not None:
            w4, self.fused_ring_w = fused
            rows_pad = lib.binhip_dgrad_rows_pad(5, G0)
            cb = lib.binhip_conv_cout_block(5, rows_pad, nterms)
            hi, lo, zb = alloc(rows_pad, 1, 5)
            items.append(relayout_item(L.RELAYOUT_DGRAD, [w4], None, hi, lo, zb, 12, G0, 5, rows_pad, 1, cb, 0))
            self.w_hi.append(hi)
            self.w_lo.append(lo)
            scratch.append(zb)
        relayout_batch(items)
        del scratch
        self.zero_bias = torch.zeros(max(D * G0, G0 + C * G, 256, 1152), dtype=torch.float32, device=dev)

    def fill_plan(self, plan):
        plan.shape = c_shape(self.shape)
        for i in range(len(self.w_hi)):
            plan.wt_hi[i] = self.w_hi[i].data_ptr()
            plan.wt_lo[i] = self.w_lo[i].data_ptr() if self.w_lo[i] is not None else None
        if self.fused_ring_w is not None:
            plan.wt_hi[len(self.w_hi)] = self.fused_ring_w.data_ptr()
        plan.zero_bias = self.zero_bias.data_ptr()


from collections import OrderedDict as _OrderedDict

_workspaces = _OrderedDict()
WORKSPACE_CACHE_ENTRIES = 12


def workspace(nbytes, device, key="fwd"):
    stream = torch.cuda.current_stream(device)
    if torch.cuda.is_current_stream_capturing():
        return torch.empty(nbytes, dtype=torch.uint8, device=device)
    key = (device.type, device.index, stream.cuda_stream, key)
    ws = _workspaces.get(key)
    if ws is None or ws.numel() < nbytes:
        ws = torch.empty(nbytes, dtype=torch.uint8, device=device)
        _workspaces[key] = ws
        while len(_workspaces) > WORKSPACE_CACHE_ENTRIES:
            _workspaces.popitem(last=False)
    _workspaces.move_to_end(key)
    return ws


def release_workspaces(stream=None):
    if stream is None:
        _workspaces.clear()
        return
    for k in [k for k in _workspaces if k[2] == stream.cuda_stream and k[1] == stream.device.index]:
        del _workspaces[k]


import os as _os


def default_plan_flags():
    flags = L.PLAN_RDB3 if _os.environ.get("BIN_AMD_RDB3", "0") == "1" else 0
    if _os.environ.get("BIN_AMD_FUSED_UPNET", "1") != "0":
        flags |= L.PLAN_FUSED_UPNET
    return flags


def rdn_forward(weights, inputs, out=None, ws=None, flags=0, profiler=None):
    _need_cuda(*inputs)
    with on_device(inputs[0]):
        return _rdn_forward(weights, inputs, out, ws, flags, profiler)


def _rdn_forward(weights, inputs, out, ws, flags, profiler):
    inputs = [t.contiguous().float() for t in inputs]
    n, c, h, w = inputs[0].shape
    assert c == 3 and len(inputs) == weights.n_inputs
    lib = L.lib()
    plan = L.BinRdnPlan()
    plan.N, plan.H, plan.W, plan.n_inputs, plan.nterms = n, h, w, weights.n_inputs, weights.nterms
    plan.reserved = int(flags or 0)
    plan.status = status_word(inputs[0].device).data_ptr()
    plan.profiler = profiler if profiler else None
    fused = None
    if plan.reserved & L.PLAN_FUSED_UPNET:
        if plan.reserved & L.PLAN_FUSED_UPNET_TRAIN:
            fused = weights.ensure_fused_upnet(train=True)
        elif not (plan.reserved & L.PLAN_KEEP_ACTS):
            fused = weights.ensure_fused_upnet()
    weights.fill_plan(plan, fused)
    nbytes = lib.binhip_rdn_workspace_bytes(n, h, w, weights.n_inputs, weights.nterms, C.byref(plan.shape))
    if nbytes == 0:
        raise RuntimeError(f"bin_amd: unsupported RDN shape N={n} H={h} W={w} (H, W must be even)")
    if ws is None:
        ws = workspace(nbytes, inputs[0].device)
    if out is None:
        out = torch.empty((n, 3, h, w), dtype=torch.float32, device=inputs[0].device)
    arr = (C.c_void_p * len(inputs))(*[t.data_ptr() for t in inputs])
    L.check(lib.binhip_rdn_forward(C.byref(plan), arr, _ptr(out), _ptr(ws), ws.numel(), _stream()), "rdn_forward")
    return out
```

### include/binhip.h

```cpp
#ifndef BINHIP_H
#define BINHIP_H

#include <stddef.h>
#include <stdint.h>

#ifdef __cplusplus
extern "C" {
#endif

#define BINHIP_API __attribute__((visibility("default")))

#define BINHIP_VERSION 622
#define BINHIP_ABI_EXPORTS 51

#define BINHIP_E_ARG      (-1)
#define BINHIP_E_SHAPE    (-2)
#define BINHIP_E_WORKSPACE (-3)

#define BINHIP_STATUS_SATURATED 1u
#define BINHIP_STATUS_SYNC_TIMEOUT 2u

#define BINHIP_EPI_PLANES  0
#define BINHIP_EPI_SHUFFLE 1
#define BINHIP_EPI_FINAL   2
#define BINHIP_EPI_FINAL_SUBPIX 4

#define BINHIP_RDN_LAYERS 66
typedef struct BinRdnShape { int32_t G0, D, C, G; } BinRdnShape;
#define BINHIP_RDN_MAX_LAYERS 192
#define BINHIP_RDN_MAX_CONVS 7

BINHIP_API int binhip_version(void);

BINHIP_API int binhip_device_cus(void);

typedef struct BinConvDesc {
    int32_t N, H, W;
    int32_t ksize;
    int32_t cin_chunks;
    int32_t cout;
    int32_t cout_pad;
    int32_t nterms;
    int32_t epilogue;
    int32_t relu;
    int32_t x_cpg;
    int64_t x_group_stride;
    int32_t n_images;
    int32_t reserved;
    void*   status;
} BinConvDesc;

#define BINHIP_CONV_HALF_LAST_CHUNK 1

BINHIP_API int binhip_conv_cout_block(int ksize, int cout_pad, int nterms);

BINHIP_API int binhip_weights_relayout(const float* w_oihw, const float* bias, int cout, int cin, int ksize,
                            int cout_pad, int cin_chunks, int cout_block, int shuffle_perm,
                            void* w_hi, void* w_lo, float* bias_out, void* stream);
BINHIP_API size_t binhip_weights_bytes(int cout_pad, int cin_chunks, int ksize);
#define BINHIP_RELAYOUT_FWD        0
#define BINHIP_RELAYOUT_DGRAD      1
#define BINHIP_RELAYOUT_RDB_GATHER 2
typedef struct BinRelayoutItem {
    const float* w[BINHIP_RDN_MAX_CONVS + 1];
    const float* bias;
    void* w_hi;
    void* w_lo;
    float* bias_out;
    int32_t kind, cout, cin, ksize, rows_pad, cin_chunks, cout_block, shuffle_or_group;
    BinRdnShape shape;
} BinRelayoutItem;
BINHIP_API int binhip_weights_relayout_batch(const BinRelayoutItem* items, int n, void* stream);

BINHIP_API int binhip_conv2d_fwd(const BinConvDesc* d,
                      const void* x_hi, const void* x_lo,
                      const void* w_hi, const void* w_lo, const float* bias,
                      const void* res_hi, const void* res_lo,
                      void* y_hi, void* y_lo,
                      float* y_f32, const float* const* images,
                      void* stream);

BINHIP_API int binhip_dgrad_rows_pad(int ksize, int cin);
BINHIP_API int binhip_weights_relayout_dgrad(const float* w_oihw, int cout, int cin, int ksize, int rows_pad,
                                  int cin_chunks, int cout_block, int shuffle_perm, void* w_hi, void* w_lo,
                                  float* bias_out, void* stream);
BINHIP_API int binhip_weights_relayout_rdb_gather(const float* const* w_oihw4, int group, int cout_block, void* w_hi, void* w_lo,
                                       float* bias_out, void* stream);
BINHIP_API int binhip_conv2d_bwd_data(const BinConvDesc* d, const void* gy_hi, const void* gy_lo,
                           const void* wt_hi, const void* wt_lo, const float* zero_bias,
                           const void* res_hi, const void* res_lo, int res_chunks,
                           const void* acc_hi, const void* acc_lo,
                           const void* mask_hi, int mask_from,
                           int y_cpg, int64_t y_group_stride,
                           void* gx_hi, void* gx_lo, void* stream);

BINHIP_API int binhip_nchw_to_planes(const float* x, int N, int C, int H, int W, void* y_hi, void* y_lo,
                          void* status, void* stream);
BINHIP_API int binhip_planes_to_nchw(const void* x_hi, const void* x_lo, int N, int C, int H, int W, float* y,
                          void* stream);
BINHIP_API int binhip_pixel_unshuffle_f32(const float* x, int N, int C, int H, int W, int r, float* y, void* stream);
BINHIP_API int binhip_pack_inputs(const float* const* images, int n_images, int N, int H, int W,
                       void* y_hi, void* y_lo, void* status, void* stream);

BINHIP_API int binhip_u8_to_frame(const unsigned char* bgr_hwc, int H, int W, int pad_left, int pad_right,
                       int pad_top, int pad_bottom, float* out_chw, void* stream);
BINHIP_API int binhip_frame_to_u8(const float* chw, int Hp, int Wp, int top, int left, int H, int W,
                       unsigned char* bgr_hwc, void* stream);

BINHIP_API int binhip_convlstm_fwd(const float* x, const float* c_prev, const float* h_prev,
                        const float* w , const float* b , float forget_bias,
                        int N, int H, int W, float* c_new, float* h_new, void* stream);

BINHIP_API int binhip_lstm_gates_fwd(const float* gates, const float* c_prev, float forget_bias, int N, int hidden, int H, int W,
                          float* c_new, float* h_new, void* stream);
BINHIP_API int binhip_lstm_gates_bwd(const float* gates, const float* c_prev, const float* g_h, const float* g_c,
                          float forget_bias, int N, int hidden, int H, int W, float* g_gates, float* g_cprev, void* stream);

BINHIP_API int binhip_charbonnier_partials(int64_t numel);
BINHIP_API int binhip_charbonnier_fwd(const float* x, const float* y, int64_t numel, float eps,
                           float* partials, float* loss, void* stream);
BINHIP_API int binhip_charbonnier_bwd(const float* x, const float* y, int64_t numel, float eps,
                           const float* gloss, float* gx, float* gy, void* stream);
#define BINHIP_LOSS_CHARBONNIER 0
#define BINHIP_LOSS_L1_SUM      1
#define BINHIP_LOSS_L2_SUM      2
BINHIP_API int binhip_pixel_loss_fwd(int kind, const float* x, const float* y, int64_t numel, float eps,
                          float* partials, float* loss, void* stream);
BINHIP_API int binhip_pixel_loss_bwd(int kind, const float* x, const float* y, int64_t numel, float eps,
                          const float* gloss, float* gx, float* gy, void* stream);

#define BINHIP_LOSS_MAX_TERMS 24
typedef struct {
    const float* x[BINHIP_LOSS_MAX_TERMS];
    const float* y[BINHIP_LOSS_MAX_TERMS];
    int32_t n_terms;
} BinLossTerms;
BINHIP_API int binhip_multi_loss_fwd(int kind, const BinLossTerms* t, int64_t numel, float eps, float* partials, float* terms,
                          float* loss, void* stream);
typedef struct {
    float* out[BINHIP_LOSS_MAX_TERMS];
    int32_t term_a[BINHIP_LOSS_MAX_TERMS], term_b[BINHIP_LOSS_MAX_TERMS];
    float sign_a[BINHIP_LOSS_MAX_TERMS], sign_b[BINHIP_LOSS_MAX_TERMS];
    int32_t n_out;
} BinLossGrads;
BINHIP_API int binhip_multi_loss_bwd(int kind, const BinLossTerms* t, int64_t numel, float eps, const float* gloss,
                          const BinLossGrads* g, void* stream);

BINHIP_API int binhip_rdb_tail_fwd(int N, int H, int W, int nterms, const void* blk_hi, const void* blk_lo,
                        const void* wc_hi, const void* wc_lo, const float* bias_c,
                        const void* wl_hi, const void* wl_lo, const float* bias_l,
                        void* y_hi, void* y_lo, int store_o3, void* status, void* stream);

#define BINHIP_PLAN_KEEP_ACTS 1
#define BINHIP_PLAN_NO_FUSE   2
#define BINHIP_PLAN_RDB3      4
#define BINHIP_PLAN_FUSED_UPNET 8
#define BINHIP_PLAN_FUSED_UPNET_TRAIN 16
typedef struct BinRdnPlan {
    int32_t N, H, W;
    int32_t n_inputs;
    int32_t nterms;
    int32_t reserved;
    BinRdnShape shape;
    const void* w_hi[BINHIP_RDN_MAX_LAYERS];
    const void* w_lo[BINHIP_RDN_MAX_LAYERS];
    const float* bias[BINHIP_RDN_MAX_LAYERS];
    void* status;
    struct BinhipProfiler* profiler;
} BinRdnPlan;

BINHIP_API size_t binhip_rdn_workspace_bytes(int N, int H, int W, int n_inputs, int nterms, const BinRdnShape* shape );
#define BINHIP_RDN_LAYOUT_WORDS 16
BINHIP_API int binhip_rdn_workspace_layout(int N, int H, int W, int n_inputs, int nterms, const BinRdnShape* shape,
                                int64_t* out, int n_out);
BINHIP_API int binhip_rdn_forward(const BinRdnPlan* plan, const float* const* inputs , float* out ,
                       void* workspace, size_t workspace_bytes, void* stream);

BINHIP_API size_t binhip_wgrad_workspace_bytes(int ksize, int N, int H, int W, int cin_chunks, int cout);
BINHIP_API int binhip_conv2d_bwd_weight(const BinConvDesc* d, const void* x_hi, const void* x_lo,
                             const void* gy_hi, const void* gy_lo, const float* inv_scale,
                             void* workspace, size_t workspace_bytes, float* dw_oihw, float* dbias,
                             int cin, int shuffle_perm, int accumulate, void* stream);

BINHIP_API int binhip_grad_scale(const float* g, int64_t numel, float target, float* partials, float* scale_out,
                      void* stream);
BINHIP_API int binhip_nchw_to_planes_scaled(const float* x, int N, int C, int H, int W, const float* scale,
                                 void* y_hi, void* y_lo, void* status, void* stream);
BINHIP_API int binhip_unshuffle_planes(const void* x_hi, const void* x_lo, int N, int H, int W, int nchunks,
                            void* y_hi, void* y_lo, void* stream);
BINHIP_API int binhip_unpack_input_grads(const void* gx0_hi, const void* gx0_lo, const float* gout,
                              const float* scale, int n_images, int N, int H, int W,
                              float* const* outs, void* stream);

BINHIP_API size_t binhip_convlstm_bwd_workspace_bytes(int N, int H, int W);
BINHIP_API int binhip_convlstm_bwd(const float* x, const float* c_prev, const float* h_prev, const float* w,
                        const float* b, float forget_bias, int N, int H, int W, const float* g_h,
                        const float* g_c, void* workspace, size_t workspace_bytes, float* gx,
                        float* g_hprev, float* g_cprev, float* dw, float* db, void* stream);

#define BINHIP_BWD_ACCUMULATE 1
#define BINHIP_BWD_FUSED_UPNET 4
#define BINHIP_BWD_SAVED_X3   2
typedef struct BinRdnBwdPlan {
    int32_t N, H, W, n_inputs, nterms, reserved;
    BinRdnShape shape;
    const void* wt_hi[BINHIP_RDN_MAX_LAYERS];
    const void* wt_lo[BINHIP_RDN_MAX_LAYERS];
    const float* zero_bias;
    float* dw[BINHIP_RDN_MAX_LAYERS];
    float* db[BINHIP_RDN_MAX_LAYERS];
    float* gin[5];
    void* status;
    void* aux_stream;
    struct BinhipProfiler* profiler;
} BinRdnBwdPlan;
BINHIP_API size_t binhip_rdn_backward_workspace_bytes(int N, int H, int W, int n_inputs, int nterms, const BinRdnShape* shape);
#define BINHIP_RDN_BWD_LAYOUT_WORDS 24
BINHIP_API int binhip_rdn_backward_workspace_layout(int N, int H, int W, int n_inputs, int nterms, const BinRdnShape* shape,
                                         int64_t* out, int n_out);
BINHIP_API int binhip_rdn_backward(const BinRdnBwdPlan* plan, const void* saved, size_t saved_bytes,
                        const float* gout, void* workspace, size_t workspace_bytes, void* stream);

#define BINHIP_SCORE_SSIM_G11 1
#define BINHIP_SCORE_SSIM_U7  2
typedef struct BinImageScore {
    int64_t sse, sad;
    double ssim_g11, ssim_u7;
} BinImageScore;
BINHIP_API size_t binhip_image_score_workspace_bytes(int n, int H, int W, int flags);
BINHIP_API int binhip_image_score(const uint8_t* a, const uint8_t* b, int n, int H, int W, int flags, const double* g11_taps,
                       void* ws, size_t ws_bytes, BinImageScore* out, void* stream);

#define BINHIP_SCORE_MAX_PAIRS 32
BINHIP_API size_t binhip_frame_score_workspace_bytes(int n, int H, int W, int flags);
BINHIP_API int binhip_frame_score(const float* const* x, const float* const* y, int n, int H, int W, int flags,
                       const double* g11_taps, void* ws, size_t ws_bytes, BinImageScore* out, void* stream);

BINHIP_API int binhip_gather_windows(const uint8_t* frames, int n_frames, int H, int W, const int32_t* table, int n, int n_slots,
                          int ch, int cw, float* out, void* stream);

BINHIP_API int binhip_gather_windows_blur(const uint8_t* frames, int n_frames, int H, int W, const int32_t* table, int n, int n_slots,
                               int n_blur, int ch, int cw, float* out, void* stream);

#define BINHIP_PROF_WGRAD 16
typedef struct BinhipProfiler BinhipProfiler;
BINHIP_API int binhip_profiler_create(int ksize, int cout_pad, int epilogue, int max_launches, BinhipProfiler** out);
BINHIP_API int binhip_profiler_read(BinhipProfiler* p, double* total_ms, int* launches);
BINHIP_API void binhip_profiler_destroy(BinhipProfiler* p);

#ifdef __cplusplus
}
#endif
#endif
```

Baseline: 16.14 interpolated frames/s.

## Fold subpixel shuffle into 5x5 upnet conv weights with 20-tap walk

Adds a folded variant of the final 5x5 FINAL_SUBPIX conv. The weights are re-laid out on the host into a 5x4 slab, so each output 2x2 subpixel group is produced by 20 MFMA taps over one row-pair accumulator instead of 25 taps per row. A new epilogue writes the upsampled pixels directly, adding the image mean and the bias. This trims MFMA work and weight LDS traffic for that layer. It adds complexity, and the border handling skips edge pixels, which the ring kernel presumably covers.

```diff
diff --git a/bin_amd/_lib.py b/bin_amd/_lib.py
--- a/bin_amd/_lib.py
+++ b/bin_amd/_lib.py
@@ -6,6 +6,7 @@
 RDN_LAYERS = 66
 RDN_MAX_LAYERS, RDN_MAX_CONVS = 192, 7
 PLAN_KEEP_ACTS, PLAN_NO_FUSE, PLAN_RDB3, PLAN_FUSED_UPNET, PLAN_FUSED_UPNET_TRAIN = 1, 2, 4, 8, 16
+PLAN_UPNET_FOLD = 32
 BWD_ACCUMULATE = 1
 BWD_SAVED_X3 = 2
 BWD_FUSED_UPNET = 4
@@ -25,6 +26,7 @@
 
 LOSS_MAX_TERMS = 24
 CONV_HALF_LAST_CHUNK = 1
+CONV_UPNET_FOLD = 2
 
 
 class BinLossTerms(C.Structure):
diff --git a/bin_amd/csrc/binhip_conv.hip b/bin_amd/csrc/binhip_conv.hip
--- a/bin_amd/csrc/binhip_conv.hip
+++ b/bin_amd/csrc/binhip_conv.hip
@@ -254,6 +254,8 @@
     a.y_cpg_inv = c.y_cpg > 0 ? (unsigned)(((1u << 20) + c.y_cpg - 1) / c.y_cpg) : 0u;
     if (c.y_cpg > 128 || (c.y_cpg > 0 && d.cout_pad / 16 >= 4096)) return BINHIP_E_SHAPE;
     a.half_last = (d.reserved & BINHIP_CONV_HALF_LAST_CHUNK) ? 1 : 0;
+    a.upnet_fold = (d.reserved & BINHIP_CONV_UPNET_FOLD) ? 1 : 0;
+    if (a.upnet_fold && (d.epilogue != BINHIP_EPI_FINAL_SUBPIX || d.nterms != 3)) return BINHIP_E_ARG;
     a.y_unshuf = c.y_unshuf;
     if (c.y_unshuf && (d.epilogue != BINHIP_EPI_PLANES || c.y_cpg > 0 || (d.H & 1) || (d.W & 1) || c.y_unshuf * 16 < d.cout))
         return BINHIP_E_SHAPE;
@@ -703,7 +705,7 @@
                       const void* w_lo, const float* bias, const void* res_hi, const void* res_lo,
                       void* y_hi, void* y_lo, float* y_f32, const float* const* images, void* stream) {
     if (!d) return BINHIP_E_ARG;
-    if (d->reserved & ~BINHIP_CONV_HALF_LAST_CHUNK) return BINHIP_E_ARG;
+    if (d->reserved & ~(BINHIP_CONV_HALF_LAST_CHUNK | BINHIP_CONV_UPNET_FOLD)) return BINHIP_E_ARG;
     if ((d->reserved & BINHIP_CONV_HALF_LAST_CHUNK) && d->ksize != 5) return BINHIP_E_ARG;
     BhConvCall c;
     c.d = *d;
diff --git a/bin_amd/csrc/binhip_conv_common.h b/bin_amd/csrc/binhip_conv_common.h
--- a/bin_amd/csrc/binhip_conv_common.h
+++ b/bin_amd/csrc/binhip_conv_common.h
@@ -56,6 +56,7 @@
     unsigned tl_launch;
     unsigned tl_base;
 #endif
+    int upnet_fold;
     int y_unshuf;
 };
 
@@ -116,6 +117,7 @@
 #endif
 
 #define BINHIP_EPI_PLANES_LFFD 3
+#define BINHIP_EPI_SUBPIX_FOLD 5
 
 template <int N>
 __device__ __forceinline__ void wait_vmcnt() {
@@ -205,6 +207,64 @@
 template <class C>
 __device__ __forceinline__ int patch_lane_off(int n, int kg, int row) { return (kg * (C::PH * C::PW) + row * C::PW + n) * 16; }
 
+__device__ __forceinline__ void upnet_fold_epilogue(const ConvKArgs& a, const float* __restrict__ bias, const floatx16& acc, int img,
+                                                    int row0, int tx0, int n, int kg) {
+    const int H2 = 2 * a.H, W2 = 2 * a.W, ncolour = a.cout >> 2, nimg = a.nimg;
+    const int X = tx0 + n;
+    float bv[2][4];
+#pragma unroll
+    for (int g = 0; g < 2; ++g) {
+        float b8[8];
+#pragma unroll
+        for (int j = 0; j < 8; ++j) b8[j] = bias[8 * g + j];
+#pragma unroll
+        for (int q = 0; q < 4; ++q) bv[g][q] = kg ? b8[4 + q] : b8[q];
+    }
+    auto pixel = [&](int r, int g, int q, bool& ok) -> long long {
+        const int c = 2 * g + kg;
+        const int Y2 = 2 * (row0 + r) - (q >> 1), X2 = 2 * X - (q & 1);
+        ok = c < ncolour && Y2 >= 1 && Y2 <= H2 - 2 && X2 >= 1 && X2 <= W2 - 2;
+        const int cc = c < ncolour ? c : 0;
+        const int yc = Y2 < 0 ? 0 : (Y2 > H2 - 1 ? H2 - 1 : Y2), xc = X2 < 0 ? 0 : (X2 > W2 - 1 ? W2 - 1 : X2);
+        return (((long long)img * ncolour + cc) * H2 + yc) * W2 + xc;
+    };
+    float sum[2][2][4];
+#pragma unroll
+    for (int r = 0; r < 2; ++r)
+#pragma unroll
+        for (int g = 0; g < 2; ++g)
+#pragma unroll
+            for (int q = 0; q < 4; ++q) {
+                bool ok;
+                const long long idx = pixel(r, g, q, ok);
+                float v[5];
+#pragma unroll
+                for (int t = 0; t < 5; ++t) v[t] = (ok && t < nimg) ? a.img[t][idx] : 0.f;
+                float sj = v[0];
+#pragma unroll
+                for (int t = 1; t < 5; ++t)
+                    if (t < nimg) sj += v[t];
+                sum[r][g][q] = (ok && nimg > 0) ? sj / (float)nimg : 0.f;
+            }
+#pragma unroll
+    for (int r = 0; r < 2; ++r)
+#pragma unroll
+        for (int g = 0; g < 2; ++g)
+#pragma unroll
+            for (int q = 0; q < 4; ++q) asm volatile("" : "+v"(sum[r][g][q]));
+    __builtin_amdgcn_sched_barrier(0);
+#pragma unroll
+    for (int r = 0; r < 2; ++r)
+#pragma unroll
+        for (int g = 0; g < 2; ++g)
+#pragma unroll
+            for (int q = 0; q < 4; ++q) {
+                bool ok;
+                const long long idx = pixel(r, g, q, ok);
+                if (ok) a.out_f32[idx] = (acc[4 * (2 * r + g) + q] + bv[g][q]) + sum[r][g][q];
+            }
+}
+
 template <int MT, int R, int NT, int EPI, bool XTRA>
 __device__ __forceinline__ void conv_epilogue(const ConvKArgs& a, const float* __restrict__ bias, floatx16 (&acc)[MT][R],
                                               int img, int row0, int tx0, int co0, bool first_col, int n, int kg,
diff --git a/bin_amd/csrc/binhip_conv_x3.hip b/bin_amd/csrc/binhip_conv_x3.hip
--- a/bin_amd/csrc/binhip_conv_x3.hip
+++ b/bin_amd/csrc/binhip_conv_x3.hip
@@ -1,14 +1,14 @@
 #include "binhip_conv_common.h"
 constexpr int X3_R = 2, X3_WN = 8;
 
-template <int KS, int R, int WN>
+template <int KS, int R, int WN, int NTAP = KS * KS>
 struct X3Cfg {
     static constexpr int PAD = KS / 2;
     static constexpr int TH = R * WN;
     static constexpr int PH = TH + KS - 1;
     static constexpr int PW = 32 + KS - 1;
     static constexpr int PP = (PH * PW * 2 + 63) / 64;
-    static constexpr int WP = KS * KS;
+    static constexpr int WP = NTAP;
     static constexpr int NW = WN;
     static constexpr int PATCH_BYTES = PP * 1024;
     static constexpr int WBUF_BYTES = 2 * WP * 1024;
@@ -17,6 +17,9 @@
     static constexpr int NWJ = (2 * WP + NW - 1) / NW;
     static_assert((KS == 3 ? 2 : 1) * LDS_BYTES <= 160 * 1024, "LDS budget");
 };
+constexpr int X3_FOLD_TAPS = 20;
+template <int KS, int R, int WN, int EPI>
+using X3CfgOf = X3Cfg<KS, R, WN, EPI == BINHIP_EPI_SUBPIX_FOLD ? X3_FOLD_TAPS : KS * KS>;
 
 template <class C>
 __device__ __forceinline__ void x3_issue_patch(const ConvKArgs& a, char* smem, int c, int pl, int buf, int wave,
@@ -31,11 +34,11 @@
     }
 }
 
-template <class C, int KS>
+template <class C>
 __device__ __forceinline__ void x3_issue_weights(const ConvKArgs& a, char* smem, int c, int buf, int wave, int lane, int z) {
-    const long long woff = ((long long)z * a.nchunks + c) * (KS * KS * 32 * 16);
-    __amdgpu_buffer_rsrc_t wh = __builtin_amdgcn_make_buffer_rsrc((void*)(a.w_hi + woff), 0, KS * KS * 1024, 0x00020000);
-    __amdgpu_buffer_rsrc_t wl = __builtin_amdgcn_make_buffer_rsrc((void*)(a.w_lo + woff), 0, KS * KS * 1024, 0x00020000);
+    const long long woff = ((long long)z * a.nchunks + c) * (C::WP * 32 * 16);
+    __amdgpu_buffer_rsrc_t wh = __builtin_amdgcn_make_buffer_rsrc((void*)(a.w_hi + woff), 0, C::WP * 1024, 0x00020000);
+    __amdgpu_buffer_rsrc_t wl = __builtin_amdgcn_make_buffer_rsrc((void*)(a.w_lo + woff), 0, C::WP * 1024, 0x00020000);
     char* lds = smem + 2 * C::PATCH_BYTES + buf * C::WBUF_BYTES;
 #pragma unroll
     for (int j = 0; j < C::NWJ; ++j) {
@@ -80,6 +83,36 @@
 #pragma unroll
         for (int r = 0; r < R; ++r)
             acc[r] = mfma_32x32x16(Ah[s & 1], B[dx & 1][r + dy], acc[r]);
+        __builtin_amdgcn_sched_barrier(0);
+    }
+}
+
+template <class C, bool HI>
+__device__ __forceinline__ void x3_compute_fold(const char* pb, const char* wb, int a_lane_off, int b_lane_off, floatx16& acc) {
+    constexpr int NT = 5, NB = 4;
+    static_assert(C::WP == NT * NB && C::PH >= 2 * (C::NW - 1) + NT && C::PW >= 32 + NB - 1, "slab and patch of the folded walk");
+    half8 B[2][NT];
+    half8 Ah[2], Al[2];
+    auto load_b = [&](int b, half8 (&dst)[NT]) {
+#pragma unroll
+        for (int t = 0; t < NT; ++t) dst[t] = ld8(pb + b_lane_off + (t * C::PW + b) * 16);
+    };
+    auto load_a = [&](int s, half8& h, half8& l) {
+        const int b = s / NT, t = s % NT;
+        const int off = (t * NB + b) * 1024 + a_lane_off;
+        h = ld8(wb + off);
+        if constexpr (HI) l = ld8(wb + C::WP * 1024 + off);
+    };
+    load_b(0, B[0]);
+    load_a(0, Ah[0], Al[0]);
+#pragma unroll
+    for (int s = 0; s < NT * NB; ++s) {
+        const int b = s / NT, t = s % NT;
+        if (s + 1 < NT * NB) load_a(s + 1, Ah[(s + 1) & 1], Al[(s + 1) & 1]);
+        if (t == 0 && b + 1 < NB) load_b(b + 1, B[(b + 1) & 1]);
+        __builtin_amdgcn_sched_barrier(0);
+        if constexpr (HI) acc = mfma_32x32x16(Al[s & 1], B[b & 1][t], acc);
+        acc = mfma_32x32x16(Ah[s & 1], B[b & 1][t], acc);
         __builtin_amdgcn_sched_barrier(0);
     }
 }
@@ -137,7 +170,10 @@
 template <int KS, int R, int WN, int EPI, bool XTRA, bool GATED = false>
 __device__ __forceinline__ void x3_tile(const ConvKArgs& a, const float* __restrict__ bias, char* smem, const ConvTile& t,
                                         const X3Gate gate = X3Gate{nullptr, 0u, 1 << 30, nullptr}) {
-    using C = X3Cfg<KS, R, WN>;
+    constexpr bool FOLD = EPI == BINHIP_EPI_SUBPIX_FOLD;
+    static_assert(!FOLD || (KS == 5 && R == 2 && !XTRA && !GATED), "the folded walk is the 5x5 FINAL_SUBPIX layer's");
+    constexpr int RA = FOLD ? 1 : R;
+    using C = X3CfgOf<KS, R, WN, EPI>;
     BH_TL_DECL;
     BH_TL_BEGIN();
     const int tid = threadIdx.x;
@@ -149,9 +185,9 @@
     unsigned voff[C::NPJ];
     patch_offsets<C, C::PAD>(voff, t, a.H, a.W, wave, lane);
 
-    floatx16 acc[1][R];
-#pragma unroll
-    for (int r = 0; r < R; ++r)
+    floatx16 acc[1][RA];
+#pragma unroll
+    for (int r = 0; r < RA; ++r)
 #pragma unroll
         for (int e = 0; e < 16; ++e) acc[0][r][e] = 0.f;
 
@@ -160,7 +196,7 @@
     const int b_lane_off = patch_lane_off<C>(n, kg, wave * R);
 
     __builtin_amdgcn_s_setprio(2);
-    x3_issue_weights<C, KS>(a, smem, 0, 0, wave, lane, z);
+    x3_issue_weights<C>(a, smem, 0, 0, wave, lane, z);
     if constexpr (GATED) {
         if (gate.chunk <= 0 && gate.flags) {
             if (tid < 9) {
@@ -198,7 +234,7 @@
         if (c == 0) BH_TL_STAMP(1);
 #endif
         x3_issue_patch<C>(a, smem, c, 1, 1, wave, voff, t);
-        if (c + 1 < nchunks) x3_issue_weights<C, KS>(a, smem, c + 1, (c + 1) & 1, wave, lane, z);
+        if (c + 1 < nchunks) x3_issue_weights<C>(a, smem, c + 1, (c + 1) & 1, wave, lane, z);
         unsigned gate_seen = gate.epoch;
         const unsigned* gate_word = nullptr;
         if constexpr (GATED) {
@@ -210,8 +246,10 @@
                 }
             }
         }
-        const bool pair = (KS == 5) && !XTRA && a.half_last && (c + 1 == nchunks);
-        if constexpr (KS == 5 && !XTRA) {
+        const bool pair = (KS == 5) && !XTRA && !FOLD && a.half_last && (c + 1 == nchunks);
+        if constexpr (FOLD) {
+            x3_compute_fold<C, true>(smem, wb, a_lane_off, b_lane_off, acc[0][0]);
+        } else if constexpr (KS == 5 && !XTRA) {
             if (pair) x3_compute_pair<C, KS, R, true>(smem, wb, n, kg, wave, acc[0]);
             else x3_compute<C, KS, R, true>(smem, wb, a_lane_off, b_lane_off, acc[0]);
         } else {
@@ -238,7 +276,9 @@
             }
         }
         if (c + 1 < nchunks) x3_issue_patch<C>(a, smem, c + 1, 0, 0, wave, voff, t);
-        if constexpr (KS == 5 && !XTRA) {
+        if constexpr (FOLD) {
+            x3_compute_fold<C, false>(smem + C::PATCH_BYTES, wb, a_lane_off, b_lane_off, acc[0][0]);
+        } else if constexpr (KS == 5 && !XTRA) {
             if (pair) x3_compute_pair<C, KS, R, false>(smem + C::PATCH_BYTES, wb, n, kg, wave, acc[0]);
             else x3_compute<C, KS, R, false>(smem + C::PATCH_BYTES, wb, a_lane_off, b_lane_off, acc[0]);
         } else {
@@ -247,7 +287,8 @@
     }
     BH_TL_STAMP(2);
     __builtin_amdgcn_s_setprio(0);
-    conv_epilogue<1, R, 3, EPI, XTRA>(a, bias, acc, img, t.ty0 + wave * R, t.tx0, z * 32, z == 0, n, kg, t.plane_elems);
+    if constexpr (FOLD) upnet_fold_epilogue(a, bias, acc[0][0], img, t.ty0 + wave * R, t.tx0, n, kg);
+    else conv_epilogue<1, R, 3, EPI, XTRA>(a, bias, acc, img, t.ty0 + wave * R, t.tx0, z * 32, z == 0, n, kg, t.plane_elems);
     BH_TL_FINISH(a, (((img * a.tiles_y + ty) * a.tiles_x + tx) * a.ncol + z));
 }
 
@@ -256,7 +297,7 @@
     __attribute__((amdgpu_waves_per_eu((KS == 5 && !XTRA) ? WN / 4 : WN / 2, (KS == 5 && !XTRA) ? WN / 4 : WN / 2)))
 conv_x3_kernel(const ConvKArgs a, const float* __restrict__ bias) {
     extern __shared__ __attribute__((aligned(16))) char smem[];
-    x3_tile<KS, R, WN, EPI, XTRA>(a, bias, smem, tile_decode<X3Cfg<KS, R, WN>::TH>(a, a.ncol));
+    x3_tile<KS, R, WN, EPI, XTRA>(a, bias, smem, tile_decode<X3CfgOf<KS, R, WN, EPI>::TH>(a, a.ncol));
 }
 
 struct Rdb3Args {
@@ -295,7 +336,7 @@
 
 template <int KS, int R, int WN, int EPI, int WIDE, bool XTRA>
 static int launch_x3_x(const ConvKArgs& ka, int cout_pad, hipStream_t s) {
-    using C = X3Cfg<KS, R, WN>;
+    using C = X3CfgOf<KS, R, WN, EPI>;
     static std::atomic<unsigned long long> lds_set{0};
     if (int rc = bh_set_max_lds(&conv_x3_kernel<KS, R, WN, EPI, WIDE, XTRA>, C::LDS_BYTES, lds_set)) return rc;
     ConvKArgs a = ka;
@@ -604,6 +645,7 @@
 }
 
 int bh_launch_conv_x3_k5_subpix(const ConvKArgs& a, hipStream_t s) {
+    if (a.upnet_fold) return launch_x3<5, X3_R, X3_WN, BINHIP_EPI_SUBPIX_FOLD, 0>(a, 32, s);
     return launch_x3<5, X3_R, X3_WN, BINHIP_EPI_FINAL_SUBPIX, 0>(a, 32, s);
 }
 
diff --git a/bin_amd/csrc/binhip_plan.hip b/bin_amd/csrc/binhip_plan.hip
--- a/bin_amd/csrc/binhip_plan.hip
+++ b/bin_amd/csrc/binhip_plan.hip
@@ -75,6 +75,7 @@
     int x_cpg = 0;
     int64_t x_group_stride = 0;
     Planes y, res;
+    int reserved = 0;
 };
 
 }
@@ -103,6 +104,8 @@
     const int N = p->N, H = p->H, W = p->W, nin = p->n_inputs, nt = p->nterms;
     if (!frames_ok(N, H, W, nin)) return BINHIP_E_SHAPE;
     if (nt != 1 && nt != 3) return BINHIP_E_ARG;
+    if ((p->reserved & BINHIP_PLAN_UPNET_FOLD) && (nt != 3 || (p->reserved & BINHIP_PLAN_KEEP_ACTS) || !(p->reserved & BINHIP_PLAN_FUSED_UPNET)))
+        return BINHIP_E_ARG;
     Shp sh;
     if (!resolve_shape(&p->shape, &sh)) return BINHIP_E_SHAPE;
     const size_t need = binhip_rdn_workspace_bytes(N, H, W, nin, nt, &p->shape);
@@ -122,7 +125,7 @@
         BhConvCall c;
         c.d.N = N; c.d.H = l.H ? l.H : h; c.d.W = l.W ? l.W : ww; c.d.ksize = l.ks; c.d.cin_chunks = l.cin_chunks; c.d.cout = l.cout;
         c.d.cout_pad = l.cout_pad ? l.cout_pad : l.cout; c.d.nterms = nt; c.d.epilogue = l.epi; c.d.relu = l.relu;
-        c.d.x_cpg = l.x_cpg; c.d.x_group_stride = l.x_group_stride; c.d.status = p->status;
+        c.d.x_cpg = l.x_cpg; c.d.x_group_stride = l.x_group_stride; c.d.status = p->status; c.d.reserved = l.reserved;
         if (l.ks == 1 && l.epi == BINHIP_EPI_PLANES && c.d.W > 32 && c.d.W % 32 == 0) { c.d.H *= c.d.W / 32; c.d.W = 32; }
         if (l.layer == 0 && l.ks == 5 && (12 * nin) % 16 >= 1 && (12 * nin) % 16 <= 8) c.d.reserved = BINHIP_CONV_HALF_LAST_CHUNK;
         c.x_hi = A.hi(l.x); c.x_lo = A.lo(l.x);
@@ -185,8 +188,10 @@
                           (!(p->reserved & BINHIP_PLAN_KEEP_ACTS) || (p->reserved & BINHIP_PLAN_FUSED_UPNET_TRAIN)) &&
                           sh.L + 1 < BINHIP_RDN_MAX_LAYERS && p->w_hi[sh.L] && (nt == 1 || p->w_lo[sh.L]) && p->bias[sh.L] &&
                           p->w_hi[sh.L + 1] && p->bias[sh.L + 1];
+    const bool fold = (p->reserved & BINHIP_PLAN_UPNET_FOLD) != 0;
     if (fused_up) {
-        if ((rc = conv({.layer = sh.L, .ks = 5, .cin_chunks = c0, .cout = 12, .cout_pad = 32, .epi = BINHIP_EPI_FINAL_SUBPIX, .x = w.g1})))
+        if ((rc = conv({.layer = sh.L, .ks = 5, .cin_chunks = c0, .cout = 12, .cout_pad = 32, .epi = BINHIP_EPI_FINAL_SUBPIX, .x = w.g1,
+                        .reserved = fold ? BINHIP_CONV_UPNET_FOLD : 0})))
             return rc;
         return bh_launch_upnet_ring(A.hi(w.g1), A.lo(w.g1), (const float*)p->w_hi[sh.L + 1], p->bias[sh.L + 1], out, inputs, nin, N, h, ww,
                                     G0, s);
diff --git a/bin_amd/rdn_plan.py b/bin_amd/rdn_plan.py
--- a/bin_amd/rdn_plan.py
+++ b/bin_amd/rdn_plan.py
@@ -57,6 +57,33 @@
     W = torch.einsum("ciyjxgab,viy,wjx,iyat,jxbu->vwcijgtu", T, keep, keep, place, place).reshape(9, 12, g0, 5, 5)
     B = (b2.view(1, 1, 3, 1, 1) + torch.einsum("ciyjx,viy,wjx->vwcij", Tb, keep, keep)).reshape(9, 12)
     return W, B
+
+
+def folded_upnet_weights(w4):
+    w4 = w4.double()
+    g0 = w4.shape[1]
+    assert tuple(w4.shape) == (12, g0, 5, 5) and g0 % 16 == 0
+    wc = w4.view(12, g0 // 16, 16, 5, 5)
+    slab = w4.new_zeros(g0 // 16, 5, 4, 32, 16)
+    for i in range(2):
+        for j in range(2):
+            rows = slice(2 * i + j, 12, 4)
+            taps = wc[rows, :, :, i:i + 4, j:j + 4].permute(1, 3, 4, 0, 2)
+            slab[:, 0:4, :, rows] = taps
+            slab[:, 1:5, :, slice(16 + 2 * i + j, 28, 4)] = taps
+    return slab
+
+
+def folded_upnet_planes(slab):
+    w = slab.float()
+    hi = w.half()
+    lo = (w - hi.float()).half()
+    odd = ((torch.arange(32, device=w.device) >> 3) & 1).bool().view(32, 1, 1)
+
+    def swizzle(p):
+        p = p.view(*p.shape[:-1], 2, 8)
+        return torch.where(odd, p.flip(-2), p).reshape(-1).contiguous()
+    return swizzle(hi), swizzle(lo)
 
 
 _FUSED_MAPS = {}
@@ -183,6 +210,7 @@
         fusable = tuple(w0.shape[2:]) == (3, 3) and w0.shape[0] == 256 and tuple(w2.shape) == (3, 64, 3, 3)
         self._up_src = src if fusable else None
         self.fused_up = None
+        self.fused_fold = None
         self.fused_w4 = None
         self.fused_train = None
         self.fused_train_w4 = None
@@ -209,10 +237,12 @@
                 self.fused_w4 = W[4].float().contiguous()
                 main = ConvWeights(self.fused_w4, B[4].float().contiguous(), nterms=self.nterms)
                 ring_w = W.permute(0, 1, 3, 4, 2).reshape(9, 12, 25, W.shape[2]).float().contiguous()
+                if self.nterms == 3:
+                    self.fused_fold = folded_upnet_planes(folded_upnet_weights(W[4]))
                 self.fused_up = (main, ring_w, B.float().contiguous())
         return self.fused_up
 
-    def fill_plan(self, plan, fused=None):
+    def fill_plan(self, plan, fused=None, fold=False):
         plan.shape = c_shape(self.shape)
         for i, cw in enumerate(self.layers):
             plan.w_hi[i] = cw.w_hi.data_ptr()
@@ -223,6 +253,8 @@
             main, ring_w, ring_b = fused
             plan.w_hi[n], plan.bias[n] = main.w_hi.data_ptr(), main.bias.data_ptr()
             plan.w_lo[n] = main.w_lo.data_ptr() if main.w_lo is not None else None
+            if fold:
+                plan.w_hi[n], plan.w_lo[n] = (t.data_ptr() for t in self.fused_fold)
             plan.w_hi[n + 1], plan.w_lo[n + 1], plan.bias[n + 1] = ring_w.data_ptr(), None, ring_b.data_ptr()
 
     def dgrad(self, module, nterms=None, fused=False):
@@ -339,6 +371,8 @@
     flags = L.PLAN_RDB3 if _os.environ.get("BIN_AMD_RDB3", "0") == "1" else 0
     if _os.environ.get("BIN_AMD_FUSED_UPNET", "1") != "0":
         flags |= L.PLAN_FUSED_UPNET
+        if _os.environ.get("BIN_AMD_UPNET_FOLD", "1") != "0":
+            flags |= L.PLAN_UPNET_FOLD
     return flags
 
 
@@ -358,13 +392,16 @@
     plan.reserved = int(flags or 0)
     plan.status = status_word(inputs[0].device).data_ptr()
     plan.profiler = profiler if profiler else None
-    fused = None
+    fused, fold = None, False
     if plan.reserved & L.PLAN_FUSED_UPNET:
         if plan.reserved & L.PLAN_FUSED_UPNET_TRAIN:
             fused = weights.ensure_fused_upnet(train=True)
         elif not (plan.reserved & L.PLAN_KEEP_ACTS):
             fused = weights.ensure_fused_upnet()
-    weights.fill_plan(plan, fused)
+            fold = bool(plan.reserved & L.PLAN_UPNET_FOLD) and fused is not None and weights.fused_fold is not None
+    if not fold:
+        plan.reserved &= ~L.PLAN_UPNET_FOLD
+    weights.fill_plan(plan, fused, fold)
     nbytes = lib.binhip_rdn_workspace_bytes(n, h, w, weights.n_inputs, weights.nterms, C.byref(plan.shape))
     if nbytes == 0:
         raise RuntimeError(f"bin_amd: unsupported RDN shape N={n} H={h} W={w} (H, W must be even)")
diff --git a/include/binhip.h b/include/binhip.h
--- a/include/binhip.h
+++ b/include/binhip.h
@@ -51,6 +51,7 @@
 } BinConvDesc;
 
 #define BINHIP_CONV_HALF_LAST_CHUNK 1
+#define BINHIP_CONV_UPNET_FOLD 2
 
 BINHIP_API int binhip_conv_cout_block(int ksize, int cout_pad, int nterms);
 
@@ -156,6 +157,7 @@
 #define BINHIP_PLAN_RDB3      4
 #define BINHIP_PLAN_FUSED_UPNET 8
 #define BINHIP_PLAN_FUSED_UPNET_TRAIN 16
+#define BINHIP_PLAN_UPNET_FOLD 32
 typedef struct BinRdnPlan {
     int32_t N, H, W;
     int32_t n_inputs;
```

Result: faster. 16.36 interpolated frames/s (median of 6 runs) (+1.3%).
